# xmengli/H-DenseUNet

Hardware: AMD Instinct MI355X
Metric: CT slices/sec fwd+bwd (2D 512^2) (higher is better)
Workload: dtype bf16

## Files before the change

h-denseunet_amd/csrc/conv_halo_wide.hip:

```cpp
#include "conv_common.h"
#include "hdu_host.h"

typedef float f32x16 __attribute__((ext_vector_type(16)));

__device__ __forceinline__ f32x16 hdu_mfma_32x32x16_bf16(u32x4 a, u32x4 b, f32x16 c) {
#ifdef HDU_EMU
  return hipemu_mfma_32x32x16_bf16(__builtin_bit_cast(hipemu_u16x8, a), __builtin_bit_cast(hipemu_u16x8, b), c);
#else
  return __builtin_amdgcn_mfma_f32_32x32x16_bf16(__builtin_bit_cast(hdu_bf16x8, a), __builtin_bit_cast(hdu_bf16x8, b), c, 0, 0, 0);
#endif
}

template <int N> __device__ __forceinline__ void hw_wait_vmcnt() {
  static_assert(N >= 0 && N < 64, "vmcnt immediate");
#ifndef HDU_EMU
  asm volatile("s_waitcnt vmcnt(%0)" ::"i"(N) : "memory");
#endif
}

template <int TH_, int NT_, int WAVES_M_, int WAVES_N_, int NS_> struct HaloWide {
  static constexpr int TH = TH_, NT = NT_, WAVES_M = WAVES_M_, WAVES_N = WAVES_N_, NS = NS_;
  static constexpr int NW = WAVES_M * WAVES_N, NTHR = NW * 64;
  static constexpr int TW = 32, HC = TW + 2, HR = TH + 2, HP = HR * HC;
  static constexpr int BN = NT * 32, BM = TH * TW;
  static constexpr int XI = (HP * 2 + 63) / 64;
  static constexpr int WI = (BN * 18 + 63) / 64;
  static constexpr int LPW = (XI + WI + NW - 1) / NW;
  static constexpr int STAGE = LPW * NW * 1024;
  static constexpr int XBYTES = XI * 1024;
  static constexpr int ROWB = BN * 2 + 16;
  static constexpr int SMEM = NS * STAGE > BM * ROWB ? NS * STAGE : BM * ROWB;
  static constexpr int MT = TH / WAVES_M, NTW = NT / WAVES_N;
  static_assert(TH % WAVES_M == 0 && NT % WAVES_N == 0, "wave layout");
  static_assert(SMEM <= 160 * 1024, "LDS");
  static_assert((NS - 2) * LPW < 64, "vmcnt");
};

template <typename C, typename RowValid>
__device__ __forceinline__ void hw_epilogue_stats(const ConvK& p, const char* smem, int n0, int tid, unsigned slot, RowValid valid) {
  constexpr int NCC = C::BN / 8, CPI = C::NTHR / 16;
  float* dst = p.stats_partial + (long long)(slot % (unsigned)p.stats_slots) * 2 * p.Cout;
  const int rl = tid & 15;
#pragma unroll 1
  for (int it = 0; it < (NCC + CPI - 1) / CPI; ++it) {
    const int cc = (tid >> 4) + it * CPI;
    const int nbase = n0 + cc * 8;
    const bool col = cc < NCC && nbase < p.Cout;
    const int ccq = col ? cc : 0, nc = col ? nbase : 0;
    float s1[8], s2[8], sh[8];
#pragma unroll
    for (int j = 0; j < 8; j += 4) {
      const f32x4 v4 = *(const f32x4*)(p.stats_shift + nc + j);
      sh[j] = v4[0]; sh[j + 1] = v4[1]; sh[j + 2] = v4[2]; sh[j + 3] = v4[3];
    }
#pragma unroll
    for (int j = 0; j < 8; ++j) { s1[j] = 0.f; s2[j] = 0.f; }
#pragma unroll 1
    for (int q0 = 0; q0 < C::BM / 16; q0 += 8) {
      u32x4 rv[8];
#pragma unroll
      for (int q = 0; q < 8; ++q) rv[q] = *(const u32x4*)(smem + (rl + (q0 + q) * 16) * C::ROWB + ccq * 16);
#pragma unroll
      for (int q = 0; q < 8; ++q) {
        const float keep = (col && valid(rl + (q0 + q) * 16)) ? 1.f : 0.f;
        float f[8];
        Chunk<bf16_t>::unpack(rv[q], f);
#pragma unroll
        for (int j = 0; j < 8; ++j) { const float d = (f[j] - sh[j]) * keep; s1[j] += d; s2[j] += d * d; }
      }
    }
#pragma unroll
    for (int j = 0; j < 8; ++j) { s1[j] = hdu_row16_sum(s1[j]); s2[j] = hdu_row16_sum(s2[j]); }
    float mine = 0.f;
#pragma unroll
    for (int j = 0; j < 8; ++j) {
      mine = rl == j ? s1[j] : mine;
      mine = rl == 8 + j ? s2[j] : mine;
    }
    if (col) atomicAdd(dst + (rl < 8 ? 0 : p.Cout) + nbase + (rl & 7), mine);
  }
}

template <typename C>
__device__ __forceinline__ void hw_epilogue(const ConvK& p, f32x16 (&acc)[C::MT][C::NTW], char* smem, long long mplane, int y0, int x0,
                                            int n0, int wm, int wn, int lane, int tid, unsigned slot) {
  typedef bf16_t T;
  constexpr int BN = C::BN, BM = C::BM, NTHR = C::NTHR, ROWB = C::ROWB, MT = C::MT, NTW = C::NTW;
  const int l31 = lane & 31, lh = lane >> 5;
  hw_wait_vmcnt<0>();
  __syncthreads();
  const unsigned dseed = p.drop_seed + (p.drop_seed_dev ? *p.drop_seed_dev : 0u);
  const bool has_bias = p.bias != nullptr, drop = p.drop_scale != 0.f, has_epi = p.epi_a != nullptr;
#pragma unroll
  for (int j = 0; j < NTW; ++j) {
    f32x4 bias_v[4], epa_v[4], epb_v[4];
#pragma unroll
    for (int g = 0; g < 4; ++g) {
      const int nn = n0 + (wn * NTW + j) * 32 + 8 * g + 4 * lh;
      const int nc = nn < p.Cout ? nn : 0;
      bias_v[g] = has_bias ? *(const f32x4*)(p.bias + nc) : f32x4{0.f, 0.f, 0.f, 0.f};
      epa_v[g] = has_epi ? *(const f32x4*)(p.epi_a + nc) : f32x4{1.f, 1.f, 1.f, 1.f};
      epb_v[g] = has_epi ? *(const f32x4*)(p.epi_b + nc) : f32x4{0.f, 0.f, 0.f, 0.f};
    }
#pragma unroll
    for (int i = 0; i < MT; ++i) {
      const int trow = wm * MT + i;
      const int row = trow * 32 + l31;
      const long long m = (mplane + y0 + trow) * p.Wo + x0 + l31;
#pragma unroll
      for (int g = 0; g < 4; ++g) {
        const int col = (wn * NTW + j) * 32 + 8 * g + 4 * lh;
        const int nn = n0 + col;
        float v[4] = {acc[i][j][4 * g], acc[i][j][4 * g + 1], acc[i][j][4 * g + 2], acc[i][j][4 * g + 3]};
        if (has_bias) {
#pragma unroll
          for (int r = 0; r < 4; ++r) v[r] += bias_v[g][r];
        }
        if (drop) {
#pragma unroll
          for (int r = 0; r < 4; ++r) {
            const unsigned h = hdu_hash32((unsigned long long)m * (unsigned)p.Cout + (unsigned)(nn + r), dseed);
            v[r] = h < p.drop_thresh ? v[r] * p.drop_scale : 0.f;
          }
        }
        if (has_epi) {
#pragma unroll
          for (int r = 0; r < 4; ++r) {
            v[r] = epa_v[g][r] * v[r] + epb_v[g][r];
            if (p.epi_relu) v[r] = v[r] > 0.f ? v[r] : 0.f;
          }
        }
        Chunk<T>::store4((T*)(smem + row * ROWB) + col, v);
      }
    }
  }
  __syncthreads();
  T* __restrict__ yp = (T*)p.y;
  constexpr int NCC = BN / 8;
  constexpr int NIT = (BM * NCC + NTHR - 1) / NTHR;
  auto out_ptr = [&](int q, bool& ok) -> T* {
    const int row = q / NCC, cc = q - row * NCC;
    const int oy = y0 + (row >> 5), ox = x0 + (row & 31);
    const int nn = n0 + cc * 8;
    ok = q < BM * NCC && oy < p.Ho && ox < p.Wo && nn < p.Cout;
    return ok ? yp + ((mplane + oy) * p.Wo + ox) * p.ldy + nn : yp;
  };
  if (p.accumulate) {
#pragma unroll 1
    for (int it0 = 0; it0 < NIT; it0 += 4) {
      u32x4 old[4];
      T* dst[4];
      bool ok[4];
#pragma unroll
      for (int u = 0; u < 4; ++u) {
        dst[u] = out_ptr(tid + (it0 + u) * NTHR, ok[u]);
        ok[u] = ok[u] && it0 + u < NIT;
        old[u] = *(const u32x4*)dst[u];
      }
#pragma unroll
      for (int u = 0; u < 4; ++u) {
        if (!ok[u]) continue;
        const int q = tid + (it0 + u) * NTHR;
        const int row = q / NCC, cc = q - row * NCC;
        float f[8], g[8];
        Chunk<T>::unpack(*(const u32x4*)(smem + row * ROWB + cc * 16), f);
        Chunk<T>::unpack(old[u], g);
#pragma unroll
        for (int jj = 0; jj < 8; ++jj) f[jj] += g[jj];
        *(u32x4*)dst[u] = Chunk<T>::pack(f);
      }
    }
  } else {
#pragma unroll
    for (int it = 0; it < NIT; ++it) {
      const int q = tid + it * NTHR;
      bool ok;
      T* dst = out_ptr(q, ok);
      if (!ok) continue;
      const int row = q / NCC, cc = q - row * NCC;
      *(u32x4*)dst = *(const u32x4*)(smem + row * ROWB + cc * 16);
    }
  }
  if (p.stats_partial)
    hw_epilogue_stats<C>(p, smem, n0, tid, slot, [&](int row) { return y0 + (row >> 5) < p.Ho && x0 + (row & 31) < p.Wo; });
}

template <typename C>
__global__ __launch_bounds__(C::NTHR) void conv_halo_wide_kernel(ConvK p, int tiles_x, int tiles_y, int ngroups) {
  typedef bf16_t T;
  constexpr int TH = C::TH, HC = C::HC, HP = C::HP, BN = C::BN, BM = C::BM, NW = C::NW, NTHR = C::NTHR, NS = C::NS;
  constexpr int XI = C::XI, WI = C::WI, LPW = C::LPW, STAGE = C::STAGE, XBYTES = C::XBYTES, ROWB = C::ROWB;
  constexpr int MT = C::MT, NTW = C::NTW;
  __shared__ __attribute__((aligned(16))) char smem[C::SMEM];

  const int tid = threadIdx.x;
  const int lane = tid & 63;
#ifdef HDU_EMU
  const int wave = tid >> 6;
#else
  const int wave = __builtin_amdgcn_readfirstlane(tid >> 6);
#endif
  const int wm = wave / C::WAVES_N, wn = wave % C::WAVES_N;
  const T* __restrict__ xp = (const T*)p.x;
  const int He = p.He, We = p.We;

  unsigned t = (p.xcd_swizzle & 1) ? xcd_tile_index(blockIdx.x, gridDim.x) : blockIdx.x;
  const int ng = (int)(t % (unsigned)ngroups); t /= (unsigned)ngroups;
  const int od = (int)(t % (unsigned)p.Do); t /= (unsigned)p.Do;
  const int txi = (int)(t % (unsigned)tiles_x); t /= (unsigned)tiles_x;
  const int tyi = (int)(t % (unsigned)tiles_y);
  const int n = (int)(t / (unsigned)tiles_y);
  const int y0 = tyi * TH, x0 = txi * C::TW;
  const int n0 = ng * BN;

  unsigned roff[LPW];
  int rlc[LPW];
#pragma unroll
  for (int j = 0; j < LPW; ++j) {
    const int jj = j * NW + wave;
    if (jj < XI) {
      const int q = jj * 64 + lane;
      const int hp = q >> 1;
      const int lc = (q & 1) ^ ((hp >> 3) & 1);
      const int hr = hp / HC, hc = hp - hr * HC;
      const int iy = y0 - 1 + hr, ix = x0 - 1 + hc;
      const bool ok = hp < HP && (unsigned)iy < (unsigned)He && (unsigned)ix < (unsigned)We;
      roff[j] = ok ? (unsigned)(((iy >> p.uh) * p.Wi + (ix >> p.uw)) * (int)p.ldx + lc * 8) * 2u : HDU_OOB;
      rlc[j] = lc * 8;
    } else if (jj < XI + WI) {
      const int q = (jj - XI) * 64 + lane;
      const int row = q / 18, rem = q - row * 18;
      const int tap = rem >> 1;
      const int lc = (rem & 1) ^ ((row >> 3) & 1);
      const int co = n0 + row;
      const bool ok = row < BN && co < p.Cout;
      roff[j] = ok ? (unsigned)((co * p.KD * 9 + tap) * p.Cin + lc * 8) * 2u : HDU_OOB;
      rlc[j] = lc * 8;
    } else {
      roff[j] = HDU_OOB;
      rlc[j] = 0;
    }
  }
  const hdu_bufsrd wsrd = hdu_make_srd(p.w, p.w_bytes);
  const long long plane_elems = (long long)p.Hi * p.Wi * p.ldx;
  const unsigned plane_bytes = (unsigned)((((long long)p.Hi * p.Wi - 1) * p.ldx + p.Cin) * 2);

  auto stage_plane = [&](int kd, int c0) -> const T* {
    const int pz = od + kd - p.pd;
    return xp + (long long)(n * p.Di + (pz >> p.ud)) * plane_elems + c0;
  };
  auto issue_piece = [&](const hdu_bufsrd& xsrd, unsigned woff, int c0, char* base, int j, bool live) {
    const int jj = j * NW + wave;
    const bool ok = live && roff[j] != HDU_OOB && c0 + rlc[j] < p.Cin;
    if (jj < XI) hdu_bufload_lds16(xsrd, ok ? roff[j] : HDU_OOB, base + jj * 1024);
    else hdu_bufload_lds16(wsrd, ok ? roff[j] + woff : HDU_OOB, base + jj * 1024);
  };

  f32x16 acc[MT][NTW];
#pragma unroll
  for (int i = 0; i < MT; ++i)
#pragma unroll
    for (int j = 0; j < NTW; ++j)
#pragma unroll
      for (int r = 0; r < 16; ++r) acc[i][j][r] = 0.f;

  const int kd_lo = p.pd - od > 0 ? p.pd - od : 0;
  const int kd_hi = p.De + p.pd - od < p.KD ? p.De + p.pd - od : p.KD;
  const int nch = (p.Cin + 15) >> 4;
  const int nst = kd_hi > kd_lo ? (kd_hi - kd_lo) * nch : 0;
  int ikd = kd_lo, ic = 0;
#pragma unroll
  for (int pre = 0; pre < NS - 1; ++pre) {
    const bool live = pre < nst;
    const int c0 = live ? ic * 16 : 0;
    const hdu_bufsrd xsrd = hdu_make_srd(stage_plane(live ? ikd : kd_lo, c0), plane_bytes - (unsigned)c0 * 2u);
    const unsigned woff = (unsigned)(ikd * 9 * p.Cin + c0) * 2u;
#pragma unroll
    for (int j = 0; j < LPW; ++j) issue_piece(xsrd, woff, c0, smem + pre * STAGE, j, live);
    if (live && ++ic == nch) { ic = 0; ++ikd; }
  }

  const int l31 = lane & 31, lh = lane >> 5;
  int wrow_off[NTW];
#pragma unroll
  for (int j = 0; j < NTW; ++j) {
    const int row = (wn * NTW + j) * 32 + l31;
    wrow_off[j] = XBYTES + row * 288 + ((lh ^ ((row >> 3) & 1)) << 4);
  }
  const int hp_base = wm * MT * HC + l31;

  int slot = 0;
  for (int s = 0; s < nst; ++s) {
    hw_wait_vmcnt<(NS - 2) * LPW>();
    HDU_RAW_BARRIER();
    const bool more = s + NS - 1 < nst;
    const int nc0 = more ? ic * 16 : 0;
    const hdu_bufsrd nxsrd = hdu_make_srd(stage_plane(more ? ikd : kd_lo, nc0), plane_bytes - (unsigned)nc0 * 2u);
    const unsigned nwoff = (unsigned)(ikd * 9 * p.Cin + nc0) * 2u;
    char* nbase = smem + (slot == 0 ? NS - 1 : slot - 1) * STAGE;
    if (more && ++ic == nch) { ic = 0; ++ikd; }
    const char* Xs = smem + slot * STAGE;
    constexpr int PER_TAP = (LPW + 8) / 9;
#pragma unroll
    for (int tap = 0; tap < 9; ++tap) {
      const int kh = tap / 3, kw = tap - kh * 3;
      u32x4 af[MT], bf[NTW];
#pragma unroll
      for (int i = 0; i < MT; ++i) {
        const int hp = hp_base + (i + kh) * HC + kw;
        af[i] = *(const u32x4*)(Xs + hp * 32 + ((lh ^ ((hp >> 3) & 1)) << 4));
      }
#pragma unroll
      for (int j = 0; j < NTW; ++j) bf[j] = *(const u32x4*)(Xs + wrow_off[j] + tap * 32);
#pragma unroll
      for (int i = 0; i < MT; ++i)
#pragma unroll
        for (int j = 0; j < NTW; ++j) acc[i][j] = hdu_mfma_32x32x16_bf16(bf[j], af[i], acc[i][j]);
#pragma unroll
      for (int u = 0; u < PER_TAP; ++u)
        if (tap * PER_TAP + u < LPW) issue_piece(nxsrd, nwoff, nc0, nbase, tap * PER_TAP + u, more);
    }
    slot = slot == NS - 1 ? 0 : slot + 1;
  }

  const long long mplane = ((long long)n * p.Do + od) * p.Ho;
  hw_epilogue<C>(p, acc, smem, mplane, y0, x0, n0, wm, wn, lane, tid, blockIdx.x);
}

struct StemCfg {
  static constexpr int TH = 16, NT = 3, WAVES_M = 8, WAVES_N = 1, NS = 4;
  static constexpr int NW = 8, NTHR = 512, TW = 32;
  static constexpr int BN = 96, BM = TH * TW;
  static constexpr int SEG = 70;
  static constexpr int XSLOTS = TH * SEG;
  static constexpr int XI = (XSLOTS + 63) / 64;
  static constexpr int WSLOTS = BN * 9;
  static constexpr int WI = (WSLOTS + 63) / 64;
  static constexpr int LPW = (XI + WI + NW - 1) / NW;
  static constexpr int STAGE = LPW * NW * 1024;
  static constexpr int XBYTES = XI * 1024;
  static constexpr int ROWB = BN * 2 + 16;
  static constexpr int SMEM = NS * STAGE > BM * ROWB ? NS * STAGE : BM * ROWB;
  static constexpr int MT = 2, NTW = 3;
  static_assert(SMEM <= 160 * 1024, "LDS");
};

__global__ __launch_bounds__(StemCfg::NTHR) void conv_stem_s2_kernel(ConvK p, int tiles_x, int tiles_y, int ngroups) {
  typedef StemCfg C;
  typedef bf16_t T;
  constexpr int NW = C::NW, NS = C::NS, XI = C::XI, WI = C::WI, LPW = C::LPW, STAGE = C::STAGE, XBYTES = C::XBYTES, SEG = C::SEG;
  constexpr int MT = C::MT, NTW = C::NTW, BN = C::BN;
  __shared__ __attribute__((aligned(16))) char smem[C::SMEM];
  const int tid = threadIdx.x;
  const int lane = tid & 63;
#ifdef HDU_EMU
  const int wave = tid >> 6;
#else
  const int wave = __builtin_amdgcn_readfirstlane(tid >> 6);
#endif
  const T* __restrict__ xp = (const T*)p.x;
  unsigned t = (p.xcd_swizzle & 1) ? xcd_tile_index(blockIdx.x, gridDim.x) : blockIdx.x;
  const int ng = (int)(t % (unsigned)ngroups); t /= (unsigned)ngroups;
  const int od = (int)(t % (unsigned)p.Do); t /= (unsigned)p.Do;
  const int txi = (int)(t % (unsigned)tiles_x); t /= (unsigned)tiles_x;
  const int tyi = (int)(t % (unsigned)tiles_y);
  const int n = (int)(t / (unsigned)tiles_y);
  const int y0 = tyi * C::TH, x0 = txi * C::TW;
  const int n0 = ng * BN;

  unsigned roff[LPW];
  int riy[LPW];
#pragma unroll
  for (int j = 0; j < LPW; ++j) {
    const int jj = j * NW + wave;
    riy[j] = -(1 << 28);
    if (jj < XI) {
      const int ps = jj * 64 + lane;
      const int q = ps ^ ((ps >> 4) & 1);
      const int r = q / SEG, c = q - r * SEG;
      const int iy = 2 * (y0 + r) - p.ph, ix = 2 * x0 - p.pw + c;
      const bool ok = q < C::XSLOTS && (unsigned)ix < (unsigned)p.Wi;
      roff[j] = ok ? (unsigned)((iy * p.Wi + ix) * (int)p.ldx) * 2u : HDU_OOB;
      riy[j] = ok ? iy : -(1 << 28);
    } else if (jj < XI + WI) {
      const int ps = (jj - XI) * 64 + lane;
      const int row = ps / 9, kw = ps - row * 9;
      const int co = n0 + row;
      const bool ok = row < BN && co < p.Cout && kw < 7;
      roff[j] = ok ? (unsigned)((co * p.KD * 49 + kw) * 8) * 2u : HDU_OOB;
    } else {
      roff[j] = HDU_OOB;
    }
  }
  const hdu_bufsrd wsrd = hdu_make_srd(p.w, p.w_bytes);
  const long long plane_elems = (long long)p.Hi * p.Wi * p.ldx;
  const unsigned plane_bytes = (unsigned)((((long long)p.Hi * p.Wi - 1) * p.ldx + 8) * 2);
  const int row_bytes = p.Wi * (int)p.ldx * 2;

  auto stage_plane = [&](int kd) -> const T* {
    const int pz = od * p.sd + kd - p.pd;
    return xp + (long long)(n * p.Di + pz) * plane_elems;
  };
  auto issue_piece = [&](const hdu_bufsrd& xsrd, int kd, int kh, char* base, int j, bool live) {
    const int jj = j * NW + wave;
    if (jj < XI) {
      const bool ok = live && (unsigned)(riy[j] + kh) < (unsigned)p.Hi;
      hdu_bufload_lds16(xsrd, ok ? roff[j] + (unsigned)(kh * row_bytes) : HDU_OOB, base + jj * 1024);
    } else {
      const bool ok = live && roff[j] != HDU_OOB;
      hdu_bufload_lds16(wsrd, ok ? roff[j] + (unsigned)((kd * 7 + kh) * 7 * 8 * 2) : HDU_OOB, base + jj * 1024);
    }
  };

  f32x16 acc[MT][NTW];
#pragma unroll
  for (int i = 0; i < MT; ++i)
#pragma unroll
    for (int j = 0; j < NTW; ++j)
#pragma unroll
      for (int r = 0; r < 16; ++r) acc[i][j][r] = 0.f;

  const int pz0 = od * p.sd - p.pd;
  const int kd_lo = pz0 < 0 ? -pz0 : 0;
  const int kd_hi = p.Di - pz0 < p.KD ? p.Di - pz0 : p.KD;
  const int nst = kd_hi > kd_lo ? (kd_hi - kd_lo) * 7 : 0;
  int ikd = kd_lo, ikh = 0;
#pragma unroll
  for (int pre = 0; pre < NS - 1; ++pre) {
    const bool live = pre < nst;
    const hdu_bufsrd xsrd = hdu_make_srd(stage_plane(live ? ikd : kd_lo), plane_bytes);
#pragma unroll
    for (int j = 0; j < LPW; ++j) issue_piece(xsrd, ikd, ikh, smem + pre * STAGE, j, live);
    if (live && ++ikh == 7) { ikh = 0; ++ikd; }
  }

  const int l31 = lane & 31, lh = lane >> 5;
  int wrow_off[NTW];
#pragma unroll
  for (int j = 0; j < NTW; ++j) wrow_off[j] = XBYTES + ((j * 32 + l31) * 9 + lh) * 16;
  int xq[MT];
#pragma unroll
  for (int i = 0; i < MT; ++i) xq[i] = (wave * MT + i) * SEG + 2 * l31 + lh;

  int slot = 0;
  for (int s = 0; s < nst; ++s) {
    hw_wait_vmcnt<(NS - 2) * LPW>();
    HDU_RAW_BARRIER();
    const bool more = s + NS - 1 < nst;
    const hdu_bufsrd nxsrd = hdu_make_srd(stage_plane(more ? ikd : kd_lo), plane_bytes);
    const int nkd = ikd, nkh = ikh;
    char* nbase = smem + (slot == 0 ? NS - 1 : slot - 1) * STAGE;
    if (more && ++ikh == 7) { ikh = 0; ++ikd; }
    const char* Xs = smem + slot * STAGE;
#pragma unroll
    for (int ks = 0; ks < 4; ++ks) {
      u32x4 af[MT], bf[NTW];
#pragma unroll
      for (int i = 0; i < MT; ++i) {
        const int q = xq[i] + 2 * ks;
        af[i] = *(const u32x4*)(Xs + ((q ^ ((q >> 4) & 1)) << 4));
      }
#pragma unroll
      for (int j = 0; j < NTW; ++j) bf[j] = *(const u32x4*)(Xs + wrow_off[j] + ks * 32);
#pragma unroll
      for (int i = 0; i < MT; ++i)
#pragma unroll
        for (int j = 0; j < NTW; ++j) acc[i][j] = hdu_mfma_32x32x16_bf16(bf[j], af[i], acc[i][j]);
      if (ks < LPW) issue_piece(nxsrd, nkd, nkh, nbase, ks, more);
    }
    slot = slot == NS - 1 ? 0 : slot + 1;
  }
  const long long mplane = ((long long)n * p.Do + od) * p.Ho;
  hw_epilogue<C>(p, acc, smem, mplane, y0, x0, n0, wave, 0, lane, tid, blockIdx.x);
}

template <int NS_> struct StemWT {
  static constexpr int TH = 4, TW = 32, PX = TH * TW, SEG = 70, NR = 2 * TH + 5, NW = 8, NTHR = 512, NS = NS_;
  static constexpr int DSLOTS = PX * 12, DI = DSLOTS / 64;
  static constexpr int XSLOTS = NR * SEG, XI = (XSLOTS + 63) / 64;
  static constexpr int LPW = (DI + XI + NW - 1) / NW;
  static constexpr int STAGE = LPW * NW * 1024, DBYTES = DI * 1024;
  static_assert(NS * STAGE <= 160 * 1024, "LDS");
};

typedef StemWT<2> StemW;
template <int NS_>
__global__ __launch_bounds__(StemW::NTHR) void conv_stem_wgrad_kernel(ConvK p, float* __restrict__ dw, int tiles_x, int tiles_y,
                                                                      int nsplit, int ngroups) {
// ... 292 lines not shown
```

h-denseunet_amd/csrc/conv_igemm.hip:

```cpp
#include "conv_common.h"
#include "../../include/hdu.h"

template <typename T, int BM, int BN> struct BnbGeom {
  static constexpr int CH = Chunk<T>::CH;
  static constexpr int NCC = BN / CH;
  static constexpr int NCCP = NCC <= 4 ? 4 : (NCC <= 8 ? 8 : (NCC <= 16 ? 16 : 32));
  static constexpr int RSTEP = 256 / NCCP;
  static constexpr int IT = (BM + RSTEP - 1) / RSTEP;
  static constexpr bool EARLY = IT <= 8;
  static_assert(NCC <= 32, "tile shape");
};

template <bool SPLIT, typename T, int BM, int BN, int WAVES_M, int WAVES_N>
__device__ __forceinline__ void conv_igemm_body(const ConvK& p, char* smem) {
  constexpr int CH = Chunk<T>::CH;
  constexpr int BK = 8 * CH;
  constexpr int A_IT = BM / 32;
  constexpr int B_IT = (BN + 31) / 32;
  constexpr int WM = BM / WAVES_M;
  constexpr int WN = BN / WAVES_N;
  constexpr int TM = WM / 16;
  constexpr int TN = WN / 16;
  constexpr int STAGE = (BM + BN) * 128;
  static_assert(WAVES_M * WAVES_N == 4, "4 waves");
// ... 2429 lines not shown
#pragma unroll
        for (int i = 0; i < 2; ++i)
#pragma unroll
          for (int j = 0; j < TN; ++j) acc[i][j] = Mma<T>::kgroup(bf[j], af[i], acc[i][j]);
      }
    }
    __syncthreads();
  }

  constexpr int ROWB = BN * 2 + 16;
  const unsigned dseed = p.drop_seed + (p.drop_seed_dev ? *p.drop_seed_dev : 0u);
  const bool has_bias = p.bias != nullptr, drop = p.drop_scale != 0.f, has_epi = p.epi_a != nullptr;
  f32x4 bias_v[TN], epa_v[TN], epb_v[TN];
#pragma unroll
  for (int j = 0; j < TN; ++j) {
    const int nn = n0 + j * 16 + lg * 4;
    const int nc = nn < p.Cout ? nn : 0;
    bias_v[j] = has_bias ? *(const f32x4*)(p.bias + nc) : f32x4{0.f, 0.f, 0.f, 0.f};
    epa_v[j] = has_epi ? *(const f32x4*)(p.epi_a + nc) : f32x4{1.f, 1.f, 1.f, 1.f};
    epb_v[j] = has_epi ? *(const f32x4*)(p.epi_b + nc) : f32x4{0.f, 0.f, 0.f, 0.f};
  }
#pragma unroll
  for (int i = 0; i < 2; ++i) {
    const int tx = i * 16 + li;
    const int row = wave * 32 + tx;
    const long long m = ((long long)(n * H + y0 + wave)) * W + x0 + tx;
#pragma unroll
    for (int j = 0; j < TN; ++j) {
      const int col = j * 16 + lg * 4;
      const int nn = n0 + col;
      float v[4] = {acc[i][j][0], acc[i][j][1], acc[i][j][2], acc[i][j][3]};
      if (has_bias) {
#pragma unroll
        for (int r = 0; r < 4; ++r) v[r] += bias_v[j][r];
      }
      if (drop) {
#pragma unroll
        for (int r = 0; r < 4; ++r) {
          const unsigned h = hdu_hash32((unsigned long long)m * (unsigned)p.Cout + (unsigned)(nn + r), dseed);
          v[r] = h < p.drop_thresh ? v[r] * p.drop_scale : 0.f;
        }
      }
      if (has_epi) {
#pragma unroll
        for (int r = 0; r < 4; ++r) {
          v[r] = epa_v[j][r] * v[r] + epb_v[j][r];
          if (p.epi_relu) v[r] = v[r] > 0.f ? v[r] : 0.f;
        }
      }
      Chunk<T>::store4((T*)(smem + row * ROWB) + col, v);
    }
  }
  __syncthreads();
  T* __restrict__ yp = (T*)p.y;
  constexpr int NCC = BN / 8;
  for (int q = tid; q < BM * NCC; q += 256) {
    const int row = q / NCC, cc = q - row * NCC;
    const int oy = y0 + (row >> 5), ox = x0 + (row & 31);
    const int nn = n0 + cc * 8;
    if (oy >= H || ox >= W || nn >= p.Cout) continue;
    u32x4 v = *(const u32x4*)(smem + row * ROWB + cc * 16);
    T* dst = yp + (((long long)(n * H + oy)) * W + ox) * p.ldy + nn;
    if (p.accumulate) {
      float f[8], g[8];
      Chunk<T>::unpack(v, f);
      Chunk<T>::unpack(*(const u32x4*)dst, g);
#pragma unroll
      for (int jj = 0; jj < 8; ++jj) f[jj] += g[jj];
      v = Chunk<T>::pack(f);
    }
    *(u32x4*)dst = v;
  }
  if (p.stats_partial)
    epilogue_stats<T, BM, BN, ROWB>(p, smem, n0, tid, blockIdx.x,
                                    [&](int row) { return y0 + (row >> 5) < H && x0 + (row & 31) < W; });
}

template <typename T>
__global__ __launch_bounds__(256) void conv_dgrad_strided_kernel(ConvK p) {
  constexpr int CH = Chunk<T>::CH;
  const int ncc = p.Cin / CH;
  const long long total = (long long)p.N * p.Di * p.Hi * p.Wi * ncc;
  const T* __restrict__ dyp = (const T*)p.y;
  const T* __restrict__ wp = (const T*)p.w;
  T* __restrict__ dxp = (T*)p.x;
  for (long long q = (long long)blockIdx.x * blockDim.x + threadIdx.x; q < total;
       q += (long long)gridDim.x * blockDim.x) {
    const int cc = (int)(q % ncc);
    long long pix = q / ncc;
    const int iw = (int)(pix % p.Wi);
    long long t = pix / p.Wi;
    const int ih = (int)(t % p.Hi);
    t /= p.Hi;
    const int id = (int)(t % p.Di);
    const int n = (int)(t / p.Di);
    float acc[CH];
#pragma unroll
    for (int j = 0; j < CH; ++j) acc[j] = 0.f;
    for (int kd = 0; kd < p.KD; ++kd) {
      const int td = id + p.pd - kd;
      if (td < 0 || td % p.sd) continue;
      const int od = td / p.sd;
      if (od >= p.Do) continue;
      for (int kh = 0; kh < p.KH; ++kh) {
        const int th = ih + p.ph - kh;
        if (th < 0 || th % p.sh) continue;
        const int oh = th / p.sh;
        if (oh >= p.Ho) continue;
        for (int kw = 0; kw < p.KW; ++kw) {
          const int tw = iw + p.pw - kw;
          if (tw < 0 || tw % p.sw) continue;
          const int ow = tw / p.sw;
          if (ow >= p.Wo) continue;
          const long long m = (((long long)n * p.Do + od) * p.Ho + oh) * p.Wo + ow;
          const int tap = (kd * p.KH + kh) * p.KW + kw;
          const T* dyr = dyp + m * p.ldy;
          const T* wr = wp + (long long)tap * p.Cin + cc * CH;
          for (int co = 0; co < p.Cout; ++co) {
            const float g = Chunk<T>::load1(dyr + co);
            float wv[CH];
            Chunk<T>::unpack(*(const u32x4*)(wr + (long long)co * p.Ktot), wv);
#pragma unroll
            for (int j = 0; j < CH; ++j) acc[j] += g * wv[j];
          }
        }
      }
    }
    T* o = dxp + pix * p.ldx + cc * CH;
    if (p.accumulate) {
      float old[CH];
      Chunk<T>::unpack(*(const u32x4*)o, old);
#pragma unroll
      for (int j = 0; j < CH; ++j) acc[j] += old[j];
    }
    *(u32x4*)o = Chunk<T>::pack(acc);
  }
}

struct ParityGeom {
  int nt[3];
  int kmax[3];
  int step[3];
  long long dst_off;
};
struct ParityTable { ParityGeom c[8]; int n; };

template <typename T>
__global__ __launch_bounds__(256) void stride2_filter_kernel(const float* __restrict__ wm, int Cout, int KD, int KH, int KW,
                                                            int Cin, ParityTable tab, T* __restrict__ out) {
  const ParityGeom g = tab.c[blockIdx.y];
  const long long total = (long long)Cin * g.nt[0] * g.nt[1] * g.nt[2] * Cout;
  for (long long q = (long long)blockIdx.x * blockDim.x + threadIdx.x; q < total; q += (long long)gridDim.x * blockDim.x) {
    const int co = (int)(q % Cout);
    long long t = q / Cout;
    const int tw = (int)(t % g.nt[2]); t /= g.nt[2];
    const int th = (int)(t % g.nt[1]); t /= g.nt[1];
    const int td = (int)(t % g.nt[0]);
    const int ci = (int)(t / g.nt[0]);
    const int kd = g.kmax[0] - g.step[0] * td, kh = g.kmax[1] - g.step[1] * th, kw = g.kmax[2] - g.step[2] * tw;
    const float v = wm[((((long long)co * KD + kd) * KH + kh) * KW + kw) * Cin + ci];
    Chunk<T>::store1(out + g.dst_off + q, v);
  }
}

template <typename T>
__global__ __launch_bounds__(256) void parity_interleave_kernel(const T* __restrict__ cls, int N, int Di, int Hi, int Wi, int C,
                                                               int sd, int sh, int sw, T* __restrict__ dx, long long lddx,
                                                               int accumulate) {
  constexpr int CH = Chunk<T>::CH;
  const int ncc = C / CH;
  const long long total = (long long)N * Di * Hi * Wi * ncc;
  const int Dq = (Di + sd - 1) / sd, Hq = (Hi + sh - 1) / sh, Wq = (Wi + sw - 1) / sw;
  const long long cls_elems = (long long)N * Dq * Hq * Wq * C;
  for (long long q = (long long)blockIdx.x * blockDim.x + threadIdx.x; q < total; q += (long long)gridDim.x * blockDim.x) {
    const int cc = (int)(q % ncc);
    long long pix = q / ncc;
    const int iw = (int)(pix % Wi);
    long long t = pix / Wi;
    const int ih = (int)(t % Hi);
    t /= Hi;
    const int id = (int)(t % Di);
    const int n = (int)(t / Di);
    const int rd = id % sd, rh = ih % sh, rw = iw % sw;
    const int ci = (rd * sh + rh) * sw + rw;
    const long long src = ci * cls_elems + ((((long long)n * Dq + id / sd) * Hq + ih / sh) * Wq + iw / sw) * C + cc * CH;
    u32x4 v = *(const u32x4*)(cls + src);
    T* o = dx + pix * lddx + cc * CH;
    if (accumulate) {
      float a[CH], b[CH];
      Chunk<T>::unpack(v, a);
      Chunk<T>::unpack(*(const u32x4*)o, b);
#pragma unroll
      for (int j = 0; j < CH; ++j) a[j] += b[j];
      v = Chunk<T>::pack(a);
    }
    *(u32x4*)o = v;
  }
}

template <typename T>
__global__ __launch_bounds__(256) void weight_prep_kernel(const float* __restrict__ wm, int Cout, int Tn, int Cin,
                                                         T* __restrict__ wf, T* __restrict__ wd) {
  const long long total = (long long)Cout * Tn * Cin;
  for (long long q = (long long)blockIdx.x * blockDim.x + threadIdx.x; q < total;
       q += (long long)gridDim.x * blockDim.x) {
    const int ci = (int)(q % Cin);
    const long long t2 = q / Cin;
    const int t = (int)(t2 % Tn);
    const int co = (int)(t2 / Tn);
    const float v = wm[q];
    if (wf) Chunk<T>::store1(wf + q, v);
    if (wd) Chunk<T>::store1(wd + ((long long)ci * Tn + (Tn - 1 - t)) * Cout + co, v);
  }
}

#define HDU_PREP_TPW 2
template <typename T>
__global__ __launch_bounds__(256) void weight_prep_batched_kernel(const hdu_prep_entry* __restrict__ table, int n,
                                                                 const float* __restrict__ master, T* __restrict__ wc,
                                                                 long long total_tiles) {
  __shared__ float tile[2][64][65];
  const long long t0 = (long long)blockIdx.x * HDU_PREP_TPW;
  int lo = 0, hi = n - 1;
  while (lo < hi) {
    const int mid = (lo + hi + 1) >> 1;
    if (table[mid].tile_begin <= t0) lo = mid; else hi = mid - 1;
  }
  hdu_prep_entry e = table[lo];
  long long next_begin = lo + 1 < n ? table[lo + 1].tile_begin : total_tiles;
  const int tx = threadIdx.x & 15, ty = threadIdx.x >> 4;
  for (int it = 0; it < HDU_PREP_TPW; ++it) {
    const long long t = t0 + it;
    if (t >= total_tiles) break;
    while (t >= next_begin) {
      ++lo;
      e = table[lo];
      next_begin = lo + 1 < n ? table[lo + 1].tile_begin : total_tiles;
    }
    const int t_local = (int)(t - e.tile_begin);
    const int nci = (e.Cin + 63) / 64, nco = (e.Cout + 63) / 64;
    const int cib = t_local % nci;
    const int cob = (t_local / nci) % nco;
    const int tap = t_local / (nci * nco);
    const float* wm = master + e.master_off;
    T* wf = e.w_f_off >= 0 ? wc + e.w_f_off : nullptr;
    T* wd = e.w_d_off >= 0 ? wc + e.w_d_off : nullptr;
    float (*tl)[65] = tile[it & 1];
    const bool vec = ((e.master_off | (e.w_f_off >= 0 ? e.w_f_off : 0) | (e.w_d_off >= 0 ? e.w_d_off : 0) | (long long)e.Cin | (long long)e.Cout) & 3) == 0 &&
                     (((uintptr_t)master | (uintptr_t)wc) & 15) == 0;
    if (vec) {
#pragma unroll
      for (int k = 0; k < 4; ++k) {
        const int r = ty + 16 * k;
        const int co = cob * 64 + r, ci = cib * 64 + tx * 4;
        float v[4] = {0.f, 0.f, 0.f, 0.f};
        if (co < e.Cout && ci < e.Cin) {
          const long long q = ((long long)co * e.T + tap) * e.Cin + ci;
          const f32x4 m = *(const f32x4*)(wm + q);
          v[0] = m.x; v[1] = m.y; v[2] = m.z; v[3] = m.w;
          if (wf) Chunk<T>::store4(wf + q, v);
        }
#pragma unroll
        for (int j = 0; j < 4; ++j) tl[r][tx * 4 + j] = v[j];
      }
      __syncthreads();
      if (wd) {
#pragma unroll
        for (int k = 0; k < 4; ++k) {
          const int r = ty + 16 * k;
          const int ci = cib * 64 + r, co = cob * 64 + tx * 4;
          if (co < e.Cout && ci < e.Cin) {
            const float v[4] = {tl[tx * 4 + 0][r], tl[tx * 4 + 1][r], tl[tx * 4 + 2][r], tl[tx * 4 + 3][r]};
            Chunk<T>::store4(wd + ((long long)ci * e.T + (e.T - 1 - tap)) * e.Cout + co, v);
          }
        }
      }
    } else {
      for (int idx = threadIdx.x; idx < 64 * 64; idx += 256) {
        const int r = idx >> 6, c = idx & 63;
        const int co = cob * 64 + r, ci = cib * 64 + c;
        float v = 0.f;
        if (co < e.Cout && ci < e.Cin) {
          const long long q = ((long long)co * e.T + tap) * e.Cin + ci;
          v = wm[q];
          if (wf) Chunk<T>::store1(wf + q, v);
        }
        tl[r][c] = v;
      }
      __syncthreads();
      if (wd) {
        for (int idx = threadIdx.x; idx < 64 * 64; idx += 256) {
          const int r = idx >> 6, c = idx & 63;
          const int ci = cib * 64 + r, co = cob * 64 + c;
          if (co < e.Cout && ci < e.Cin)
            Chunk<T>::store1(wd + ((long long)ci * e.T + (e.T - 1 - tap)) * e.Cout + co, tl[c][r]);
        }
      }
    }
  }
}

#include "hdu_host.h"

int g_tuning[32] = {2, 0, 0, 1, 0, 0, 0, 0, 0, 0, 0, 0, 0, 0, 0, 0, 0, 0, 0, 0, 0, 0, 0, 0, 0, 0, 0, 0, 0, 0, 0, 0};

extern "C" int hdu_set_tuning(int key, int value) {
  if (key < 0 || key >= 32) return hdu_set_error(HDU_ERR_ARG, "set_tuning: bad key");
  g_tuning[key] = value;
  return 0;
}

static void fastdiv_magic(int d, unsigned* mul, unsigned* shr) {
  if (d <= 1) { *mul = 0u; *shr = 0u; return; }
  int cl = 0;
  while ((1ll << cl) < (long long)d) ++cl;
  const int p = 31 + cl;
  *mul = (unsigned)((((unsigned long long)1 << p) + (unsigned long long)d - 1) / (unsigned long long)d);
  *shr = (unsigned)(p - 32);
}

static int fill_convk(const hdu_conv_desc* d, ConvK* k, bool wgrad, bool exact_grid = false) {
  if (!d) return hdu_set_error(HDU_ERR_ARG, "conv: null descriptor");
  if (d->dtype != HDU_BF16 && d->dtype != HDU_F32) return hdu_set_error(HDU_ERR_ARG, "conv: bad dtype");
  const int ch = d->dtype == HDU_BF16 ? 8 : 4;
  if (d->Cin <= 0 || d->Cin % ch) return hdu_set_error(HDU_ERR_ARG, "conv: Cin must be a positive multiple of the 16-byte chunk");
  if (d->ldx % ch || (d->skip && d->ldskip % ch)) return hdu_set_error(HDU_ERR_ARG, "conv: input pixel stride must be a multiple of the 16-byte chunk");
  if (wgrad && (d->ldy % ch || d->Cout % ch)) return hdu_set_error(HDU_ERR_ARG, "conv_wgrad: dy stride / Cout must be multiples of the 16-byte chunk");
  if ((uintptr_t)d->x % 16 || (uintptr_t)d->w % 16 || (d->skip && (uintptr_t)d->skip % 16))
    return hdu_set_error(HDU_ERR_ARG, "conv: x / w / skip must be 16-byte aligned");
  if ((d->ud | d->uh | d->uw) & ~1) return hdu_set_error(HDU_ERR_ARG, "conv: upsample shifts must be 0 or 1");
  if (d->KD <= 0 || d->KH <= 0 || d->KW <= 0 || d->sd <= 0 || d->sh <= 0 || d->sw <= 0)
    return hdu_set_error(HDU_ERR_ARG, "conv: bad kernel/stride");
  if ((d->pro_a == nullptr) != (d->pro_b == nullptr)) return hdu_set_error(HDU_ERR_ARG, "conv: pro_a/pro_b must both be set");
  k->x = d->x; k->skip = d->skip; k->w = d->w; k->y = d->y;
  k->pro_a = d->pro_a; k->pro_b = d->pro_b; k->bias = d->bias;
  k->epi_a = wgrad ? nullptr : d->epi_a; k->epi_b = d->epi_b; k->epi_relu = d->epi_relu;
  if (k->epi_a && (!k->epi_b || d->accumulate || d->stats_partial || d->bnb_u))
    return hdu_set_error(HDU_ERR_ARG, "conv: the output affine needs epi_b and excludes accumulate / epilogue statistics / the fused BN backward");
  k->ldx = d->ldx; k->ldskip = d->ldskip; k->ldy = d->ldy;
  k->N = d->N; k->Di = d->Di; k->Hi = d->Hi; k->Wi = d->Wi; k->Cin = d->Cin;
  k->ud = d->ud; k->uh = d->uh; k->uw = d->uw;
  k->De = d->Di << d->ud; k->He = d->Hi << d->uh; k->We = d->Wi << d->uw;
  k->KD = d->KD; k->KH = d->KH; k->KW = d->KW;
  k->sd = d->sd; k->sh = d->sh; k->sw = d->sw;
  k->pd = d->pd; k->ph = d->ph; k->pw = d->pw;
  k->Do = d->Do; k->Ho = d->Ho; k->Wo = d->Wo; k->Cout = d->Cout;
  const int eDo = (k->De + 2 * d->pd - d->KD) / d->sd + 1;
  const int eHo = (k->He + 2 * d->ph - d->KH) / d->sh + 1;
  const int eWo = (k->We + 2 * d->pw - d->KW) / d->sw + 1;
  const bool exact = wgrad || exact_grid;
  const int xd = exact ? 0 : d->KD - 1, xh = exact ? 0 : d->KH - 1, xw = exact ? 0 : d->KW - 1;
  if (d->Do < eDo || d->Do > eDo + xd || d->Ho < eHo || d->Ho > eHo + xh || d->Wo < eWo || d->Wo > eWo + xw)
    return hdu_set_error(HDU_ERR_ARG, "conv: output dims inconsistent with input dims / kernel / stride / pad");
  k->M = (long long)d->N * d->Do * d->Ho * d->Wo;
  if ((long long)d->N * k->De * k->He * k->We >= (1ll << 31) || k->M >= (1ll << 31))
    return hdu_set_error(HDU_ERR_ARG, "conv: more than 2^31 pixels per tensor (shard the volume)");
  k->Ktot = d->KD * d->KH * d->KW * d->Cin;
  fastdiv_magic(d->Wo, &k->div_wo_mul, &k->div_wo_shr);
  fastdiv_magic(d->Ho, &k->div_ho_mul, &k->div_ho_shr);
  fastdiv_magic(d->Do, &k->div_do_mul, &k->div_do_shr);
  k->spread_h = k->spread_d = 0u;
  if (d->KD * d->KH * d->KW <= 32) {
    for (int q = 0; q < d->KH; ++q) k->spread_h |= 1u << (q * d->KW);
    for (int q = 0; q < d->KD; ++q) k->spread_d |= 1u << (q * d->KH * d->KW);
  }
  fastdiv_magic(d->Cin, &k->div_cin_mul, &k->div_cin_shr);
  fastdiv_magic(d->KW, &k->div_kw_mul, &k->div_kw_shr);
  fastdiv_magic(d->KH, &k->div_kh_mul, &k->div_kh_shr);
  k->sk_div_mul = 0u; k->sk_div_shr = 0u;
  {
    const long long esz = d->dtype == HDU_BF16 ? 2 : 4;
    const long long xb = (((long long)d->N * d->Di * d->Hi * d->Wi - 1) * d->ldx + d->Cin) * esz;
    const long long wb = (long long)d->Cout * k->Ktot * esz;
    k->x_bytes = xb > 0 && xb < (1ll << 32) ? (unsigned)xb : 0u;
    if (g_tuning[HDU_TUNE_DEBUG] & 16) k->x_bytes = 0u;
    if (!wgrad && wb >= (1ll << 32)) return hdu_set_error(HDU_ERR_ARG, "conv: filter larger than 4 GiB");
    k->w_bytes = (unsigned)wb;
  }
  k->pro_relu = d->pro_relu; k->accumulate = d->accumulate;
  if (d->drop_keep > 0.f && d->drop_keep < 1.f) {
    k->drop_scale = 1.f / d->drop_keep;
    k->drop_thresh = (unsigned)((double)d->drop_keep * 4294967296.0);
  } else {
    k->drop_scale = 0.f;
    k->drop_thresh = 0xffffffffu;
  }
  k->drop_seed = d->drop_seed;
  k->drop_seed_dev = d->drop_seed_dev;
  k->stats_partial = wgrad ? nullptr : d->stats_partial;
  k->stats_shift = d->stats_shift;
  k->stats_slots = d->stats_slots;
  if (k->stats_partial && (!k->stats_shift || k->stats_slots <= 0 || d->accumulate))
    return hdu_set_error(HDU_ERR_ARG, "conv: epilogue statistics need stats_shift, stats_slots > 0 and accumulate == 0");
  k->bnb_u = wgrad ? nullptr : d->bnb_u; k->bnb_ldu = d->bnb_ldu;
  k->bnb_a = d->bnb_a; k->bnb_b = d->bnb_b; k->bnb_mean = d->bnb_mean; k->bnb_rstd = d->bnb_rstd;
  k->bnb_relu = d->bnb_relu; k->bnb_partial = d->bnb_partial; k->bnb_slots = d->bnb_slots;
  if (k->bnb_u) {
    if (!k->bnb_a || !k->bnb_b || (uintptr_t)k->bnb_u % 16 || k->bnb_ldu % ch || d->pro_a || d->skip || d->bias ||
        d->stats_partial || (d->drop_keep > 0.f && d->drop_keep < 1.f))
      return hdu_set_error(HDU_ERR_ARG, "conv: the fused BN backward needs bnb_a/bnb_b, a 16-byte addressable bnb_u and a plain data-gradient launch (no prologue / skip / bias / dropout / statistics)");
    if (k->bnb_partial && (!k->bnb_mean || !k->bnb_rstd || k->bnb_slots <= 0))
      return hdu_set_error(HDU_ERR_ARG, "conv: bnb_partial needs bnb_mean, bnb_rstd and bnb_slots > 0");
  }
  if (((uintptr_t)k->bias | (uintptr_t)k->epi_a | (uintptr_t)k->epi_b | (uintptr_t)(k->stats_partial ? k->stats_shift : nullptr) |
       (uintptr_t)k->bnb_a | (uintptr_t)k->bnb_b | (uintptr_t)k->bnb_mean | (uintptr_t)k->bnb_rstd) & 15)
    return hdu_set_error(HDU_ERR_ARG, "conv: bias / epi_* / stats_shift / bnb_* vectors must be 16-byte aligned");
  k->M_layer = d->layer_rows > 0 ? d->layer_rows : k->M;
  k->sk_ws = wgrad ? nullptr : (float*)d->splitk_ws;
  k->sk_cnt = wgrad ? nullptr : d->splitk_counters;
  if (k->sk_ws && ((uintptr_t)k->sk_ws % 16 || !k->sk_cnt))
    return hdu_set_error(HDU_ERR_ARG, "conv: splitk_ws must be 16-byte aligned and come with splitk_counters");
  k->xcd_swizzle = g_tuning[HDU_TUNE_XCD_SWIZZLE];
  k->vec_out = 1;
  k->debug_flags = g_tuning[HDU_TUNE_DEBUG];
  k->f32_split = (d->dtype == HDU_F32 && g_tuning[HDU_TUNE_F32_SPLIT]) ? 1 : 0;
  if (!wgrad && d->y && (d->Cout % ch || d->ldy % ch || (uintptr_t)d->y % 16))
    return hdu_set_error(HDU_ERR_ARG, "conv: Cout / output pixel stride must be multiples of the 16-byte chunk and y 16-byte aligned");
  return 0;
}

static bool igemm_fast_ok(const ConvK& k) {
  if (g_tuning[HDU_TUNE_NO_FAST]) return false;
  if ((k.ud | k.uh | k.uw) != 0 || k.KD * k.KH * k.KW > 32) return false;
  const long long span = ((long long)k.N * k.De * k.He * k.We + (long long)k.He * k.We * 8) * k.ldx;
  return span < (1ll << 31) && k.x_bytes != 0;
}

static bool conv_pointwise(const ConvK& k) {
  return k.KD * k.KH * k.KW == 1 && k.sd == 1 && k.sh == 1 && k.sw == 1 && (k.pd | k.ph | k.pw) == 0 && (k.ud | k.uh | k.uw) == 0;
}

static bool igemm_pro_dma_ok(const ConvK& k) {
  return k.pro_a != nullptr && k.skip == nullptr && k.vec_out && k.bnb_u == nullptr && conv_pointwise(k) && k.Cin <= HDU_PRO_CMAX &&
         k.Do == k.De && k.Ho == k.He && k.Wo == k.We && igemm_fast_ok(k) && !g_tuning[HDU_TUNE_NO_PRO_DMA] &&
         ((uintptr_t)k.pro_a % 16 == 0) && ((uintptr_t)k.pro_b % 16 == 0);
}

static int ring_wgs_per_cu(int bm, bool bf16) { return (bm == 64 && bf16) ? 2 : 1; }

static int choose_splitk(long long nblk, int nk, int bm, int bn, int per_cu, size_t* bytes) {
  *bytes = 0;
  const int mode = g_tuning[HDU_TUNE_SPLITK];
  const int target = g_tuning[HDU_TUNE_SPLITK_TARGET] > 0 ? g_tuning[HDU_TUNE_SPLITK_TARGET] : 256 * per_cu;
  const int min_steps = g_tuning[HDU_TUNE_SPLITK_MIN_STEPS] > 0 ? g_tuning[HDU_TUNE_SPLITK_MIN_STEPS] : 4;
  if (mode == 1 || nblk > target / 2) return 1;
  int S = mode >= 2 ? mode : (int)((target + nblk - 1) / nblk);
  if (S > nk / min_steps) S = nk / min_steps;
  if (S > 16) S = 16;
  if (S < 2) return 1;
  *bytes = (size_t)nblk * (size_t)S * (size_t)bm * (size_t)bn * sizeof(float);
  return S;
}

static bool igemm_ring_ok(long long nblk, int Ktot, int stage_bytes, int nsd) {
  const int mode = g_tuning[HDU_TUNE_DMA_STAGES];
  return stage_bytes * nsd <= 160 * 1024 && (mode == 6 || (mode == 2 && nblk <= 256 && Ktot > g_tuning[HDU_TUNE_RING_MIN_K]));
}

template <typename T, int BM, int BN, int PROC> struct ProRing {
  static constexpr int STAGE = (BM + ((BN + 31) / 32) * 32) * 128;
  static constexpr int NSD = STAGE * 6 <= 160 * 1024 ? 6 : 4;
  static constexpr int NSR0 = (BM == 64 && sizeof(T) == 2 && NSD == 6) ? 3 : NSD;
  static constexpr int NSR = (NSR0 * STAGE + 8 * PROC <= 160 * 1024) ? NSR0 : (NSR0 == 6 ? 4 : 3);
  static_assert(NSR * STAGE + 8 * PROC <= 160 * 1024, "LDS");
};

template <typename T, int BM, int BN, int WMv, int WNv, int PROC>
static void launch_igemm_pro(const ConvK& k, dim3 grid, size_t sk_bytes_avail, hipStream_t s) {
  typedef ProRing<T, BM, BN, PROC> R;
  const long long nblk = (long long)grid.x * grid.y;
  const long long nblk_layer = (long long)((k.M_layer + BM - 1) / BM) * grid.y;
  if (igemm_ring_ok(nblk_layer, k.Ktot, R::STAGE, R::NSD)) {
    constexpr int BK = 8 * Chunk<T>::CH;
    size_t need;
    const int S = choose_splitk(nblk_layer, (k.Ktot + BK - 1) / BK, BM, BN, ring_wgs_per_cu(BM, sizeof(T) == 2), &need);
    need = need / (size_t)nblk_layer * (size_t)nblk;
    ConvK kk = k;
    if (S > 1 && k.sk_ws && k.sk_cnt && need <= sk_bytes_avail && nblk <= 512) {
      grid.z = (unsigned)S;
      fastdiv_magic(S, &kk.sk_div_mul, &kk.sk_div_shr);
    }
    HDU_LAUNCH((conv_igemm_ring_kernel<T, BM, BN, WMv, WNv, R::NSR, true, false, PROC>), grid, dim3(256), 0, s, kk);
  } else {
    HDU_LAUNCH((conv_igemm_dma_kernel<T, BM, BN, WMv, WNv, true, false, PROC>), grid, dim3(256), 0, s, k);
  }
}

template <typename T, int BM, int BN, int WMv, int WNv>
static void launch_igemm(const ConvK& k, size_t sk_bytes_avail, hipStream_t s) {
  dim3 grid((unsigned)((k.M + BM - 1) / BM), (unsigned)((k.Cout + BN - 1) / BN), 1);
  if (igemm_pro_dma_ok(k)) {
    if (k.Cin <= HDU_PRO_CSMALL) launch_igemm_pro<T, BM, BN, WMv, WNv, HDU_PRO_CSMALL>(k, grid, sk_bytes_avail, s);
    else launch_igemm_pro<T, BM, BN, WMv, WNv, HDU_PRO_CMAX>(k, grid, sk_bytes_avail, s);
    return;
  }
  if (k.pro_a == nullptr && k.skip == nullptr && k.vec_out) {
    constexpr int STAGE = (BM + ((BN + 31) / 32) * 32) * 128;
    constexpr int NSD = STAGE * 6 <= 160 * 1024 ? 6 : 4;
    const long long nblk = (long long)grid.x * grid.y;
    const long long nblk_layer = (long long)((k.M_layer + BM - 1) / BM) * grid.y;
    const int mode = g_tuning[HDU_TUNE_DMA_STAGES];
    const bool fast = igemm_fast_ok(k);
    if (igemm_ring_ok(nblk_layer, k.Ktot, STAGE, NSD)) {
      constexpr int BK = 8 * Chunk<T>::CH;
      size_t need;
      const int S = choose_splitk(nblk_layer, (k.Ktot + BK - 1) / BK, BM, BN, ring_wgs_per_cu(BM, sizeof(T) == 2), &need);
      need = need / (size_t)nblk_layer * (size_t)nblk;
      ConvK kk = k;
      if (S > 1 && k.sk_ws && k.sk_cnt && need <= sk_bytes_avail && nblk <= 512) {
        grid.z = (unsigned)S;
        fastdiv_magic(S, &kk.sk_div_mul, &kk.sk_div_shr);
      }
      constexpr int NSR = (BM == 64 && sizeof(T) == 2 && NSD == 6) ? 3 : NSD;
      if (k.bnb_u != nullptr) {
        if (fast) HDU_LAUNCH((conv_igemm_ring_kernel<T, BM, BN, WMv, WNv, NSR, true, true>), grid, dim3(256), 0, s, kk);
        else HDU_LAUNCH((conv_igemm_ring_kernel<T, BM, BN, WMv, WNv, NSR, false, true>), grid, dim3(256), 0, s, kk);
      } else if (fast) HDU_LAUNCH((conv_igemm_ring_kernel<T, BM, BN, WMv, WNv, NSR, true>), grid, dim3(256), 0, s, kk);
      else HDU_LAUNCH((conv_igemm_ring_kernel<T, BM, BN, WMv, WNv, NSR, false>), grid, dim3(256), 0, s, kk);
    } else {
      if (k.bnb_u != nullptr) {
        if (fast) HDU_LAUNCH((conv_igemm_dma_kernel<T, BM, BN, WMv, WNv, true, true>), grid, dim3(256), 0, s, k);
        else HDU_LAUNCH((conv_igemm_dma_kernel<T, BM, BN, WMv, WNv, false, true>), grid, dim3(256), 0, s, k);
      } else if (fast) HDU_LAUNCH((conv_igemm_dma_kernel<T, BM, BN, WMv, WNv, true>), grid, dim3(256), 0, s, k);
      else HDU_LAUNCH((conv_igemm_dma_kernel<T, BM, BN, WMv, WNv, false>), grid, dim3(256), 0, s, k);
    }
  } else
    HDU_LAUNCH((conv_igemm_kernel<T, BM, BN, WMv, WNv>), grid, dim3(256), 0, s, k);
}

static void choose_igemm(const ConvK& k, int* bm, int* bn) {
  const int cands[5] = {128, 96, 64, 48, 32};
  int best = 64;
  long long best_cost = -1;
  const int maxbn = g_tuning[HDU_TUNE_MAX_BN] > 0 ? g_tuning[HDU_TUNE_MAX_BN] : 128;
  for (int i = 0; i < 5; ++i) {
    const int c = cands[i];
    if (c > maxbn) continue;
    const long long ntiles = (k.Cout + c - 1) / c;
    const long long cost = ntiles * (c + 32);
    if (best_cost < 0 || cost < best_cost) { best_cost = cost; best = c; }
  }
  *bn = best;
  *bm = (k.M_layer <= (g_tuning[HDU_TUNE_BM64_MAX_M] > 0 ? (long long)g_tuning[HDU_TUNE_BM64_MAX_M] : 16384)) ? 64 : 128;
}

template <int BM, int BN> struct WaveLayout {
  static constexpr int WM = (BN >= 128) ? 2 : ((BM == 64 && (BN == 64 || BN == 32)) ? 2 : 4);
  static constexpr int WN = 4 / WM;
};

template <typename T, int BM>
static void dispatch_igemm_bn(const ConvK& k, int bn, size_t skb, hipStream_t s) {
  switch (bn) {
    case 128: launch_igemm<T, BM, 128, WaveLayout<BM, 128>::WM, WaveLayout<BM, 128>::WN>(k, skb, s); return;
    case 96: launch_igemm<T, BM, 96, WaveLayout<BM, 96>::WM, WaveLayout<BM, 96>::WN>(k, skb, s); return;
    case 64: launch_igemm<T, BM, 64, WaveLayout<BM, 64>::WM, WaveLayout<BM, 64>::WN>(k, skb, s); return;
    case 48: launch_igemm<T, BM, 48, WaveLayout<BM, 48>::WM, WaveLayout<BM, 48>::WN>(k, skb, s); return;
    default: launch_igemm<T, BM, 32, WaveLayout<BM, 32>::WM, WaveLayout<BM, 32>::WN>(k, skb, s); return;
  }
}

static int pers_table_cap(int bn, int cin) {
  const int stage3 = 3 * (256 + bn) * 128;
  if (cin <= HDU_PRO_CSMALL && stage3 + 8 * HDU_PRO_CSMALL <= 160 * 1024) return HDU_PRO_CSMALL;
  if (stage3 + 8 * HDU_PRO_CMAX <= 160 * 1024) return HDU_PRO_CMAX;
  return -1;
}

static bool igemm_pers_ok(const ConvK& k, int bn) {
  if (g_tuning[HDU_TUNE_PERS] == 0) return false;
  if (k.skip != nullptr || !k.vec_out || k.bnb_u != nullptr || !igemm_fast_ok(k)) return false;
  if (k.f32_split) return false;
  if (k.pro_a != nullptr && (!igemm_pro_dma_ok(k) || pers_table_cap(bn, k.Cin) < 0)) return false;
  const long long items = ((k.M_layer + 255) / 256) * ((k.Cout + bn - 1) / bn);
  const int min_items = g_tuning[HDU_TUNE_PERS_MIN_ITEMS] > 0 ? g_tuning[HDU_TUNE_PERS_MIN_ITEMS] : 512;
  return items >= min_items && k.M < (1ll << 31) - 256;
}

template <typename T, int BN>
static void launch_pers(const ConvK& k, hipStream_t s) {
  const int tiles_m = (int)((k.M + 255) / 256), tiles_n = (k.Cout + BN - 1) / BN;
  const int cus = g_tuning[HDU_TUNE_PERS] > 1 ? g_tuning[HDU_TUNE_PERS] : 256;
  long long items = (long long)tiles_m * tiles_n;
  const dim3 grid((unsigned)(items < cus ? items : cus));
  if (k.pro_a != nullptr) {
    const int cap = pers_table_cap(BN, k.Cin);
    if (cap == HDU_PRO_CSMALL) {
      if constexpr (3 * (256 + BN) * 128 + 8 * HDU_PRO_CSMALL <= 160 * 1024)
        HDU_LAUNCH((conv_igemm_pers_kernel<T, BN, HDU_PRO_CSMALL>), grid, dim3(512), 0, s, k, tiles_m, tiles_n);
    } else {
      if constexpr (3 * (256 + BN) * 128 + 8 * HDU_PRO_CMAX <= 160 * 1024)
        HDU_LAUNCH((conv_igemm_pers_kernel<T, BN, HDU_PRO_CMAX>), grid, dim3(512), 0, s, k, tiles_m, tiles_n);
    }
  } else {
    HDU_LAUNCH((conv_igemm_pers_kernel<T, BN, 0>), grid, dim3(512), 0, s, k, tiles_m, tiles_n);
  }
}

template <typename T>
static void dispatch_igemm(const ConvK& k, size_t skb, hipStream_t s) {
  int bm, bn;
  choose_igemm(k, &bm, &bn);
  if (bm == 128 && igemm_pers_ok(k, bn)) {
    switch (bn) {
      case 128: launch_pers<T, 128>(k, s); return;
      case 96: launch_pers<T, 96>(k, s); return;
      case 64: launch_pers<T, 64>(k, s); return;
      case 48: launch_pers<T, 48>(k, s); return;
      default: launch_pers<T, 32>(k, s); return;
    }
  }
  if (bm == 64) dispatch_igemm_bn<T, 64>(k, bn, skb, s);
  else dispatch_igemm_bn<T, 128>(k, bn, skb, s);
}

bool hdu_halo_wide_taken(const ConvK& k, int dtype);
const char* hdu_halo_wide_name(const ConvK& k, int dtype);
bool hdu_halo_wide_launch(const ConvK& k, int dtype, hipStream_t s);
bool hdu_stem_wgrad_taken(const ConvK& k, int dtype);
bool hdu_stem_wgrad_launch(const ConvK& k, int dtype, float* dw, hipStream_t s);

static bool fprop_halo_ok(const ConvK& k, int dtype) {
  return dtype == HDU_BF16 && k.bnb_u == nullptr && !g_tuning[HDU_TUNE_NO_HALO_FPROP] && k.pro_a == nullptr && k.skip == nullptr && k.KD == 1 &&
         k.KH == 3 && k.KW == 3 && k.sd == 1 && k.sh == 1 && k.sw == 1 && k.pd == 0 && k.ph == 1 && k.pw == 1 &&
         (k.ud | k.uh | k.uw) == 0 && k.Di == 1 && k.Cin % 8 == 0 && k.We >= 32 && k.He >= 4 &&
         k.Do == 1 && k.Ho == k.He && k.Wo == k.We &&
         k.Cin >= 128 && k.Cout <= 96 &&
         (long long)k.N * ((k.He + 3) / 4) * ((k.We + 31) / 32) * k.M_layer / k.M >= (g_tuning[HDU_TUNE_HALO_MIN_TILES] > 0 ? g_tuning[HDU_TUNE_HALO_MIN_TILES] : 128);
}

static int choose_halo_bn(const ConvK& k) {
  const int cands[4] = {96, 64, 48, 32};
  int best = 64;
  long long best_cost = -1;
  for (int i = 0; i < 4; ++i) {
    const int c = cands[i];
    const long long cost = (long long)((k.Cout + c - 1) / c) * (c + 24);
    if (best_cost < 0 || cost < best_cost) { best_cost = cost; best = c; }
  }
  return best;
}

template <int BN>
static void launch_halo_fprop(const ConvK& k, hipStream_t s) {
  const unsigned tiles = (unsigned)(k.N * ((k.He + 3) / 4) * ((k.We + 31) / 32));
  HDU_LAUNCH((conv_halo_fprop_kernel<BN>), dim3(tiles, (unsigned)((k.Cout + BN - 1) / BN)), dim3(256), 0, s, k);
}

static bool pw_bstat_ok(const ConvK& k, int dtype) {
  return dtype == HDU_BF16 && !g_tuning[HDU_TUNE_NO_PW_BSTAT] && k.KD * k.KH * k.KW == 1 && k.sd == 1 && k.sh == 1 && k.sw == 1 &&
         (k.pd | k.ph | k.pw) == 0 && (k.ud | k.uh | k.uw) == 0 && k.pro_a == nullptr && k.skip == nullptr && k.bias == nullptr &&
         k.epi_a == nullptr && k.stats_partial == nullptr && (k.bnb_u != nullptr ? (!g_tuning[HDU_TUNE_NO_PW_BSTAT_BNB] && !(k.bnb_relu & 6)) : !k.accumulate) &&
         k.drop_scale == 0.f &&
         (k.Ktot == 128 || k.Ktot == 192) && k.Cout >= 256 && k.M >= 64 && k.x_bytes != 0 &&
         (k.M - 1) * k.ldy + k.Cout < (1ll << 31) && (k.bnb_u == nullptr || (k.M - 1) * k.bnb_ldu + k.Cout < (1ll << 31)) &&
         (long long)k.Cout * k.Ktot * 2 < (1ll << 31) && k.Do == k.De && k.Ho == k.He && k.Wo == k.We;
}

template <int BN, int NSA>
static void launch_pw_bstat_form(const ConvK& k, int target, hipStream_t s) {
  const unsigned ny = (unsigned)((k.Cout + BN - 1) / BN);
  long long splits = target / (long long)ny;
  if (splits < 1) splits = 1;
  const long long tiles = (k.M + 63) / 64;
  if (splits > tiles) splits = tiles;
  const long long rows = ((tiles + splits - 1) / splits) * 64;
  const unsigned gx = (unsigned)((k.M + rows - 1) / rows);
  if (k.bnb_u != nullptr) {
    if (k.Ktot == 192) HDU_LAUNCH((conv_pw_bstat_kernel<3, BN, true, NSA>), dim3(gx, ny), dim3(256), 0, s, k, (int)rows);
    else HDU_LAUNCH((conv_pw_bstat_kernel<2, BN, true, NSA>), dim3(gx, ny), dim3(256), 0, s, k, (int)rows);
    return;
  }
  if (k.Ktot == 192) HDU_LAUNCH((conv_pw_bstat_kernel<3, BN, false, NSA>), dim3(gx, ny), dim3(256), 0, s, k, (int)rows);
  else HDU_LAUNCH((conv_pw_bstat_kernel<2, BN, false, NSA>), dim3(gx, ny), dim3(256), 0, s, k, (int)rows);
}

static int pw_bstat_form(const ConvK& k) {
  const int f = g_tuning[HDU_TUNE_PW_BSTAT_FORM];
  if (f == 1 || f == 2) return f;
  return k.bnb_u != nullptr ? 2 : 1;
}

static void launch_pw_bstat(const ConvK& k, hipStream_t s) {
  const int wgs = g_tuning[HDU_TUNE_PW_BSTAT_WGS];
  if (pw_bstat_form(k) == 2) launch_pw_bstat_form<64, 2>(k, wgs > 0 ? wgs : 512, s);
  else launch_pw_bstat_form<128, 3>(k, wgs > 0 ? wgs : 256, s);
}

extern "C" int hdu_conv_fprop(const hdu_conv_desc* d, void* stream) {
  ConvK k;
  if (int e = fill_convk(d, &k, false)) return e;
  if (!d->y) return hdu_set_error(HDU_ERR_ARG, "conv_fprop: null output");
  if (k.M == 0) return 0;
  if (pw_bstat_ok(k, d->dtype)) {
    launch_pw_bstat(k, (hipStream_t)stream);
    return hdu_check_launch("conv_fprop(pointwise, filter-stationary)");
  }
  if (hdu_halo_wide_launch(k, d->dtype, (hipStream_t)stream)) return hdu_check_launch("conv_fprop(halo, wide)");
  if (fprop_halo_ok(k, d->dtype)) {
    switch (choose_halo_bn(k)) {
      case 96: launch_halo_fprop<96>(k, (hipStream_t)stream); break;
      case 64: launch_halo_fprop<64>(k, (hipStream_t)stream); break;
      case 48: launch_halo_fprop<48>(k, (hipStream_t)stream); break;
      default: launch_halo_fprop<32>(k, (hipStream_t)stream); break;
    }
    return hdu_check_launch("conv_fprop(halo)");
  }
  if (d->dtype == HDU_BF16) dispatch_igemm<bf16_t>(k, d->splitk_ws_bytes, (hipStream_t)stream);
  else dispatch_igemm<float>(k, d->splitk_ws_bytes, (hipStream_t)stream);
  return hdu_check_launch("conv_fprop");
}

extern "C" size_t hdu_conv_splitk_ws_bytes(const hdu_conv_desc* d) {
  ConvK k;
  if (fill_convk(d, &k, false)) return 0;
  if (k.M == 0 || pw_bstat_ok(k, d->dtype) || hdu_halo_wide_taken(k, d->dtype) || fprop_halo_ok(k, d->dtype) || (k.pro_a != nullptr && !igemm_pro_dma_ok(k)) || k.skip != nullptr) return 0;
  int bm, bn;
  choose_igemm(k, &bm, &bn);
  if (bm == 128 && igemm_pers_ok(k, bn)) return 0;
  const long long nblk = ((k.M + bm - 1) / bm) * ((k.Cout + bn - 1) / bn);
  const long long nblk_layer = ((k.M_layer + bm - 1) / bm) * ((k.Cout + bn - 1) / bn);
  const int stage = (bm + ((bn + 31) / 32) * 32) * 128;
  const int nsd = stage * 6 <= 160 * 1024 ? 6 : 4;
  if (!igemm_ring_ok(nblk_layer, k.Ktot, stage, nsd)) return 0;
  const int bk = d->dtype == HDU_BF16 ? 64 : 32;
  size_t need;
  choose_splitk(nblk_layer, (k.Ktot + bk - 1) / bk, bm, bn, ring_wgs_per_cu(bm, d->dtype == HDU_BF16), &need);
  return need / (size_t)nblk_layer * (size_t)nblk;
}

template <typename T, int BCO>
static void launch_wgrad(const ConvK& k, float* dw, hipStream_t s) {
  constexpr int PX = 8 * Chunk<T>::CH;
  const unsigned gx = (unsigned)((k.Ktot + 127) / 128), gy = (unsigned)((k.Cout + BCO - 1) / BCO);
  const long long target = g_tuning[HDU_TUNE_WGRAD_TARGET_WGS] > 0 ? g_tuning[HDU_TUNE_WGRAD_TARGET_WGS] : 1024;
  long long want = target / ((long long)gx * gy);
  if (want < 1) want = 1;
  long long steps = (k.M + PX - 1) / PX;
  if (want > steps) want = steps;
  long long steps_per = (steps + want - 1) / want;
  const long long rows_per = steps_per * PX;
  const unsigned gz = (unsigned)((k.M + rows_per - 1) / rows_per);
  HDU_LAUNCH((conv_wgrad_kernel<T, BCO>), dim3(gx, gy, gz), dim3(256), 0, s, k, dw, rows_per);
}

static int choose_wgrad(const ConvK& k) {
  const int cands[3] = {64, 48, 32};
  int best = 64;
  long long best_cost = -1;
  for (int i = 0; i < 3; ++i) {
    const long long padded = (long long)((k.Cout + cands[i] - 1) / cands[i]) * cands[i];
    if (best_cost < 0 || padded < best_cost) { best_cost = padded; best = cands[i]; }
  }
  return best;
}

static unsigned wgrad_grid(const ConvK& k) { return (unsigned)k.wg_gz * (unsigned)(k.wg_gx * k.wg_gy); }


static bool wgrad_pointwise(const ConvK& k) {
  return k.KD * k.KH * k.KW == 1 && k.sd == 1 && k.sh == 1 && k.sw == 1 && (k.pd | k.ph | k.pw) == 0 &&
         (k.ud | k.uh | k.uw) == 0;
}

static int wgrad_nct(const ConvK& k, int BCO) {
  if (g_tuning[HDU_TUNE_WGRAD_NCT] == 1 || !wgrad_pointwise(k) || BCO != 64) return 1;
  const int tiles = (k.Cout + BCO - 1) / BCO;
  return tiles >= 3 ? 3 : (tiles == 2 ? 2 : 1);
}

static bool wgrad_dma_ok(const ConvK& k) {
  return k.skip == nullptr && (k.pro_a == nullptr || (wgrad_pointwise(k) && !g_tuning[HDU_TUNE_NO_PRO_DMA]));
}

static long long wgrad_dma_geometry(const ConvK& k, int BCO, int target, ConvK* kk, int default_min_steps = 4, int nct = 1) {
  constexpr int PX = 64;
  const unsigned gx = (unsigned)((k.Ktot + 127) / 128), gy = (unsigned)((k.Cout + BCO * nct - 1) / (BCO * nct));
  long long want = target / ((long long)gx * gy);
  if (want < 1) want = 1;
  long long steps = (k.M + PX - 1) / PX;
  const int min_steps = g_tuning[HDU_TUNE_WGRAD_MIN_STEPS] > 0 ? g_tuning[HDU_TUNE_WGRAD_MIN_STEPS] : default_min_steps;
  if (want > (steps + min_steps - 1) / min_steps) want = (steps + min_steps - 1) / min_steps;
  if (want < 1) want = 1;
  long long steps_per = (steps + want - 1) / want;
  const long long rows_per = steps_per * PX;
  const unsigned gz = (unsigned)((k.M + rows_per - 1) / rows_per);
  *kk = k;
  kk->wg_gx = (int)gx; kk->wg_gy = (int)gy; kk->wg_gz = (int)gz;
  return rows_per;
}

template <int BCO>
static void launch_wgrad_tr(const ConvK& k, float* dw, hipStream_t s) {
  const int target = g_tuning[HDU_TUNE_WGRAD_TARGET_WGS] > 0 ? g_tuning[HDU_TUNE_WGRAD_TARGET_WGS] : 768;
  ConvK kk;
  const bool dma = wgrad_dma_ok(k);
  const int nct = dma ? wgrad_nct(k, BCO) : 1;
  const long long rows_per = wgrad_dma_geometry(k, BCO, target, &kk, 4, nct);
  if (dma) {
    if constexpr (BCO == 64) {
      if (nct == 3) { HDU_LAUNCH((conv_wgrad_dma_kernel<64, true, 3>), dim3(wgrad_grid(kk)), dim3(256), 0, s, kk, dw, rows_per); return; }
      if (nct == 2) { HDU_LAUNCH((conv_wgrad_dma_kernel<64, true, 2>), dim3(wgrad_grid(kk)), dim3(256), 0, s, kk, dw, rows_per); return; }
    }
    if (wgrad_pointwise(k)) HDU_LAUNCH((conv_wgrad_dma_kernel<BCO, true>), dim3(wgrad_grid(kk)), dim3(256), 0, s, kk, dw, rows_per);
    else HDU_LAUNCH((conv_wgrad_dma_kernel<BCO, false>), dim3(wgrad_grid(kk)), dim3(256), 0, s, kk, dw, rows_per);
  } else
    HDU_LAUNCH((conv_wgrad_tr_kernel<BCO>), dim3((unsigned)kk.wg_gx, (unsigned)kk.wg_gy, (unsigned)kk.wg_gz), dim3(256), 0, s,
               k, dw, rows_per);
}

static bool wgrad_halo_ok(const ConvK& k) {
  const bool d2 = k.KD == 1 && k.pd == 0 && k.Di == 1;
  const bool d3 = k.KD == 3 && k.pd >= -1 && k.pd <= 1 && k.Do == k.De + 2 * k.pd - 2 && k.Ho == k.He && k.Wo == k.We &&
                  !(g_tuning[HDU_TUNE_NO_HALO] & 2);
  return !(g_tuning[HDU_TUNE_NO_HALO] & 1) && k.pro_a == nullptr && k.skip == nullptr && (d2 || d3) && k.KH == 3 && k.KW == 3 &&
         k.sd == 1 && k.sh == 1 && k.sw == 1 && k.ph == 1 && k.pw == 1 &&
         ((k.ud | k.uh | k.uw) == 0 || !(g_tuning[HDU_TUNE_NO_HALO] & 4)) &&
         k.Cin % 8 == 0 && k.We >= (g_tuning[HDU_TUNE_HALO_MIN_W] > 0 ? g_tuning[HDU_TUNE_HALO_MIN_W] : 24) &&
         ((long long)k.Hi * k.Wi + k.Wi + 2) * k.ldx * 2 < (1ll << 31) && ((long long)k.He * k.We + k.We + 2) * k.ldy * 2 < (1ll << 31);
}

static int wgrad_halo_geometry(const ConvK& k, int BCO, int target, ConvK* kk, int min_tiles = 2) {
  const int tiles = k.N * k.Do * ((k.He + 3) / 4) * ((k.We + 31) / 32);
  const unsigned gx = (unsigned)((k.Cin + 31) / 32), gy = (unsigned)((k.Cout + BCO - 1) / BCO);
  int want = target / (int)(gx * gy * (unsigned)k.KD);
  if (want < 1) want = 1;
  if (min_tiles < 1) min_tiles = 1;
  if (want > (tiles + min_tiles - 1) / min_tiles) want = (tiles + min_tiles - 1) / min_tiles;
  if (want < 1) want = 1;
  const int per = (tiles + want - 1) / want;
  const unsigned gz = (unsigned)((tiles + per - 1) / per) * (unsigned)k.KD;
  *kk = k;
  kk->wg_gx = (int)gx; kk->wg_gy = (int)gy; kk->wg_gz = (int)gz;
  return per;
}

template <int BCO>
static void launch_wgrad_halo(const ConvK& k, float* dw, hipStream_t s) {
  const int target = g_tuning[HDU_TUNE_HALO_TARGET_WGS] > 0 ? g_tuning[HDU_TUNE_HALO_TARGET_WGS] : 512;
  ConvK kk;
  const int per = wgrad_halo_geometry(k, BCO, target, &kk);
  HDU_LAUNCH((conv_wgrad_halo_kernel<BCO>), dim3(wgrad_grid(kk)), dim3(256), 0, s, kk, dw, per);
}

template <typename T>
static void dispatch_wgrad(const ConvK& k, float* dw, hipStream_t s) {
  const int best = choose_wgrad(k);
  if (sizeof(T) == 2 && wgrad_halo_ok(k)) {
    if (best == 64) launch_wgrad_halo<64>(k, dw, s);
    else if (best == 48) launch_wgrad_halo<48>(k, dw, s);
    else launch_wgrad_halo<32>(k, dw, s);
    return;
  }
  if (sizeof(T) == 2) {
    if (best == 64) launch_wgrad_tr<64>(k, dw, s);
    else if (best == 48) launch_wgrad_tr<48>(k, dw, s);
    else launch_wgrad_tr<32>(k, dw, s);
    return;
  }
  if (best == 64) launch_wgrad<T, 64>(k, dw, s);
  else if (best == 48) launch_wgrad<T, 48>(k, dw, s);
  else launch_wgrad<T, 32>(k, dw, s);
}

extern "C" int hdu_conv_wgrad(const hdu_conv_desc* d, float* dw, void* stream) {
  ConvK k;
  if (int e = fill_convk(d, &k, true)) return e;
  if (!dw || !d->y) return hdu_set_error(HDU_ERR_ARG, "conv_wgrad: null dw / dy");
  if ((uintptr_t)d->y % 16) return hdu_set_error(HDU_ERR_ARG, "conv_wgrad: dy must be 16-byte aligned");
  if (k.M == 0) return 0;
  if (hdu_stem_wgrad_launch(k, d->dtype, dw, (hipStream_t)stream)) return hdu_check_launch("conv_wgrad(stem)");
  if (d->dtype == HDU_BF16) dispatch_wgrad<bf16_t>(k, dw, (hipStream_t)stream);
  else dispatch_wgrad<float>(k, dw, (hipStream_t)stream);
  return hdu_check_launch("conv_wgrad");
}

extern "C" size_t hdu_wgrad_plan_entry_bytes(void) { return sizeof(WgradEntry); }

extern "C" int hdu_wgrad_plan_fill(const hdu_conv_desc* d, float* dw, int target_wgs, int min_steps, void* entry, int* variant,
                                   uint32_t* nblocks) {
  if (!d || !dw || !entry || !variant || !nblocks) return hdu_set_error(HDU_ERR_ARG, "wgrad_plan_fill: null pointer");
  ConvK k;
  if (int e = fill_convk(d, &k, true)) return e;
  if (d->dtype != HDU_BF16 || !wgrad_dma_ok(k) || k.M == 0 || !d->y || (uintptr_t)d->y % 16)
    return hdu_set_error(HDU_ERR_ARG, "wgrad_plan_fill: only bf16 layers with materialised inputs (or pointwise layers with a BN prologue) and a 16-byte aligned dy can be batched");
  WgradEntry* e = (WgradEntry*)entry;
  const int best = choose_wgrad(k);
  const int bi = best == 64 ? 0 : (best == 48 ? 1 : 2);
  if (wgrad_halo_ok(k)) {
    const int target = target_wgs > 0 ? target_wgs : (g_tuning[HDU_TUNE_HALO_TARGET_WGS] > 0 ? g_tuning[HDU_TUNE_HALO_TARGET_WGS] : 512);
    e->per = wgrad_halo_geometry(k, best, target, &e->k, min_steps > 0 ? min_steps : 2);
    *variant = 8 + bi;
  } else {
    const int target = target_wgs > 0 ? target_wgs : (g_tuning[HDU_TUNE_WGRAD_TARGET_WGS] > 0 ? g_tuning[HDU_TUNE_WGRAD_TARGET_WGS] : 768);
    const int nct = wgrad_nct(k, best);
    e->per = wgrad_dma_geometry(k, best, target, &e->k, min_steps > 0 ? min_steps : 8, nct);
    *variant = nct == 3 ? 6 : (nct == 2 ? 7 : bi * 2 + (wgrad_pointwise(k) ? 1 : 0));
  }
  e->dw = dw;
  *nblocks = wgrad_grid(e->k);
  return 0;
}

extern "C" int hdu_wgrad_plan_shape(const hdu_conv_desc* d, int* variant, uint32_t* tiles, uint32_t* steps) {
  if (!d || !variant || !tiles || !steps) return hdu_set_error(HDU_ERR_ARG, "wgrad_plan_shape: null pointer");
  ConvK k;
  if (int e = fill_convk(d, &k, true)) return e;
  if (d->dtype != HDU_BF16 || !wgrad_dma_ok(k) || k.M == 0)
    return hdu_set_error(HDU_ERR_ARG, "wgrad_plan_shape: not a layer hdu_wgrad_plan_fill accepts");
  const int best = choose_wgrad(k);
  const int bi = best == 64 ? 0 : (best == 48 ? 1 : 2);
  if (wgrad_halo_ok(k)) {
    *variant = 8 + bi;
    *tiles = (uint32_t)((k.Cin + 31) / 32) * (uint32_t)((k.Cout + best - 1) / best) * (uint32_t)k.KD;
    *steps = (uint32_t)(k.N * k.Do * ((k.He + 3) / 4) * ((k.We + 31) / 32));
  } else {
    const int nct = wgrad_nct(k, best);
    *variant = nct == 3 ? 6 : (nct == 2 ? 7 : bi * 2 + (wgrad_pointwise(k) ? 1 : 0));
    *tiles = (uint32_t)((k.Ktot + 127) / 128) * (uint32_t)((k.Cout + best * nct - 1) / (best * nct));
    *steps = (uint32_t)((k.M + 63) / 64);
  }
  return 0;
}

extern "C" int hdu_wgrad_plan_run(int variant, const void* dev_entries, const uint32_t* dev_begins, int n,
                                  uint32_t total_blocks, void* stream) {
  if (!dev_entries || !dev_begins || n <= 0 || total_blocks == 0) return hdu_set_error(HDU_ERR_ARG, "wgrad_plan_run: bad args");
  const WgradEntry* tab = (const WgradEntry*)dev_entries;
  hipStream_t s = (hipStream_t)stream;
  const dim3 g(total_blocks), b(256);
  switch (variant) {
    case 0: HDU_LAUNCH((conv_wgrad_dma_batched_kernel<64, false>), g, b, 0, s, tab, dev_begins, n); break;
    case 1: HDU_LAUNCH((conv_wgrad_dma_batched_kernel<64, true>), g, b, 0, s, tab, dev_begins, n); break;
    case 2: HDU_LAUNCH((conv_wgrad_dma_batched_kernel<48, false>), g, b, 0, s, tab, dev_begins, n); break;
    case 3: HDU_LAUNCH((conv_wgrad_dma_batched_kernel<48, true>), g, b, 0, s, tab, dev_begins, n); break;
    case 4: HDU_LAUNCH((conv_wgrad_dma_batched_kernel<32, false>), g, b, 0, s, tab, dev_begins, n); break;
    case 5: HDU_LAUNCH((conv_wgrad_dma_batched_kernel<32, true>), g, b, 0, s, tab, dev_begins, n); break;
    case 6: HDU_LAUNCH((conv_wgrad_dma_batched_kernel<64, true, 3>), g, b, 0, s, tab, dev_begins, n); break;
    case 7: HDU_LAUNCH((conv_wgrad_dma_batched_kernel<64, true, 2>), g, b, 0, s, tab, dev_begins, n); break;
    case 8: HDU_LAUNCH((conv_wgrad_halo_batched_kernel<64>), g, b, 0, s, tab, dev_begins, n); break;
    case 9: HDU_LAUNCH((conv_wgrad_halo_batched_kernel<48>), g, b, 0, s, tab, dev_begins, n); break;
    case 10: HDU_LAUNCH((conv_wgrad_halo_batched_kernel<32>), g, b, 0, s, tab, dev_begins, n); break;
    default: return hdu_set_error(HDU_ERR_ARG, "wgrad_plan_run: unknown variant");
  }
  return hdu_check_launch("wgrad_plan_run");
}

extern "C" int hdu_conv_dgrad_strided(const hdu_conv_desc* d, void* stream) {
  ConvK k;
  if (int e = fill_convk(d, &k, false, true)) return e;
  if (d->ud | d->uh | d->uw) return hdu_set_error(HDU_ERR_ARG, "conv_dgrad_strided: upsampled input not supported");
  if (!d->x || !d->y) return hdu_set_error(HDU_ERR_ARG, "conv_dgrad_strided: null dx / dy");
  if (d->epi_a) return hdu_set_error(HDU_ERR_ARG, "conv_dgrad_strided: no output affine");
  const long long total = (long long)d->N * d->Di * d->Hi * d->Wi * (d->Cin / (d->dtype == HDU_BF16 ? 8 : 4));
  if (total == 0) return 0;
  long long blocks = (total + 255) / 256;
  if (blocks > 8192) blocks = 8192;
  if (d->dtype == HDU_BF16)
    HDU_LAUNCH((conv_dgrad_strided_kernel<bf16_t>), dim3((unsigned)blocks), dim3(256), 0, (hipStream_t)stream, k);
  else
    HDU_LAUNCH((conv_dgrad_strided_kernel<float>), dim3((unsigned)blocks), dim3(256), 0, (hipStream_t)stream, k);
  return hdu_check_launch("conv_dgrad_strided");
}

static int parity_table(int KD, int KH, int KW, int sd, int sh, int sw, int pd, int ph, int pw, int Cin, int Cout,
                        ParityTable* tab) {
  const int K[3] = {KD, KH, KW}, S[3] = {sd, sh, sw}, P[3] = {pd, ph, pw};
  for (int a = 0; a < 3; ++a)
    if (S[a] != 1 && S[a] != 2) return -1;
  tab->n = sd * sh * sw;
  long long off = 0;
  for (int c = 0; c < tab->n; ++c) {
    const int r[3] = {c / (sh * sw), (c / sw) % sh, c % sw};
    ParityGeom& g = tab->c[c];
    for (int a = 0; a < 3; ++a) {
      g.step[a] = S[a];
      int kmax = K[a] - 1;
      if (S[a] == 2 && ((kmax - r[a] - P[a]) & 1)) --kmax;
      g.kmax[a] = kmax;
      g.nt[a] = kmax < 0 ? 0 : kmax / S[a] + 1;
      if (g.nt[a] <= 0) return -1;
    }
    g.dst_off = off;
    off += (long long)Cin * g.nt[0] * g.nt[1] * g.nt[2] * Cout;
  }
  return 0;
}

extern "C" int hdu_stride2_dgrad_filters(int dtype, const float* w_master, int Cout, int KD, int KH, int KW, int Cin, int sd,
                                         int sh, int sw, int pd, int ph, int pw, void* w_out, void* stream) {
  ParityTable tab;
  if (!w_master || !w_out || Cout <= 0 || Cin <= 0 || parity_table(KD, KH, KW, sd, sh, sw, pd, ph, pw, Cin, Cout, &tab))
    return hdu_set_error(HDU_ERR_ARG, "stride2_dgrad_filters: bad args (strides must be 1 or 2)");
  const dim3 grid(64, (unsigned)tab.n);
  if (dtype == HDU_BF16)
    HDU_LAUNCH((stride2_filter_kernel<bf16_t>), grid, dim3(256), 0, (hipStream_t)stream, w_master, Cout, KD, KH, KW, Cin, tab, (bf16_t*)w_out);
  else if (dtype == HDU_F32)
    HDU_LAUNCH((stride2_filter_kernel<float>), grid, dim3(256), 0, (hipStream_t)stream, w_master, Cout, KD, KH, KW, Cin, tab, (float*)w_out);
  else
    return hdu_set_error(HDU_ERR_ARG, "stride2_dgrad_filters: bad dtype");
  return hdu_check_launch("stride2_dgrad_filters");
}

extern "C" int hdu_parity_interleave(int dtype, const void* cls, int N, int Di, int Hi, int Wi, int C, int sd, int sh, int sw,
                                     void* dx, int64_t lddx, int accumulate, void* stream) {
  const int ch = dtype == HDU_BF16 ? 8 : 4;
  if (!cls || !dx || N <= 0 || C <= 0 || C % ch || lddx % ch || Di % sd || Hi % sh || Wi % sw || (sd != 1 && sd != 2) ||
      (sh != 1 && sh != 2) || (sw != 1 && sw != 2))
    return hdu_set_error(HDU_ERR_ARG, "parity_interleave: bad args (dims must be multiples of the strides)");
  const long long total = (long long)N * Di * Hi * Wi * (C / ch);
  long long blocks = (total + 255) / 256;
  if (blocks > 8192) blocks = 8192;
  if (dtype == HDU_BF16)
    HDU_LAUNCH((parity_interleave_kernel<bf16_t>), dim3((unsigned)blocks), dim3(256), 0, (hipStream_t)stream, (const bf16_t*)cls,
               N, Di, Hi, Wi, C, sd, sh, sw, (bf16_t*)dx, (long long)lddx, accumulate);
  else if (dtype == HDU_F32)
    HDU_LAUNCH((parity_interleave_kernel<float>), dim3((unsigned)blocks), dim3(256), 0, (hipStream_t)stream, (const float*)cls, N,
               Di, Hi, Wi, C, sd, sh, sw, (float*)dx, (long long)lddx, accumulate);
  else
    return hdu_set_error(HDU_ERR_ARG, "parity_interleave: bad dtype");
  return hdu_check_launch("parity_interleave");
}

extern "C" int hdu_weight_prep(int dtype, const float* w_master, int Cout, int T, int Cin, void* w_f, void* w_d,
                               void* stream) {
  if (!w_master || Cout <= 0 || T <= 0 || Cin <= 0) return hdu_set_error(HDU_ERR_ARG, "weight_prep: bad args");
  const long long total = (long long)Cout * T * Cin;
  long long blocks = (total + 255) / 256;
  if (blocks > 2048) blocks = 2048;
  if (dtype == HDU_BF16)
    HDU_LAUNCH((weight_prep_kernel<bf16_t>), dim3((unsigned)blocks), dim3(256), 0, (hipStream_t)stream, w_master,
               Cout, T, Cin, (bf16_t*)w_f, (bf16_t*)w_d);
  else if (dtype == HDU_F32)
    HDU_LAUNCH((weight_prep_kernel<float>), dim3((unsigned)blocks), dim3(256), 0, (hipStream_t)stream, w_master,
               Cout, T, Cin, (float*)w_f, (float*)w_d);
  else
    return hdu_set_error(HDU_ERR_ARG, "weight_prep: bad dtype");
  return hdu_check_launch("weight_prep");
}

#include <cstdio>
extern "C" int hdu_conv_kernel_name(const hdu_conv_desc* d, int op, char* buf, size_t buflen) {
  ConvK k;
  if (int e = fill_convk(d, &k, op == 1)) return e;
  if (!buf || buflen < 8) return hdu_set_error(HDU_ERR_ARG, "conv_kernel_name: bad buffer");
  const char* t = d->dtype == HDU_BF16 ? "unsigned short" : "float";
  if (op == 1) {
    const bool dma = wgrad_dma_ok(k);
    const bool pw = k.KD * k.KH * k.KW == 1 && k.sd == 1 && k.sh == 1 && k.sw == 1 && (k.pd | k.ph | k.pw) == 0 &&
                    (k.ud | k.uh | k.uw) == 0;
    if (hdu_stem_wgrad_taken(k, d->dtype)) snprintf(buf, buflen, "conv_stem_wgrad_kernel");
    else if (d->dtype == HDU_BF16 && wgrad_halo_ok(k)) snprintf(buf, buflen, "conv_wgrad_halo_kernel<%d>", choose_wgrad(k));
    else if (d->dtype == HDU_BF16 && dma) snprintf(buf, buflen, "conv_wgrad_dma_kernel<%d, %s>", choose_wgrad(k), pw ? "true" : "false");
    else if (d->dtype == HDU_BF16) snprintf(buf, buflen, "conv_wgrad_tr_kernel<%d>", choose_wgrad(k));
    else snprintf(buf, buflen, "conv_wgrad_kernel<float, %d>", choose_wgrad(k));
  } else if (pw_bstat_ok(k, d->dtype)) {
    if (pw_bstat_form(k) == 2) snprintf(buf, buflen, "conv_pw_bstat_kernel<%d, 64, %s, 2>", k.Ktot / 64, k.bnb_u ? "true" : "false");
    else snprintf(buf, buflen, "conv_pw_bstat_kernel<%d, 128, %s, 3>", k.Ktot / 64, k.bnb_u ? "true" : "false");
  } else if (hdu_halo_wide_taken(k, d->dtype)) {
    snprintf(buf, buflen, "%s", hdu_halo_wide_name(k, d->dtype));
  } else if (fprop_halo_ok(k, d->dtype)) {
    snprintf(buf, buflen, "conv_halo_fprop_kernel<%d>", choose_halo_bn(k));
  } else {
    int bm, bn;
    choose_igemm(k, &bm, &bn);
    if (bm == 128 && igemm_pers_ok(k, bn)) {
      snprintf(buf, buflen, "conv_igemm_pers_kernel<%s, %d, %d>", t, bn, k.pro_a ? pers_table_cap(bn, k.Cin) : 0);
      return 0;
    }
    const int wm = (bn >= 128) ? 2 : ((bm == 64 && (bn == 64 || bn == 32)) ? 2 : 4);
    const bool prodma = igemm_pro_dma_ok(k);
    const bool dma = prodma || (k.pro_a == nullptr && k.skip == nullptr && k.vec_out);
    const long long nblk = ((k.M_layer + bm - 1) / bm) * ((k.Cout + bn - 1) / bn);
    const int mode = g_tuning[HDU_TUNE_DMA_STAGES];
    const int stage = (bm + ((bn + 31) / 32) * 32) * 128;
    const int nsd = stage * 6 <= 160 * 1024 ? 6 : 4;
    const bool ring = dma && igemm_ring_ok(nblk, k.Ktot, stage, nsd);
    int nsr = (nsd == 6 && ring_wgs_per_cu(bm, d->dtype == HDU_BF16) == 2) ? 3 : nsd;
    const int proc = prodma ? (k.Cin <= HDU_PRO_CSMALL ? HDU_PRO_CSMALL : HDU_PRO_CMAX) : 0;
    if (prodma && nsr * stage + 8 * proc > 160 * 1024) nsr = nsr == 6 ? 4 : 3;
    const char* fast = igemm_fast_ok(k) ? "true" : "false";
    const char* bnb = k.bnb_u != nullptr ? "true" : "false";
    if (ring) snprintf(buf, buflen, "conv_igemm_ring_kernel<%s, %d, %d, %d, %d, %d, %s, %s, %d>", t, bm, bn, wm, 4 / wm, nsr, fast, bnb, proc);
    else if (dma) snprintf(buf, buflen, "conv_igemm_dma_kernel<%s, %d, %d, %d, %d, %s, %s, %d>", t, bm, bn, wm, 4 / wm, fast, bnb, proc);
    else snprintf(buf, buflen, "conv_igemm_kernel<%s, %d, %d, %d, %d>", t, bm, bn, wm, 4 / wm);
  }
  return 0;
}

extern "C" int hdu_weight_prep_batched(int dtype, const hdu_prep_entry* table, int n, int64_t total_tiles,
                                       const float* master_base, void* wc_base, void* stream) {
  if (!table || n <= 0 || total_tiles <= 0 || !master_base || !wc_base)
    return hdu_set_error(HDU_ERR_ARG, "weight_prep_batched: bad args");
  if (dtype == HDU_BF16)
    HDU_LAUNCH((weight_prep_batched_kernel<bf16_t>), dim3((unsigned)((total_tiles + HDU_PREP_TPW - 1) / HDU_PREP_TPW)), dim3(256), 0,
               (hipStream_t)stream, table, n, master_base, (bf16_t*)wc_base, (long long)total_tiles);
  else if (dtype == HDU_F32)
    HDU_LAUNCH((weight_prep_batched_kernel<float>), dim3((unsigned)((total_tiles + HDU_PREP_TPW - 1) / HDU_PREP_TPW)), dim3(256), 0,
               (hipStream_t)stream, table, n, master_base, (float*)wc_base, (long long)total_tiles);
  else
    return hdu_set_error(HDU_ERR_ARG, "weight_prep_batched: bad dtype");
  return hdu_check_launch("weight_prep_batched");
}
```

h-denseunet_amd/csrc/hdu_host.h:

```cpp
#pragma once
#include "../../include/hdu.h"
#include "hdu_platform.h"

int hdu_set_error(int code, const char* msg);
int hdu_check_launch(const char* what);

static inline unsigned hdu_grid_1d(long long work_items, int per_block, unsigned cap) {
  long long b = (work_items + per_block - 1) / per_block;
  if (b < 1) b = 1;
  if (b > (long long)cap) b = cap;
  return (unsigned)b;
}

extern int g_tuning[32];
```

h-denseunet_amd/engine.py:

```python
import ctypes
import math
import os
from collections import OrderedDict

import numpy as np
import torch

from . import ops
from . import shard as _sh
from .lib import HDU_BF16, HDU_F32


class Param:
    __slots__ = ("layer", "idx", "kind", "keras_shape", "shape", "trainable", "init", "offset", "numel", "ctx", "meta")

    def __init__(self, ctx, layer, idx, kind, keras_shape, shape, trainable, init, meta=None):
        self.ctx, self.layer, self.idx, self.kind = ctx, layer, idx, kind
        self.keras_shape, self.shape, self.trainable, self.init = tuple(keras_shape), tuple(shape), trainable, init
        self.numel = int(np.prod(shape))
        self.offset = None
        self.meta = meta or {}

    @property
    def data(self):
# ... 628 lines not shown
                _sh.allreduce_sum(ctx.shard, self.s12)
                ops.bn_bwd_coef(self.C, x.M * ctx.shard.world, True, self.s12[:self.C], self.s12[self.C:],
                                self.gamma.data, self.beta.data, self.sg.data if self.sg else None, self.rstd, self.k1,
                                self.k2, self.k3)
        elif (need_sums and self.bsum is not None and xvar.root.needs_grad and ctx._zeroed_bwd_pass == ctx.pass_id
              and self._bsum_pass != ctx.pass_id):
            self._bsum_pass = ctx.pass_id
            acc = xvar.grad_mode()
            drop = xvar.root.drop if (ctx.dropout_enabled and ctx.learning_phase == 1) else None
            ops.bn_bwd_fused(dz_act, x, self.a, self.b, self.relu, self.mean_used, self.rstd, self.batch_now,
                             self.gamma.data, self.beta.data, self.sg.data if self.sg else None, self.bsum, self.BSUM_SLOTS,
                             self.gamma.grad if tr_bn else None, self.beta.grad if tr_bn else None,
                             self.sg.grad if tr_sc else None, self.sb.grad if tr_sc else None, xvar.grad, acc,
                             drop[0] if drop else 1.0, drop[1] if drop else 0, ctx.seed_dev if drop else None,
                             sums_ready=sums_ready)
            return
        elif need_sums:
            assert not sums_ready
            ops.bn_bwd_reduce_coef(dz_act, x, self.a, self.b, self.relu, self.mean_used, self.rstd, self.batch_now,
                                   self.gamma.data, self.beta.data, self.sg.data if self.sg else None, self.s1,
                                   self.s2, self.k1, self.k2, self.k3, self.gamma.grad if tr_bn else None,
                                   self.beta.grad if tr_bn else None, self.sg.grad if tr_sc else None,
                                   self.sb.grad if tr_sc else None, ctx.ws)
        else:
            ops.bn_bwd_coef(self.C, x.M, False, None, None, self.gamma.data, self.beta.data,
                            self.sg.data if self.sg else None, self.rstd, self.k1, self.k2, self.k3)
        if xvar.root.needs_grad:
            acc = xvar.grad_mode()
            drop = xvar.root.drop if (ctx.dropout_enabled and ctx.learning_phase == 1) else None
            ops.bn_bwd_apply(dz_act, x, self.a, self.b, self.relu, self.mean_used, self.k1, self.k2, self.k3,
                             xvar.grad, acc, drop[0] if drop else 1.0, drop[1] if drop else 0,
                             ctx.seed_dev if drop else None)


class ConvLayer:

    def __init__(self, ctx, name, x, filters, K, stride=(1, 1, 1), pad=(0, 0, 0), bn=None, up=(0, 0, 0), skip=None,
                 use_bias=True, out=None, init="glorot", trainable=True, dropout=0.0, keras_nd=2, cin_logical=None,
                 halo=0, producer=None):
        self.ctx, self.name, self.x, self.bn, self.up, self.skip = ctx, name, x, bn, up, skip
        self.K, self.stride = K, stride
        self.halo = halo
        if halo:
            assert not ctx.fuse_prologue, "halo mode materialises the conv input"
            assert skip is None or up == (0, 0, 0), "a skip add in halo mode must be at the stored resolution"
            pad = (pad[0] - (halo << up[0]), pad[1], pad[2])
        self.pad = pad
        self.trainable = trainable
        dt = ctx.dtype
        xa = x.act
        cin_p = xa.C
        cin = cin_logical or cin_p
        cout_p = ops.cpad(filters, dt)
        De, He, We = (xa.D + 2 * halo) << up[0], xa.H << up[1], xa.W << up[2]
        Do = (De + 2 * pad[0] - K[0]) // stride[0] + 1
        Ho = (He + 2 * pad[1] - K[1]) // stride[1] + 1
        Wo = (We + 2 * pad[2] - K[2]) // stride[2] + 1
        if out is None:
            out = ctx.new_var(xa.N, Do, Ho, Wo, cout_p)
        else:
            assert (out.act.N, out.act.D, out.act.H, out.act.W, out.act.C) == (xa.N, Do, Ho, Wo, cout_p)
        self.out = out
        kshape = ((K[1], K[2]) if keras_nd == 2 else (K[1], K[2], K[0])) + (cin, filters)
        self.kernel = ctx.add_param(name, "conv_kernel", 0, kshape, (cout_p, K[0], K[1], K[2], cin_p), trainable, init)
        self.bias = ctx.add_param(name, "conv_bias", 1, (filters,), (cout_p,), trainable, "zeros") if use_bias else None
        ctx.layer_kind[name] = "conv"
        self.T = K[0] * K[1] * K[2]
        self.cin_p, self.cout_p = cin_p, cout_p
        self.dropout = dropout
        if dropout > 0:
            ctx.drop_layers += 1
            self.drop_seed = 7919 * ctx.drop_layers
            out.root.drop = (1.0 - dropout, self.drop_seed)
        need_input_grad = x.root.needs_grad
        if ctx.grad_enabled:
            out.require_grad()
        self.xin = None
        self.conv_up = up
        self.pw_fused = bool(ctx.fuse_pw and bn is not None and skip is None and not halo and K == (1, 1, 1)
                             and stride == (1, 1, 1) and pad == (0, 0, 0) and up == (0, 0, 0) and cin_p <= ops.PRO_CMAX)
        if self.pw_fused:
            pass
        elif halo:
            self.xin = ctx.new_var(xa.N, xa.D + 2 * halo, xa.H, xa.W, cin_p)
            plane = xa.H * xa.W * cin_p
            self.xin_interior = ops.Act(self.xin.act.buf, halo * plane, xa.N, xa.D, xa.H, xa.W, cin_p, cin_p, dt)
            self._halo_tmp = ctx.scratch("halo_tmp", 1, 2 * halo, xa.H, xa.W, cin_p)
        elif (bn is not None or skip is not None) and not ctx.fuse_prologue:
            if skip is not None:
                self.xin = ctx.new_var(xa.N, De, He, We, cin_p)
                self.conv_up = (0, 0, 0)
            else:
                self.xin = ctx.new_var(xa.N, xa.D, xa.H, xa.W, cin_p)
        st = getattr(bn, "stats_src", None) if bn is not None else None
        if (st is not None and self.xin is not None and not halo and st.producer is not None and st.absorber is None
                and x.root is st.var.root and bn.C == x.C and x.c0 == (0 if bn is st.fold_next else st.var.c0)):
            st.absorber = self
        self.need_input_grad = need_input_grad
        self.epi_consumer = None
        self.epi_producer = None
        if (producer is not None and ctx.fuse_bn_epilogue and bn is not None and self.xin is not None and not halo
                and skip is None and up == (0, 0, 0) and x is producer.out and x.root is x and producer.epi_consumer is None):
            self.epi_producer = producer
            producer.epi_consumer = self
        self.strided = stride != (1, 1, 1)
        pw_stream = bool(ctx.fuse_bn_bwd_pw and dt == HDU_BF16 and K == (1, 1, 1) and pad == (0, 0, 0) and cout_p in (128, 192)
                         and cin_p >= 256 and xa.M >= 64)
        self.bnb_fused = bool(ctx.fuse_bn_bwd and need_input_grad and bn is not None and up == (0, 0, 0) and skip is None
                              and not halo and stride == (1, 1, 1) and not ctx.fuse_prologue and x.root.drop is None
                              and (ctx.fuse_bn_bwd_mode >= 2 or bn.mode != "batch" or pw_stream))
        self.bnb_off = None
        self._sums_kernel_ok = None
        self._s2 = None
        self._s2_ok = (os.environ.get("HDU_STRIDE2_DGRAD", "1") == "1" and all(v in (1, 2) for v in stride)
                       and xa.D % stride[0] == 0 and xa.H % stride[1] == 0 and xa.W % stride[2] == 0 and up == (0, 0, 0)
                       and bn is None and skip is None and not halo)
        self.need_dgrad_filter = need_input_grad and not self.strided
        self.wf_off = self.wd_off = None
        ctx.convs.append(self)
        if bn is not None:
            ctx.need_ws(xa.M, xa.C)
        ctx.need_ws(out.act.M, cout_p)
        if need_input_grad:
            if bn is not None or up != (0, 0, 0) or halo:
                self._dxe = ctx.scratch("dxe", xa.N, De, He, We, cin_p)
            if (bn is not None or halo) and up != (0, 0, 0):
                self._dz = ctx.scratch("dz", xa.N, xa.D + 2 * halo, xa.H, xa.W, cin_p)
        ctx.fwd.append(self.forward)
        ctx.bwd.append(self.backward)

    def bind(self):
        ctx = self.ctx
        esz = ctx.Wc.element_size()
        if ctx.dtype == HDU_F32:
            self.wf_ptr = ctypes.c_void_p(self.kernel.data.data_ptr())
        else:
            self.wf_ptr = ctypes.c_void_p(ctx.Wc.data_ptr() + self.wf_off * esz)
        self.wd_ptr = ctypes.c_void_p(ctx.Wc.data_ptr() + self.wd_off * esz) if self.need_dgrad_filter else None
        x, out = self.x.act, self.out.act
        pro = (self.bn.a, self.bn.b) if self.bn is not None else None
        relu = self.bn.relu if self.bn is not None else False
        skip = self.skip.act if self.skip is not None else None
        up = self.up
        if self.xin is not None:
            x, pro, relu, skip, up = self.xin.act, None, False, None, self.conv_up
        bias = self.bias.data if self.bias is not None else None
        if self.strided and self.need_input_grad and self._s2_ok and self.out.root.needs_grad:
            xa = self.x.act
            self._s2 = ops.Stride2Dgrad(ctx.dtype, self.kernel.data, self.out.grad, (xa.N, xa.D, xa.H, xa.W), xa.C, self.K,
                                        self.stride, self.pad, shard_world=ctx.shard_world())
        self.d_f = ctx.conv_desc(x, self.wf_ptr, out, self.K, self.stride, self.pad, up, skip, pro, relu, bias)
        self.d_f_drop = None
        if self.dropout > 0:
            self.d_f_drop = ctx.conv_desc(x, self.wf_ptr, out, self.K, self.stride, self.pad, up, skip, pro, relu,
                                          bias, False, 1.0 - self.dropout, self.drop_seed, ctx.seed_dev)
        self.d_f_epi = self.d_f_drop_epi = None
        cons = self.epi_consumer
        if cons is not None:
            epi = (cons.bn.a, cons.bn.b, cons.bn.relu)
            self.d_f_epi = ctx.conv_desc(x, self.wf_ptr, cons.xin.act, self.K, self.stride, self.pad, up, skip, pro, relu, bias,
                                         epi=epi)
            if self.dropout > 0:
                self.d_f_drop_epi = ctx.conv_desc(x, self.wf_ptr, cons.xin.act, self.K, self.stride, self.pad, up, skip, pro,
                                                  relu, bias, False, 1.0 - self.dropout, self.drop_seed, ctx.seed_dev, epi=epi)
        self.d_f_st = self.d_f_drop_st = None
        sink = getattr(self, "stats_sink", None)
        if sink is not None:
            shift = sink.var.stats_shift()
            part = ctypes.c_void_p(ctx.stats_acc.data_ptr() + 4 * sink.acc_off)

            def with_stats(d):
                if d is None:
                    return None
                c = type(d)()
                ctypes.memmove(ctypes.byref(c), ctypes.byref(d), ctypes.sizeof(d))
                c.stats_partial, c.stats_shift, c.stats_slots = part, ctypes.c_void_p(shift.data_ptr()), sink.SLOTS
                return c
            self.d_f_st, self.d_f_drop_st = with_stats(self.d_f), with_stats(self.d_f_drop)

    def prep(self):
        ctx = self.ctx
        if ctx.dtype == HDU_F32 and not self.need_dgrad_filter:
            return
        wf = None if ctx.dtype == HDU_F32 else ctx.Wc[self.wf_off:self.wf_off + self.kernel.numel]
        wd = ctx.Wc[self.wd_off:self.wd_off + self.kernel.numel] if self.need_dgrad_filter else None
        ops.weight_prep(ctx.dtype, self.kernel.data, self.cout_p, self.T, self.cin_p, wf, wd)

    def epi_active(self):
        ctx, bn = self.ctx, self.bn
        if self.epi_producer is None or (bn.mode == "batch" and ctx.learning_phase == 1):
            return False
        if ctx.learning_phase == 0 or not (self.need_input_grad or bn.any_trainable()):
            return True
        return ctx.fuse_bn_epilogue_train and self.bnb_fused and self.need_input_grad and ctx.bnb_fusable()

    def forward(self):
        ctx = self.ctx
        if self.epi_producer is not None and self.epi_active():
            return self._forward_conv()
        if self.bn is not None:
            self.bn.fold(self.x)
        if self.xin is not None:
            bn = self.bn
            up = self.up if self.skip is not None else (0, 0, 0)
            skip = self.skip.act if self.skip is not None else None
            dst = self.xin_interior if self.halo else self.xin.act
            pend = bn.pending_stats if bn is not None else None
            if pend is not None and pend[0] == ctx.pass_id and pend[1].absorber is self:
                ops.materialize_stats(self.x.act, pend[1].stats_block(bn), bn.relu, up, skip, dst)
            else:
                ops.materialize(self.x.act, bn.a if bn else None, bn.b if bn else None, bn.relu if bn else False, up, skip, dst)
            if self.halo:
                _sh.halo_exchange(ctx.shard, self.xin.act, self.halo)
        self._forward_conv()

    def _forward_conv(self):
        ctx = self.ctx
        cons = self.epi_consumer
        if cons is not None and cons.epi_active():
            cons.bn.fold(self.out)
            drop = self.d_f_drop_epi is not None and ctx.learning_phase == 1 and ctx.dropout_enabled
            ops.conv_fprop(self.d_f_drop_epi if drop else self.d_f_epi)
            return
        st = ctx.learning_phase == 1 and self.d_f_st is not None and self.stats_sink.primed
        if self.d_f_drop is not None and ctx.learning_phase == 1 and ctx.dropout_enabled:
            ops.conv_fprop(self.d_f_drop_st if st else self.d_f_drop)
        else:
            ops.conv_fprop(self.d_f_st if st else self.d_f)

    def backward(self):
        ctx = self.ctx
        out = self.out
        if not out.root.needs_grad:
            return
        dy = out.dy()
        x = self.x.act
        if self.trainable and (getattr(self, "in_plan", False) or (ctx._split_now and getattr(self, "in_split_plan", False))):
            if self.bias is not None:
                ops.colsum(dy, self.bias.grad, ctx.ws)
        elif self.trainable:
            if self.xin is not None:
                d = ctx.conv_desc(self.xin.act, self.wf_ptr, dy, self.K, self.stride, self.pad, self.conv_up)
            else:
                d = ctx.conv_desc(x, self.wf_ptr, dy, self.K, self.stride, self.pad, self.up,
                                  self.skip.act if self.skip is not None else None,
                                  (self.bn.a, self.bn.b) if self.bn is not None else None,
                                  self.bn.relu if self.bn is not None else False)
            ops.conv_wgrad(d, self.kernel.grad)
            if self.bias is not None:
                ops.colsum(dy, self.bias.grad, ctx.ws)
        if not self.need_input_grad:
            return
        K, pad = self.K, self.pad
        if self.halo:
            return self._backward_halo(dy)
        if self.bnb_fused and ctx.fuse_bn_bwd_now:
            return self._backward_fused_bn(dy)
        De, He, We = x.D << self.up[0], x.H << self.up[1], x.W << self.up[2]
        direct = self.bn is None and self.up == (0, 0, 0)
        sums_ready = False
        skip_first = self.skip is not None and self.skip.root.needs_grad and not self.skip.root.written \
            and self.skip.c0 == 0
        if direct:
            tgt, acc = self.x.grad, self.x.grad_mode()
        elif skip_first:
            tgt, acc = self.skip.grad, self.skip.grad_mode()
        else:
            tgt, acc = self._dxe(), False
        if self.strided:
            tgt_act = ops.Act(tgt.buf, tgt.off, x.N, x.D, x.H, x.W, x.C, tgt.ld, tgt.dtype)
            if self._s2 is not None:
                self._s2.run(tgt_act, accumulate=acc)
            else:
                d = ctx.conv_desc(tgt_act, self.wf_ptr, dy, K, self.stride, pad, accumulate=acc)
                ops.conv_dgrad_strided(d)
        else:
            d = ctx.conv_desc(dy, self.wd_ptr, ops.Act(tgt.buf, tgt.off, x.N, De, He, We, x.C, tgt.ld, tgt.dtype), K,
                              (1, 1, 1), (K[0] - 1 - pad[0], K[1] - 1 - pad[1], K[2] - 1 - pad[2]), accumulate=acc)
            sums_ready = self._epilogue_sums(d)
            ops.conv_fprop(d)
        if self.skip is not None and self.skip.root.needs_grad and not skip_first:
            ops.upsample_bwd(tgt, self.skip.grad, (0, 0, 0), accumulate=self.skip.grad_mode())
        if direct:
            return
        dz = tgt
        if self.up != (0, 0, 0):
            if self.bn is None:
                ops.upsample_bwd(tgt, self.x.grad, self.up, accumulate=self.x.grad_mode())
                return
            dz = self._dz()
            ops.upsample_bwd(tgt, dz, self.up)
        if self.bn is not None:
            self.bn.backward(self.x, dz, sums_ready=sums_ready)
        else:
            ops.upsample_bwd(dz, self.x.grad, (0, 0, 0), accumulate=self.x.grad_mode())

    def _epilogue_sums(self, d):
        ctx, bn = self.ctx, self.bn
        if not (ctx.bnb_sums_epilogue and bn is not None and self.up == (0, 0, 0) and self.skip is None and not self.halo
                and self.x.root.drop is None and ctx.bnb_fusable() and bn.BSUM_SLOTS <= 32):
            return False
        if self._sums_kernel_ok is None:
            name = ops.conv_kernel_name(d, 0)
            self._sums_kernel_ok = name.startswith("conv_igemm_ring_kernel") or name.startswith("conv_igemm_dma_kernel")
        if not self._sums_kernel_ok or not bn.takes_epilogue_sums(self.x):
            return False
        x = self.x.act
        d.bnb_u, d.bnb_ldu = x.ptr, x.ld
        d.bnb_a, d.bnb_b = bn.a.data_ptr(), bn.b.data_ptr()
        d.bnb_relu = (1 if bn.relu else 0) | 4
        d.bnb_mean, d.bnb_rstd = bn.mean_used.data_ptr(), bn.rstd.data_ptr()
        d.bnb_partial, d.bnb_slots = bn.bsum.data_ptr(), bn.BSUM_SLOTS
        return True


def _conv_backward_fused_bn(self, dy):
    ctx, bn, xv = self.ctx, self.bn, self.x
    x = xv.act
    K, pad = self.K, self.pad
    acc = xv.grad_mode()
    tgt = xv.grad
    d = ctx.conv_desc(dy, self.wd_ptr, ops.Act(tgt.buf, tgt.off, x.N, x.D, x.H, x.W, x.C, tgt.ld, tgt.dtype), K, (1, 1, 1),
                      (K[0] - 1 - pad[0], K[1] - 1 - pad[1], K[2] - 1 - pad[2]), accumulate=acc)
    d.bnb_u, d.bnb_ldu = x.ptr, x.ld
    d.bnb_a, d.bnb_b, d.bnb_relu = bn.a.data_ptr(), bn.b.data_ptr(), 1 if bn.relu else 0
    if self.epi_producer is not None and self.epi_active():
        d.bnb_u, d.bnb_ldu = self.xin.act.ptr, self.xin.act.ld
        d.bnb_relu |= 2
    need_sums = bn.batch_now or bn.any_trainable()
    part = None
    if need_sums:
        n = self.BNB_SLOTS * 2 * bn.C
        part = ctx.bnb_acc[self.bnb_off:self.bnb_off + n]
        d.bnb_mean, d.bnb_rstd = bn.mean_used.data_ptr(), bn.rstd.data_ptr()
        d.bnb_partial, d.bnb_slots = part.data_ptr(), self.BNB_SLOTS
    ops.conv_fprop(d)
    if need_sums:
        tr_bn = bn.trainable
        tr_sc = bn.sg is not None and bn.scale_trainable
        c3 = c4 = None
        if bn.batch_now:
            r = xv.root
            ld = r.act.ld
            base = r.corr_off + xv.c0
            c3, c4 = ctx.corr_acc[base:base + bn.C], ctx.corr_acc[base + ld:base + ld + bn.C]
        if not bn.batch_now and ctx.batch_wgrad and ctx.defer_bnb_finalize:
            ctx._bnb_deferred.append((id(self), (part, self.BNB_SLOTS, bn.C, bn.gamma.data, bn.beta.data,
                                                 bn.sg.data if bn.sg else None, bn.gamma.grad if tr_bn else None,
                                                 bn.beta.grad if tr_bn else None, bn.sg.grad if tr_sc else None,
                                                 bn.sb.grad if tr_sc else None)))
            return
        fin_args = (part, self.BNB_SLOTS, x.M, bn.C, bn.gamma.data, bn.beta.data, bn.sg.data if bn.sg else None, bn.mean_used, bn.rstd,
                    bn.gamma.grad if tr_bn else None, bn.beta.grad if tr_bn else None,
                    bn.sg.grad if tr_sc else None, bn.sb.grad if tr_sc else None, c3, c4)
        if bn.batch_now and ctx.merge_fin_correct and self.BNB_SLOTS <= 32 and bn.C % 4 == 0:
            ctx.flush_pending_finalize()
            ctx._pending_fin = dict(root=xv.root, c0=xv.c0, C=bn.C, M=x.M, args=fin_args)
            return
        ops.bn_bwd_finalize(part, self.BNB_SLOTS, x.M, bn.C, bn.batch_now, bn.gamma.data, bn.beta.data,
                            bn.sg.data if bn.sg else None, bn.mean_used, bn.rstd,
                            bn.gamma.grad if tr_bn else None, bn.beta.grad if tr_bn else None,
                            bn.sg.grad if tr_sc else None, bn.sb.grad if tr_sc else None, c3, c4)


ConvLayer._backward_fused_bn = _conv_backward_fused_bn
ConvLayer.BNB_SLOTS = int(os.environ.get("HDU_BNB_SLOTS", "16"))


def _conv_backward_halo(self, dy):
    ctx = self.ctx
    x = self.x.act
    K, pad, h = self.K, self.pad, self.halo
    De, He, We = (x.D + 2 * h) << self.up[0], x.H << self.up[1], x.W << self.up[2]
    tgt = self._dxe()
    if self.strided:
        d = ctx.conv_desc(ops.Act(tgt.buf, tgt.off, x.N, De, He, We, x.C, tgt.ld, tgt.dtype), self.wf_ptr, dy, K,
                          self.stride, pad)
        ops.conv_dgrad_strided(d)
    else:
        d = ctx.conv_desc(dy, self.wd_ptr, ops.Act(tgt.buf, tgt.off, x.N, De, He, We, x.C, tgt.ld, tgt.dtype), K, (1, 1, 1),
                          (K[0] - 1 - pad[0], K[1] - 1 - pad[1], K[2] - 1 - pad[2]), halo_out=(2 * h) << self.up[0])
        ops.conv_fprop(d)
    dz = tgt
    if self.up != (0, 0, 0):
        dz = self._dz()
        ops.upsample_bwd(tgt, dz, self.up)
    _sh.halo_reduce(ctx.shard, dz, h, self._halo_tmp().buf)
    plane = x.H * x.W * dz.ld
    interior = ops.Act(dz.buf, dz.off + h * plane, x.N, x.D, x.H, x.W, x.C, dz.ld, dz.dtype)
    if self.skip is not None and self.skip.root.needs_grad:
        ops.upsample_bwd(interior, self.skip.grad, (0, 0, 0), accumulate=self.skip.grad_mode())
    if self.bn is not None:
        self.bn.backward(self.x, interior)
    else:
        ops.upsample_bwd(interior, self.x.grad, (0, 0, 0), accumulate=self.x.grad_mode())


ConvLayer._backward_halo = _conv_backward_halo


class StatsOp:

    SLOTS = int(os.environ.get("HDU_STATS_SLOTS", "32"))

    def __init__(self, ctx, var):
        self.ctx, self.var = ctx, var
        self.fused = None
        self.fold_next = None
        self.absorber = None
        world = ctx.shard.world if ctx.shard is not None else 1
        self.sync_buf = ctx.fvec(world * (1 + 2 * var.C)) if world > 1 else None
        ctx.need_ws(var.act.M, var.C)
        var.stats()
        self.producer = None
        prod = ctx.convs[-1] if ctx.convs else None
        sharded = ctx.shard is not None and ctx.shard.world > 1
        if (ctx.epilogue_stats and not sharded and prod is not None and ctx.fwd and ctx.fwd[-1] == prod.forward
                and prod.out.root is var.root and prod.out.c0 == var.c0 and prod.out.C == var.C
                and getattr(prod, "stats_sink", None) is None):
            self.producer = prod
            prod.stats_sink = self
            self.acc_off = None
            self.primed = False
            ctx.stats_sinks.append(self)
        ctx.fwd.append(self.forward)

    def fuse(self, bn):
        assert bn.C == self.var.C and bn.mode == "batch"
        self.fused = bn
        bn.stats_src = self
        return self

    def then_fold(self, bn):
        if self.fused is None and bn.mode == "batch" and self.ctx.fold_next and bn.C == self.var.c0 + self.var.C:
            self.fold_next = bn
            bn.stats_src = self
        return self

    def stats_block(self, bn):
        ctx = self.ctx
        n = self.SLOTS * 2 * self.var.C
        fold = (bn.gamma.data, bn.beta.data, bn.eps, bn.sg.data if bn.sg else None, bn.sb.data if bn.sb else None,
                bn.a, bn.b, bn.rstd, bn.mm.data, bn.mv.data, bn.momentum)
        part = ctx.stats_acc[self.acc_off:self.acc_off + n]
        if bn is self.fused:
            mean, var = self.var.stats()
            return (part, self.SLOTS, self.var.act.M, self.var.C, 0, self.var.stats_shift(), mean, var, fold)
        r = self.var.root
        return (part, self.SLOTS, self.var.act.M, self.var.C, self.var.c0, r.shift[:bn.C], r.mean[:bn.C], r.var[:bn.C], fold)

    def forward(self):
        ctx = self.ctx
        if ctx.learning_phase != 1:
            return
        mean, var = self.var.stats()
        bn = self.fused
        if ctx.shard is not None and ctx.shard.world > 1:
            ops.bn_stats(self.var.act, mean, var, ctx.ws)
            _sh.sync_stats(ctx.shard, mean, var, self.var.act.M, self.sync_buf)
            return
        fold = None
        if bn is not None:
            fold = (bn.gamma.data, bn.beta.data, bn.eps, bn.sg.data if bn.sg else None, bn.sb.data if bn.sb else None,
                    bn.a, bn.b, bn.rstd, bn.mm.data, bn.mv.data, bn.momentum)
        if self.producer is not None and not self.primed:
            self.primed = True
            if bn is None:
                ops.bn_stats(self.var.act, mean, var, ctx.ws)
                return
            ops.bn_stats_fold(self.var.act, mean, var, *fold, ctx.ws)
        elif self.producer is not None:
            n = self.SLOTS * 2 * self.var.C
            nb = self.fold_next
            tgt = nb if nb is not None else bn
            if tgt is not None and self.absorber is not None and ctx.absorb_stats:
                tgt.batch_now = True
                tgt.mean_used = self.var.root.mean[:tgt.C] if nb is not None else mean
                tgt.folded_pass = ctx.pass_id
                tgt.pending_stats = (ctx.pass_id, self)
                return
            if nb is not None:
                r = self.var.root
                f2 = (nb.gamma.data, nb.beta.data, nb.eps, nb.sg.data if nb.sg else None, nb.sb.data if nb.sb else None,
                      nb.a, nb.b, nb.rstd, nb.mm.data, nb.mv.data, nb.momentum)
                ops.bn_stats_finalize_fold_next(ctx.stats_acc[self.acc_off:self.acc_off + n], self.SLOTS, self.var.act.M,
                                                self.var.C, self.var.c0, nb.C, r.shift[:nb.C], r.mean[:nb.C], r.var[:nb.C], f2)
                nb.batch_now = True
                nb.mean_used = r.mean[:nb.C]
                nb.folded_pass = ctx.pass_id
                return
            ops.bn_stats_finalize(ctx.stats_acc[self.acc_off:self.acc_off + n], self.SLOTS, self.var.act.M, self.var.C,
                                  self.var.stats_shift(), mean, var, fold)
        elif bn is None:
            ops.bn_stats(self.var.act, mean, var, ctx.ws)
            return
        else:
            ops.bn_stats_fold(self.var.act, mean, var, *fold, ctx.ws)
        if bn is not None:
            bn.mean_used = mean
            bn.folded_pass = ctx.pass_id


class MaterializeLayer:

    def __init__(self, ctx, x, bn, halo=0):
        self.ctx, self.x, self.bn, self.halo = ctx, x, bn, halo
        a = x.act
        self.out = ctx.new_var(a.N, a.D + 2 * halo, a.H, a.W, a.C)
        if ctx.grad_enabled:
            self.out.require_grad()
        if halo:
            self._halo_tmp = ctx.scratch("halo_tmp", 1, 2 * halo, a.H, a.W, a.C)
        ctx.need_ws(a.M, a.C)
        ctx.fwd.append(self.forward)
        ctx.bwd.append(self.backward)

    def _interior(self, act):
        a, h = self.x.act, self.halo
        return ops.Act(act.buf, act.off + h * a.H * a.W * act.ld, a.N, a.D, a.H, a.W, a.C, act.ld, act.dtype)

    def forward(self):
        self.bn.fold(self.x)
        if self.halo:
            ops.affine_act(self.x.act, self.bn.a, self.bn.b, self.bn.relu, self._interior(self.out.act))
            _sh.halo_exchange(self.ctx.shard, self.out.act, self.halo)
        else:
            ops.affine_act(self.x.act, self.bn.a, self.bn.b, self.bn.relu, self.out.act)

    def backward(self):
        if not self.out.root.needs_grad:
            return
        if self.halo:
            _sh.halo_reduce(self.ctx.shard, self.out.grad, self.halo, self._halo_tmp().buf)
            self.bn.backward(self.x, self._interior(self.out.grad))
        else:
            self.bn.backward(self.x, self.out.dy())


class MaxPoolLayer:

    def __init__(self, ctx, x, out=None, pad_d=1):
        self.ctx, self.x, self.pad_d = ctx, x, pad_d
        a = x.act
        Do = 1 if a.D == 1 else (a.D + 2 * pad_d - 3) // 2 + 1
        dims = (a.N, Do, (a.H - 1) // 2 + 1, (a.W - 1) // 2 + 1)
        self.out = out if out is not None else ctx.new_var(*dims, a.C)
        assert (self.out.act.N, self.out.act.D, self.out.act.H, self.out.act.W) == dims
        if ctx.grad_enabled:
            self.out.require_grad()
        oa = self.out.act
        self.argmax = torch.zeros(oa.M * a.C, dtype=torch.uint8, device=ctx.dev) if self.x.root.needs_grad else None
        ctx.fwd.append(lambda: ops.maxpool_fwd(self.x.act, self.out.act, self.argmax, self.pad_d))
        ctx.bwd.append(self.backward)

    def backward(self):
        if self.out.root.needs_grad and self.x.root.needs_grad:
            ops.maxpool_bwd(self.argmax, self.out.dy(), self.x.grad, self.x.grad_mode(), self.pad_d)


class AvgPoolLayer:

    def __init__(self, ctx, x, out):
        self.ctx, self.x, self.out = ctx, x, out
        if ctx.grad_enabled:
            out.require_grad()
        ctx.fwd.append(lambda: ops.avgpool_fwd(self.x.act, self.out.act))
        ctx.bwd.append(self.backward)

    def backward(self):
        if self.out.root.needs_grad and self.x.root.needs_grad:
            ops.avgpool_bwd(self.out.dy(), self.x.grad, self.x.grad_mode())


class LossLayer:

    def __init__(self, ctx, logits, ranges, weights=(0.78, 0.65, 8.57)):
        self.ctx, self.logits, self.ranges, self.weights = ctx, logits, ranges, weights
        self.count = sum(m for _, m in ranges)
        self.labels = torch.zeros(logits.act.M, dtype=torch.uint8, device=ctx.dev)
        self.loss_sum = torch.zeros(1, dtype=torch.float32, device=ctx.dev)
        self.class_count = torch.zeros(3, dtype=torch.float32, device=ctx.dev)
        self.global_scale = 1.0
        ctx.loss_layers.append(self)
        ctx.need_ws(1 << 14, 8)

    def set_labels(self, lab_u8_internal):
        lab = np.asarray(lab_u8_internal).reshape(-1)
        if lab.size != self.labels.numel():
            raise ValueError("labels: expected %d entries, got %d" % (self.labels.numel(), lab.size))
        if int(lab.max()) > 2 or int(lab.min()) < 0:
            raise ValueError("labels must be in {0,1,2} (loss.py:14-21)")
        self.labels.copy_(torch.from_numpy(lab.astype(np.uint8)).to(self.ctx.dev))

    def run(self, with_grad=True):
        if self.ctx._zeroed_fwd_pass != self.ctx.pass_id:
            i = self.ctx.loss_layers.index(self)
            ops.zero_tensor(self.ctx.arena[4 * i:4 * i + 4])
        dl = None
        if with_grad:
            self.logits.root.written = True
            dl = self.logits.grad
        gs = self.global_scale / float(self.count)
        for row0, m in self.ranges:
            ops.wce_loss(self.logits.act, self.labels, row0, m, self.weights, gs, dl, self.loss_sum, self.class_count,
                         self.ctx.ws)

    def value(self):
# ... 2 lines not shown
```

h-denseunet_amd/lib.py:

```python
import ctypes
import os

_HERE = os.path.dirname(os.path.abspath(__file__))
_ROOT = os.path.dirname(_HERE)

HDU_BF16 = 0
HDU_F32 = 1

c_int, c_i64, c_f, c_p, c_u32, c_sz = (ctypes.c_int, ctypes.c_int64, ctypes.c_float, ctypes.c_void_p,
                                       ctypes.c_uint32, ctypes.c_size_t)


class ConvDesc(ctypes.Structure):
    _fields_ = [
        ("dtype", c_int),
        ("x", c_p), ("ldx", c_i64),
        ("N", c_int), ("Di", c_int), ("Hi", c_int), ("Wi", c_int), ("Cin", c_int),
        ("ud", c_int), ("uh", c_int), ("uw", c_int),
        ("skip", c_p), ("ldskip", c_i64),
        ("pro_a", c_p), ("pro_b", c_p), ("pro_relu", c_int),
        ("w", c_p),
        ("KD", c_int), ("KH", c_int), ("KW", c_int),
        ("sd", c_int), ("sh", c_int), ("sw", c_int),
        ("pd", c_int), ("ph", c_int), ("pw", c_int),
        ("y", c_p), ("ldy", c_i64),
        ("Do", c_int), ("Ho", c_int), ("Wo", c_int), ("Cout", c_int),
        ("bias", c_p),
        ("epi_a", c_p), ("epi_b", c_p), ("epi_relu", c_int),
        ("accumulate", c_int),
        ("drop_keep", c_f),
        ("drop_seed", c_u32),
        ("drop_seed_dev", c_p),
        ("stats_partial", c_p),
        ("stats_shift", c_p),
        ("stats_slots", c_int),
        ("bnb_u", c_p), ("bnb_ldu", c_i64),
        ("bnb_a", c_p), ("bnb_b", c_p), ("bnb_mean", c_p), ("bnb_rstd", c_p),
        ("bnb_relu", c_int),
        ("bnb_partial", c_p), ("bnb_slots", c_int),
        ("splitk_ws", c_p),
        ("splitk_ws_bytes", c_sz),
        ("splitk_counters", c_p),
        ("layer_rows", ctypes.c_int64),
    ]


class PrepEntry(ctypes.Structure):
    _fields_ = [("master_off", c_i64), ("w_f_off", c_i64), ("w_d_off", c_i64), ("tile_begin", c_i64),
                ("Cout", ctypes.c_int32), ("T", ctypes.c_int32), ("Cin", ctypes.c_int32), ("pad_", ctypes.c_int32)]


class AugSample(ctypes.Structure):
    _fields_ = [("img_off", c_i64), ("vrows", ctypes.c_int32), ("vcols", ctypes.c_int32), ("vslices", ctypes.c_int32),
                ("a0", ctypes.c_int32), ("b0", ctypes.c_int32), ("c0", ctypes.c_int32), ("crop", ctypes.c_int32),
                ("flip", ctypes.c_int32)]


class ZeroEntry(ctypes.Structure):
    _fields_ = [("ptr", c_p), ("bytes", ctypes.c_uint64), ("block_begin", ctypes.c_uint32), ("pad_", ctypes.c_uint32),
                ("src", c_p)]


class BnBwdEntry(ctypes.Structure):
    _fields_ = [("partial", c_p), ("slots", ctypes.c_int32), ("C", ctypes.c_int32), ("gamma", c_p), ("beta", c_p),
                ("sgamma", c_p), ("dgamma", c_p), ("dbeta", c_p), ("dsgamma", c_p), ("dsbeta", c_p)]


class BnStatsFold(ctypes.Structure):
    _fields_ = [("partial", c_p), ("slots", ctypes.c_int32), ("Cseg", ctypes.c_int32), ("seg_c0", ctypes.c_int32),
                ("pad_", ctypes.c_int32), ("M", c_i64), ("shift", c_p), ("mean", c_p), ("var", c_p), ("gamma", c_p),
                ("beta", c_p), ("sgamma", c_p), ("sbeta", c_p), ("eps", c_f), ("momentum", c_f), ("a", c_p), ("b", c_p),
                ("rstd", c_p), ("mov_mean", c_p), ("mov_var", c_p)]


ZERO_BLOCK_BYTES = 65536


class Split3Entry(ctypes.Structure):
    _fields_ = [("src", c_p), ("dst", c_p), ("a", c_p), ("b", c_p), ("ld_src", ctypes.c_uint64), ("rows", ctypes.c_uint64),
                ("C", ctypes.c_uint32), ("relu", ctypes.c_uint32), ("pattern", ctypes.c_uint32), ("cols", ctypes.c_uint32),
                ("col_groups", ctypes.c_uint32), ("block_begin", ctypes.c_uint32), ("iters", ctypes.c_uint32),
                ("chl", ctypes.c_uint32)]


SPLIT3_OPERAND, SPLIT3_GRADIENT = 0, 1


class FoldEntry(ctypes.Structure):
    _fields_ = [("mean", c_p), ("var", c_p), ("gamma", c_p), ("beta", c_p), ("sgamma", c_p), ("sbeta", c_p),
                ("a", c_p), ("b", c_p), ("rstd", c_p), ("C", ctypes.c_int32), ("eps", c_f)]


_SIGS = {
    "hdu_last_error": (ctypes.c_char_p, []),
    "hdu_backend": (ctypes.c_char_p, []),
    "hdu_abi_version": (c_int, []),
    "hdu_sizeof_conv_desc": (c_sz, []),
    "hdu_set_tuning": (c_int, [c_int, c_int]),
    "hdu_conv_fprop": (c_int, [ctypes.POINTER(ConvDesc), c_p]),
    "hdu_bn_bwd_finalize": (c_int, [c_p, c_int, c_i64, c_int, c_int, c_p, c_p, c_p, c_p, c_p, c_p, c_p, c_p, c_p, c_p, c_p, c_p]),
    "hdu_bn_bwd_correct": (c_int, [c_int, c_p, c_i64, c_i64, c_int, c_p, c_p, c_p, c_i64, c_p]),
    "hdu_bn_bwd_finalize_correct": (c_int, [c_int, c_p, c_int, c_i64, c_int, c_p, c_p, c_p, c_p, c_p, c_p, c_p, c_p, c_p, c_p, c_p,
                                            c_int, c_int, c_p, c_i64, c_p, c_i64, c_p]),
    "hdu_conv_splitk_ws_bytes": (c_sz, [ctypes.POINTER(ConvDesc)]),
    "hdu_conv_wgrad": (c_int, [ctypes.POINTER(ConvDesc), c_p, c_p]),
    "hdu_conv_dgrad_strided": (c_int, [ctypes.POINTER(ConvDesc), c_p]),
    "hdu_stride2_dgrad_filters": (c_int, [c_int, c_p, c_int, c_int, c_int, c_int, c_int, c_int, c_int, c_int, c_int, c_int,
                                          c_int, c_p, c_p]),
    "hdu_parity_interleave": (c_int, [c_int, c_p, c_int, c_int, c_int, c_int, c_int, c_int, c_int, c_int, c_p, c_i64, c_int,
                                      c_p]),
    "hdu_conv_kernel_name": (c_int, [ctypes.POINTER(ConvDesc), c_int, ctypes.c_char_p, c_sz]),
    "hdu_weight_prep": (c_int, [c_int, c_p, c_int, c_int, c_int, c_p, c_p, c_p]),
    "hdu_weight_prep_batched": (c_int, [c_int, c_p, c_int, c_i64, c_p, c_p, c_p]),
    "hdu_reduce_ws_bytes": (c_sz, [c_i64, c_int]),
    "hdu_bn_stats": (c_int, [c_int, c_p, c_i64, c_i64, c_int, c_p, c_p, c_p, c_sz, c_p]),
    "hdu_bn_fold": (c_int, [c_int, c_p, c_p, c_p, c_p, c_f, c_p, c_p, c_p, c_p, c_p, c_p, c_p, c_f, c_p]),
    "hdu_augment_batch": (c_int, [c_p, c_p, c_p, c_int, c_int, c_int, c_int, c_f, c_p, c_p, c_i64, c_i64, c_i64, c_p, c_i64,
                                  c_i64, c_p]),
    "hdu_bn_fold_batched": (c_int, [c_p, c_p, c_int, ctypes.c_uint32, c_p]),
    "hdu_bn_stats_fold": (c_int, [c_int, c_p, c_i64, c_i64, c_int, c_p, c_p, c_p, c_p, c_f, c_p, c_p, c_p, c_p, c_p, c_p,
                                  c_p, c_f, c_p, c_sz, c_p]),
    "hdu_bn_bwd_reduce_coef": (c_int, [c_int, c_p, c_i64, c_p, c_i64, c_i64, c_int, c_p, c_p, c_int, c_p, c_p, c_int,
                                       c_p, c_p, c_p, c_p, c_p, c_p, c_p, c_p, c_p, c_p, c_p, c_p, c_p, c_sz, c_p]),
    "hdu_bn_bwd_reduce": (c_int, [c_int, c_p, c_i64, c_p, c_i64, c_i64, c_int, c_p, c_p, c_int, c_p, c_p, c_p, c_p,
                                  c_p, c_sz, c_p]),
    "hdu_bn_bwd_coef": (c_int, [c_int, c_i64, c_int, c_p, c_p, c_p, c_p, c_p, c_p, c_p, c_p, c_p, c_p, c_p, c_p,
                                c_p, c_p]),
    "hdu_bn_bwd_apply": (c_int, [c_int, c_p, c_i64, c_p, c_i64, c_i64, c_int, c_p, c_p, c_int, c_p, c_p, c_p, c_p,
                                 c_p, c_i64, c_int, c_f, c_u32, c_p, c_p]),
    "hdu_bn_bwd_fused": (c_int, [c_int, c_p, c_i64, c_p, c_i64, c_i64, c_int, c_p, c_p, c_int, c_p, c_p, c_int, c_p, c_p,
                                 c_p, c_p, c_int, c_p, c_p, c_p, c_p, c_p, c_i64, c_int, c_f, c_u32, c_p, c_p]),
    "hdu_bn_bwd_apply_sums": (c_int, [c_int, c_p, c_i64, c_p, c_i64, c_i64, c_int, c_p, c_p, c_int, c_p, c_p, c_int, c_p, c_p,
                                      c_p, c_p, c_int, c_p, c_p, c_p, c_p, c_p, c_i64, c_int, c_f, c_u32, c_p, c_p]),
    "hdu_affine_act": (c_int, [c_int, c_p, c_i64, c_i64, c_int, c_p, c_p, c_int, c_p, c_i64, c_p]),
    "hdu_materialize": (c_int, [c_int, c_p, c_i64, c_int, c_int, c_int, c_int, c_int, c_p, c_p, c_int, c_int, c_int, c_int,
                                c_p, c_i64, c_p, c_i64, c_p]),
    "hdu_bn_bwd_finalize_batched": (c_int, [c_p, c_p, c_int, c_u32, c_p]),
    "hdu_materialize_stats": (c_int, [c_int, c_p, c_i64, c_int, c_int, c_int, c_int, c_int, c_p, c_int, c_int, c_int, c_int,
                                      c_p, c_i64, c_p, c_i64, c_p]),
    "hdu_wgrad_plan_entry_bytes": (c_sz, []),
    "hdu_wgrad_plan_fill": (c_int, [ctypes.POINTER(ConvDesc), c_p, c_int, c_int, c_p, ctypes.POINTER(c_int), ctypes.POINTER(ctypes.c_uint32)]),
    "hdu_wgrad_plan_shape": (c_int, [ctypes.POINTER(ConvDesc), ctypes.POINTER(c_int), ctypes.POINTER(ctypes.c_uint32),
                                     ctypes.POINTER(ctypes.c_uint32)]),
    "hdu_wgrad_plan_run": (c_int, [c_int, c_p, c_p, c_int, ctypes.c_uint32, c_p]),
    "hdu_bn_stats_finalize_fold_next": (c_int, [c_p, c_int, c_i64, c_int, c_int, c_int, c_p, c_p, c_p, c_p, c_p, c_f, c_p, c_p,
                                                c_p, c_p, c_p, c_p, c_p, c_f, c_p]),
    "hdu_bn_stats_finalize": (c_int, [c_p, c_int, c_i64, c_int, c_p, c_p, c_p, c_p, c_p, c_f, c_p, c_p, c_p, c_p, c_p, c_p, c_p,
                                      c_f, c_p]),
    "hdu_stats_sync_floats": (c_sz, [c_int, c_int]),
    "hdu_stats_pack": (c_int, [c_int, c_p, c_p, c_i64, c_int, c_int, c_p, c_p]),
    "hdu_stats_unpack": (c_int, [c_int, c_p, c_int, c_p, c_p, c_p]),
    "hdu_colsum": (c_int, [c_int, c_p, c_i64, c_i64, c_int, c_p, c_p, c_sz, c_p]),
    "hdu_maxpool3s2_fwd": (c_int, [c_int, c_p, c_i64, c_int, c_int, c_int, c_int, c_int, c_p, c_i64, c_p, c_int, c_p]),
    "hdu_maxpool3s2_bwd": (c_int, [c_int, c_p, c_p, c_i64, c_int, c_int, c_int, c_int, c_int, c_p, c_i64, c_int, c_int, c_p]),
    "hdu_avgpool2_fwd": (c_int, [c_int, c_p, c_i64, c_int, c_int, c_int, c_int, c_int, c_p, c_i64, c_p]),
    "hdu_avgpool2_bwd": (c_int, [c_int, c_p, c_i64, c_int, c_int, c_int, c_int, c_int, c_p, c_i64, c_int, c_p]),
    "hdu_upsample_bwd": (c_int, [c_int, c_p, c_i64, c_int, c_int, c_int, c_int, c_int, c_int, c_int, c_int, c_p,
                                 c_i64, c_int, c_p]),
    "hdu_wce_loss": (c_int, [c_int, c_p, c_i64, c_p, c_i64, c_f, c_f, c_f, c_f, c_p, c_i64, c_int, c_p, c_p, c_p,
                             c_sz, c_p]),
    "hdu_sgd_nesterov": (c_int, [c_p, c_p, c_p, c_i64, c_f, c_f, c_f, c_p]),
    "hdu_slab25d": (c_int, [c_int, c_p, c_int, c_int, c_int, c_p, c_int, c_p]),
    "hdu_make_input3d": (c_int, [c_int, c_p, c_p, c_i64, c_f, c_int, c_int, c_int, c_p, c_int, c_p]),
    "hdu_make_input3d_bwd": (c_int, [c_int, c_p, c_int, c_f, c_i64, c_p, c_i64, c_int, c_int, c_p]),
    "hdu_cast_pad": (c_int, [c_int, c_p, c_i64, c_int, c_p, c_i64, c_int, c_p]),
    "hdu_cast_out": (c_int, [c_int, c_p, c_i64, c_i64, c_int, c_p, c_p]),
    "hdu_softmax_accumulate": (c_int, [c_int, c_p, c_i64, c_i64, c_int, c_p, c_p]),
    "hdu_pp_threshold": (c_int, [c_p, c_p, c_int, c_int, c_int, c_int, c_int, c_int, ctypes.c_double, ctypes.c_double, c_p, c_p, c_p]),
    "hdu_pp_dilate": (c_int, [c_p, c_int, c_int, c_int, c_p, c_p]),
    "hdu_pp_label": (c_int, [c_p, c_int, c_int, c_int, c_int, c_int, c_p, c_p]),
    "hdu_pp_largest": (c_int, [c_p, c_int, c_int, c_int, c_p, c_p, c_p, c_p, c_p]),
    "hdu_pp_fill_holes": (c_int, [c_p, c_int, c_int, c_int, c_p, c_p, c_p, c_p]),
    "hdu_pp_bbox": (c_int, [c_p, c_int, c_int, c_int, c_p, c_p]),
    "hdu_pp_merge": (c_int, [c_int, c_p, c_p, c_i64, c_p, c_p]),
    "hdu_zero_regions": (c_int, [c_p, c_int, c_u32, c_p, c_u32, c_p]),
    "hdu_zero": (c_int, [c_p, ctypes.c_uint64, c_p]),
    "hdu_split3_entry_fill": (c_int, [c_p, c_p, c_i64, c_i64, c_int, c_p, c_p, c_int, c_int, c_p, c_u32, ctypes.POINTER(c_u32)]),
    "hdu_split3_batched": (c_int, [c_p, c_int, c_u32, c_int, c_p]),
    "hdu_profile_begin": (c_int, [c_int]),
    "hdu_profile_count": (c_int, []),
    "hdu_profile_end": (c_int, []),
    "hdu_profile_get": (c_int, [c_int, ctypes.c_char_p, c_sz, ctypes.POINTER(c_f)]),
    "hdu_comm_unique_id": (c_int, [c_p]),
    "hdu_comm_init": (c_int, [ctypes.POINTER(c_p), c_int, c_int, c_p]),
    "hdu_comm_destroy": (c_int, [c_p]),
    "hdu_comm_allreduce_f32": (c_int, [c_p, c_p, c_i64, c_p]),
    "hdu_comm_sendrecv": (c_int, [c_p, c_int, c_p, c_p, c_int, c_p, c_p, c_sz, c_p]),
}

EXPORTS = tuple(_SIGS.keys())

_lib = None
_backend = None


class HduError(RuntimeError):
    pass


ABI_VERSION = 8


def product_library_path():
    return os.path.join(_HERE, "libhdu.so")


def _bind(path):
    import torch
    lib = ctypes.CDLL(path)
    for name, (res, args) in _SIGS.items():
        fn = getattr(lib, name)
        fn.restype = res
        fn.argtypes = args
    if lib.hdu_abi_version() != ABI_VERSION or lib.hdu_sizeof_conv_desc() != ctypes.sizeof(ConvDesc):
        raise HduError("%s has ABI version %d / hdu_conv_desc of %d bytes, this binding expects %d / %d -- rebuild it "
                       "(python -c 'import __graft_entry__ as g; g.build()')" %
                       (path, lib.hdu_abi_version(), lib.hdu_sizeof_conv_desc(), ABI_VERSION, ctypes.sizeof(ConvDesc)))
    return lib


def _apply_env_tuning(lib):
    if "HDU_DMA_STAGES" in os.environ:
        lib.hdu_set_tuning(0, int(os.environ["HDU_DMA_STAGES"]))
    if "HDU_SPLITK" in os.environ:
        lib.hdu_set_tuning(13, int(os.environ["HDU_SPLITK"]))
    if "HDU_BM64_MAX_M" in os.environ:
        lib.hdu_set_tuning(18, int(os.environ["HDU_BM64_MAX_M"]))
    if "HDU_SPLITK_TARGET" in os.environ:
        lib.hdu_set_tuning(16, int(os.environ["HDU_SPLITK_TARGET"]))
    if "HDU_SPLITK_MIN_STEPS" in os.environ:
        lib.hdu_set_tuning(17, int(os.environ["HDU_SPLITK_MIN_STEPS"]))
    if "HDU_HALO_MIN_TILES" in os.environ:
        lib.hdu_set_tuning(15, int(os.environ["HDU_HALO_MIN_TILES"]))
    if "HDU_RING_MIN_K" in os.environ:
        lib.hdu_set_tuning(14, int(os.environ["HDU_RING_MIN_K"]))
    if "HDU_RED_WGS" in os.environ:
        lib.hdu_set_tuning(11, int(os.environ["HDU_RED_WGS"]))
    if "HDU_ROW_WGS" in os.environ:
        lib.hdu_set_tuning(12, int(os.environ["HDU_ROW_WGS"]))
    if "HDU_NO_HALO_FPROP" in os.environ:
        lib.hdu_set_tuning(9, int(os.environ["HDU_NO_HALO_FPROP"]))
    if "HDU_NO_HALO" in os.environ:
        lib.hdu_set_tuning(8, int(os.environ["HDU_NO_HALO"]))
    if "HDU_HALO_WIDE" in os.environ:
        lib.hdu_set_tuning(29, int(os.environ["HDU_HALO_WIDE"]))
    if "HDU_HALO_MIN_W" in os.environ:
        lib.hdu_set_tuning(28, int(os.environ["HDU_HALO_MIN_W"]))
    if "HDU_HALO_TARGET" in os.environ:
        lib.hdu_set_tuning(7, int(os.environ["HDU_HALO_TARGET"]))
    if "HDU_MAX_BN" in os.environ:
        lib.hdu_set_tuning(6, int(os.environ["HDU_MAX_BN"]))
    if "HDU_NO_FAST" in os.environ:
        lib.hdu_set_tuning(5, int(os.environ["HDU_NO_FAST"]))
    if "HDU_DEBUG_FLAGS" in os.environ:
        lib.hdu_set_tuning(4, int(os.environ["HDU_DEBUG_FLAGS"]))
    if "HDU_XCD_SWIZZLE" in os.environ:
        lib.hdu_set_tuning(3, int(os.environ["HDU_XCD_SWIZZLE"]))
    if "HDU_WGRAD_TARGET" in os.environ:
        lib.hdu_set_tuning(2, int(os.environ["HDU_WGRAD_TARGET"]))
    if "HDU_NO_PW_BSTAT" in os.environ:
        lib.hdu_set_tuning(19, int(os.environ["HDU_NO_PW_BSTAT"]))
    if "HDU_PW_BSTAT_WGS" in os.environ:
        lib.hdu_set_tuning(20, int(os.environ["HDU_PW_BSTAT_WGS"]))
    if "HDU_PW_BSTAT_FORM" in os.environ:
        lib.hdu_set_tuning(30, int(os.environ["HDU_PW_BSTAT_FORM"]))
    if "HDU_SPLIT3_FORM" in os.environ:
        lib.hdu_set_tuning(31, int(os.environ["HDU_SPLIT3_FORM"]))
    if "HDU_WGRAD_NCT" in os.environ:
        lib.hdu_set_tuning(21, int(os.environ["HDU_WGRAD_NCT"]))
    if "HDU_NO_PRO_DMA" in os.environ:
        lib.hdu_set_tuning(22, int(os.environ["HDU_NO_PRO_DMA"]))
    if "HDU_PERS" in os.environ:
        lib.hdu_set_tuning(23, int(os.environ["HDU_PERS"]))
    if "HDU_NO_PW_BSTAT_BNB" in os.environ:
        lib.hdu_set_tuning(26, int(os.environ["HDU_NO_PW_BSTAT_BNB"]))
    lib.hdu_set_tuning(TUNE_F32_SPLIT, _F32_MODES[_f32_contraction])
    if "HDU_PERS_MIN_ITEMS" in os.environ:
        lib.hdu_set_tuning(24, int(os.environ["HDU_PERS_MIN_ITEMS"]))
    if "HDU_WGRAD_MIN_STEPS" in os.environ:
        lib.hdu_set_tuning(1, int(os.environ["HDU_WGRAD_MIN_STEPS"]))


def load(path=None):
    global _lib, _backend
    path = path or product_library_path()
    if not os.path.exists(path):
        raise HduError(
            "libhdu.so not found at %s -- run `python -c 'import __graft_entry__ as g; g.build()'` "
            "(hipcc --offload-arch=gfx950).  There is no CPU fallback." % path)
    bound = _bind(path)
    backend = bound.hdu_backend().decode()
    if backend != "hip-gfx950":
        raise HduError("%s is not the gfx950 product library (hdu_backend() = %r).  There is no CPU fallback." % (path, backend))
    _lib, _backend = bound, backend
    _apply_env_tuning(_lib)
    return _lib


class _CallLog:

    def __init__(self, lib):
        self._lib, self.calls = lib, []

    def __getattr__(self, name):
        fn = getattr(self._lib, name)
        if not name.startswith("hdu_") or name.startswith("hdu_profile") or name in ("hdu_last_error", "hdu_conv_kernel_name"):
            return fn
        lib, calls = self._lib, self.calls

        def wrapped(*args):
            n0 = lib.hdu_profile_count()
            r = fn(*args)
            n1 = lib.hdu_profile_count()
            if n1 > n0:
                calls.append((name, args, n0, n1))
            return r
        return wrapped


_call_log = None

TUNE_F32_SPLIT = 27


def set_f32_contraction(mode):
    global _f32_contraction
    prev = _f32_contraction
    check(get().hdu_set_tuning(TUNE_F32_SPLIT, _F32_MODES[_check_f32_mode(mode)]), "hdu_set_tuning")
    _f32_contraction = mode
    return prev


_F32_MODES = {"exact": 0, "bf16x3": 1, "bf16x3_bwd": 0}


def f32_split_in_backward_only():
    return _f32_contraction == "bf16x3_bwd"


def f32_contraction():
    return _f32_contraction


def set_f32_split_now(on):
    check(get().hdu_set_tuning(TUNE_F32_SPLIT, 1 if on else 0), "hdu_set_tuning")


def _check_f32_mode(mode, what="f32 contraction mode"):
    if mode not in _F32_MODES:
        raise ValueError("%s: 'exact', 'bf16x3' or 'bf16x3_bwd', not %r" % (what, mode))
    return mode


_f32_contraction = _check_f32_mode(os.environ.get("HDU_F32_CONTRACTION", "exact"), "HDU_F32_CONTRACTION")


def profile_begin(max_records=1 << 16):
    global _call_log
    lib = get() if _call_log is None else _call_log._lib
    check(lib.hdu_profile_begin(max_records), "hdu_profile_begin")
    _call_log = _CallLog(lib)


def profile_end():
    global _call_log
    log, _call_log = _call_log, None
    lib = log._lib
    n = lib.hdu_profile_end()
    if n < 0:
        raise HduError("hdu_profile_end failed: %s" % lib.hdu_last_error().decode())
    buf = ctypes.create_string_buffer(256)
    ms = c_f(0.0)
    recs = []
    for i in range(n):
        check(lib.hdu_profile_get(i, buf, 256, ctypes.byref(ms)), "hdu_profile_get")
        recs.append((buf.value.decode(), float(ms.value)))
    return recs, log.calls


def get():
    if _call_log is not None:
        return _call_log
    if _lib is None:
        load()
    return _lib


def backend():
    get()
    return _backend


def is_emulator():
    return backend() == "emu-x86"


def check(code, what=""):
    if code != 0:
        raise HduError("%s failed (%d): %s" % (what or "hdu call", code, get().hdu_last_error().decode()))
```

include/hdu.h:

```cpp
#ifndef HDU_H_
#define HDU_H_

#include <stddef.h>
#include <stdint.h>

#ifdef __cplusplus
extern "C" {
#endif

#define HDU_BF16 0
#define HDU_F32 1

#define HDU_OK 0
#define HDU_ERR_ARG (-1)
#define HDU_ERR_LAUNCH (-2)
#define HDU_ERR_WORKSPACE (-3)

const char* hdu_last_error(void);
const char* hdu_backend(void);
#define HDU_ABI_VERSION 8
int hdu_abi_version(void);
size_t hdu_sizeof_conv_desc(void);
int hdu_profile_begin(int max_records);
int hdu_profile_count(void);
int hdu_profile_end(void);
int hdu_profile_get(int i, char* name_buf, size_t buflen, float* ms);
#define HDU_TUNE_DMA_STAGES 0
#define HDU_TUNE_HALO_TARGET_WGS 7
#define HDU_TUNE_MAX_BN 6
#define HDU_TUNE_NO_FAST 5
#define HDU_TUNE_DEBUG 4
#define HDU_TUNE_XCD_SWIZZLE 3
#define HDU_TUNE_RED_WGS 11
#define HDU_TUNE_ROW_WGS 12
#define HDU_TUNE_NO_HALO_FPROP 9
#define HDU_TUNE_NO_HALO 8
#define HDU_TUNE_WGRAD_TARGET_WGS 2
#define HDU_TUNE_SPLITK 13
#define HDU_TUNE_BM64_MAX_M 18
#define HDU_TUNE_SPLITK_TARGET 16
#define HDU_TUNE_SPLITK_MIN_STEPS 17
#define HDU_TUNE_HALO_MIN_TILES 15
#define HDU_TUNE_RING_MIN_K 14
#define HDU_TUNE_WGRAD_MIN_STEPS 1
#define HDU_TUNE_NO_PW_BSTAT 19
#define HDU_TUNE_PW_BSTAT_WGS 20
#define HDU_TUNE_PW_BSTAT_FORM 30
#define HDU_TUNE_NO_PRO_DMA 22
#define HDU_TUNE_PERS 23
#define HDU_TUNE_NO_PW_BSTAT_BNB 26
#define HDU_TUNE_PERS_MIN_ITEMS 24
#define HDU_TUNE_HALO_MIN_W 28
#define HDU_TUNE_F32_SPLIT 27
#define HDU_TUNE_HALO_WIDE 29
#define HDU_TUNE_SPLIT3_FORM 31
#define HDU_TUNE_WGRAD_NCT 21
int hdu_set_tuning(int key, int value);

typedef struct hdu_conv_desc {
  int dtype;
  const void* x;      int64_t ldx;
  int N, Di, Hi, Wi, Cin;
  int ud, uh, uw;
  const void* skip;   int64_t ldskip;
  const float* pro_a; const float* pro_b; int pro_relu;
  const void* w;
  int KD, KH, KW;
  int sd, sh, sw;
  int pd, ph, pw;
  void* y;            int64_t ldy;
  int Do, Ho, Wo, Cout;
  const float* bias;
  const float* epi_a; const float* epi_b; int epi_relu;
  int accumulate;
  float drop_keep;
  uint32_t drop_seed;
  const uint32_t* drop_seed_dev;
  float* stats_partial;
  const float* stats_shift;
  int stats_slots;
  const void* bnb_u;  int64_t bnb_ldu;
  const float* bnb_a; const float* bnb_b; const float* bnb_mean; const float* bnb_rstd;
  int bnb_relu;
  float* bnb_partial; int bnb_slots;
  void* splitk_ws;
  size_t splitk_ws_bytes;
  uint32_t* splitk_counters;
  int64_t layer_rows;
} hdu_conv_desc;

int hdu_bn_bwd_finalize(const float* partial, int slots, int64_t M, int C, int batch_stats, const float* gamma,
                        const float* beta, const float* sgamma, const float* mean, const float* rstd, float* dgamma,
                        float* dbeta, float* dsgamma, float* dsbeta, float* corr3, float* corr4, void* stream);

typedef struct hdu_bnbwd_entry {
  const float* partial;
  int32_t slots, C;
  const float* gamma; const float* beta; const float* sgamma;
  float* dgamma; float* dbeta; float* dsgamma; float* dsbeta;
} hdu_bnbwd_entry;
int hdu_bn_bwd_finalize_batched(const hdu_bnbwd_entry* table, const uint32_t* begins, int n, uint32_t total_blocks, void* stream);

int hdu_bn_bwd_correct(int dtype, const void* u, int64_t ldu, int64_t M, int C, const float* corr3, const float* corr4,
                       void* du, int64_t lddu, void* stream);
int hdu_bn_bwd_finalize_correct(int dtype, const float* partial, int slots, int64_t M, int C, const float* gamma, const float* beta,
                                const float* sgamma, const float* mean, const float* rstd, float* dgamma, float* dbeta,
                                float* dsgamma, float* dsbeta, float* corr3, float* corr4, int cs0, int Cc, const void* u,
                                int64_t ldu, void* du, int64_t lddu, void* stream);

size_t hdu_conv_splitk_ws_bytes(const hdu_conv_desc* d);

int hdu_conv_fprop(const hdu_conv_desc* d, void* stream);

int hdu_conv_wgrad(const hdu_conv_desc* d, float* dw, void* stream);

size_t hdu_wgrad_plan_entry_bytes(void);
int hdu_wgrad_plan_fill(const hdu_conv_desc* d, float* dw, int target_wgs, int min_steps, void* entry, int* variant,
                        uint32_t* nblocks);
int hdu_wgrad_plan_shape(const hdu_conv_desc* d, int* variant, uint32_t* tiles, uint32_t* steps);
int hdu_wgrad_plan_run(int variant, const void* dev_entries, const uint32_t* dev_begins, int n, uint32_t total_blocks,
                       void* stream);

int hdu_conv_dgrad_strided(const hdu_conv_desc* d, void* stream);

int hdu_stride2_dgrad_filters(int dtype, const float* w_master, int Cout, int KD, int KH, int KW, int Cin, int sd, int sh,
                              int sw, int pd, int ph, int pw, void* w_out, void* stream);
int hdu_parity_interleave(int dtype, const void* cls, int N, int Di, int Hi, int Wi, int C, int sd, int sh, int sw, void* dx,
                          int64_t lddx, int accumulate, void* stream);

int hdu_conv_kernel_name(const hdu_conv_desc* d, int op, char* buf, size_t buflen);

int hdu_weight_prep(int dtype, const float* w_master, int Cout, int T, int Cin, void* w_f, void* w_d, void* stream);

#define HDU_PREP_TILE 64
typedef struct hdu_prep_entry {
  int64_t master_off, w_f_off, w_d_off, tile_begin;
  int32_t Cout, T, Cin, pad_;
} hdu_prep_entry;
int hdu_weight_prep_batched(int dtype, const hdu_prep_entry* table, int n, int64_t total_tiles,
                            const float* master_base, void* wc_base, void* stream);

typedef struct hdu_aug_sample {
  int64_t img_off;
  int32_t vrows, vcols, vslices;
  int32_t a0, b0, c0;
  int32_t crop, flip;
} hdu_aug_sample;
int hdu_augment_batch(const float* img, const uint8_t* lab, const hdu_aug_sample* samples, int n, int size, int nslices,
                      int lab_slice, float mean, float* minmax_ws, float* x_out, int64_t x_sample, int64_t x_pix,
                      int64_t x_slice, uint8_t* y_out, int64_t y_sample, int64_t y_slice, void* stream);

size_t hdu_reduce_ws_bytes(int64_t M, int C);

typedef struct hdu_fold_entry {
  const float* mean; const float* var; const float* gamma; const float* beta; const float* sgamma; const float* sbeta;
  float* a; float* b; float* rstd;
  int32_t C; float eps;
} hdu_fold_entry;
int hdu_bn_fold_batched(const hdu_fold_entry* table, const uint32_t* begins, int n, uint32_t total_blocks, void* stream);

int hdu_bn_stats(int dtype, const void* x, int64_t ldx, int64_t M, int C, float* mean, float* var, void* ws,
                 size_t ws_bytes, void* stream);

int hdu_bn_fold(int C, const float* mean, const float* var, const float* gamma, const float* beta, float eps,
                const float* sgamma, const float* sbeta, float* a, float* b, float* rstd, float* mov_mean,
                float* mov_var, float momentum, void* stream);

int hdu_bn_stats_fold(int dtype, const void* x, int64_t ldx, int64_t M, int C, float* mean, float* var,
                      const float* gamma, const float* beta, float eps, const float* sgamma, const float* sbeta,
                      float* a, float* b, float* rstd, float* mov_mean, float* mov_var, float momentum, void* ws,
                      size_t ws_bytes, void* stream);

int hdu_bn_bwd_reduce_coef(int dtype, const void* dz, int64_t lddz, const void* x, int64_t ldx, int64_t M, int C,
                           const float* a, const float* b, int relu, const float* mean, const float* rstd,
                           int batch_stats, const float* gamma, const float* beta, const float* sgamma, float* s1,
                           float* s2, float* k1, float* k2, float* k3, float* dgamma, float* dbeta, float* dsgamma,
                           float* dsbeta, void* ws, size_t ws_bytes, void* stream);

int hdu_bn_bwd_reduce(int dtype, const void* dz, int64_t lddz, const void* x, int64_t ldx, int64_t M, int C,
                      const float* a, const float* b, int relu, const float* mean, const float* rstd, float* s1,
                      float* s2, void* ws, size_t ws_bytes, void* stream);

int hdu_bn_bwd_coef(int C, int64_t M, int batch_stats, const float* s1, const float* s2, const float* gamma,
                    const float* beta, const float* sgamma, const float* rstd, float* k1, float* k2, float* k3,
                    float* dgamma, float* dbeta, float* dsgamma, float* dsbeta, void* stream);

int hdu_bn_bwd_apply(int dtype, const void* dz, int64_t lddz, const void* x, int64_t ldx, int64_t M, int C,
                     const float* a, const float* b, int relu, const float* mean, const float* k1,
                     const float* k2, const float* k3, void* dx, int64_t lddx, int accumulate, float drop_keep,
                     uint32_t drop_seed, const uint32_t* drop_seed_dev, void* stream);

int hdu_bn_bwd_fused(int dtype, const void* dz, int64_t lddz, const void* x, int64_t ldx, int64_t M, int C, const float* a,
                     const float* b, int relu, const float* mean, const float* rstd, int batch_stats, const float* gamma,
                     const float* beta, const float* sgamma, float* sums, int slots, float* dgamma, float* dbeta,
                     float* dsgamma, float* dsbeta, void* dx, int64_t lddx, int accumulate, float drop_keep,
                     uint32_t drop_seed, const uint32_t* drop_seed_dev, void* stream);

int hdu_bn_bwd_apply_sums(int dtype, const void* dz, int64_t lddz, const void* x, int64_t ldx, int64_t M, int C, const float* a,
                          const float* b, int relu, const float* mean, const float* rstd, int batch_stats, const float* gamma,
                          const float* beta, const float* sgamma, float* sums, int slots, float* dgamma, float* dbeta,
                          float* dsgamma, float* dsbeta, void* dx, int64_t lddx, int accumulate, float drop_keep,
                          uint32_t drop_seed, const uint32_t* drop_seed_dev, void* stream);

int hdu_affine_act(int dtype, const void* x, int64_t ldx, int64_t M, int C, const float* a, const float* b,
                   int relu, void* z, int64_t ldz, void* stream);

int hdu_materialize(int dtype, const void* x, int64_t ldx, int N, int D, int H, int W, int C, const float* a,
                    const float* b, int relu, int ud, int uh, int uw, const void* skip, int64_t ldskip, void* out,
                    int64_t ldout, void* stream);

int hdu_bn_stats_finalize(const float* partial, int slots, int64_t M, int C, const float* shift, float* mean, float* var,
                          const float* gamma, const float* beta, float eps, const float* sgamma, const float* sbeta,
                          float* a, float* b, float* rstd, float* mov_mean, float* mov_var, float momentum, void* stream);

int hdu_bn_stats_finalize_fold_next(const float* partial, int slots, int64_t M, int Cseg, int seg_c0, int C_all,
                                    const float* shift_all, float* mean_all, float* var_all, const float* gamma,
                                    const float* beta, float eps, const float* sgamma, const float* sbeta, float* a, float* b,
                                    float* rstd, float* mov_mean, float* mov_var, float momentum, void* stream);

typedef struct hdu_stats_fold_desc {
  const float* partial;
  int32_t slots, Cseg, seg_c0, pad_;
  int64_t M;
  const float* shift;
  float* mean;
  float* var;
  const float* gamma; const float* beta; const float* sgamma; const float* sbeta;
  float eps, momentum;
  float* a; float* b; float* rstd; float* mov_mean; float* mov_var;
} hdu_stats_fold_desc;
int hdu_materialize_stats(int dtype, const void* x, int64_t ldx, int N, int D, int H, int W, int C, const hdu_stats_fold_desc* f,
                          int relu, int ud, int uh, int uw, const void* skip, int64_t ldskip, void* out, int64_t ldout,
                          void* stream);

size_t hdu_stats_sync_floats(int C, int world);
int hdu_stats_pack(int C, const float* mean, const float* var, int64_t n_local, int rank, int world, float* buf, void* stream);
int hdu_stats_unpack(int C, const float* buf, int world, float* mean, float* var, void* stream);

int hdu_colsum(int dtype, const void* x, int64_t ldx, int64_t M, int C, float* out, void* ws, size_t ws_bytes,
               void* stream);

int hdu_maxpool3s2_fwd(int dtype, const void* x, int64_t ldx, int N, int D, int H, int W, int C, void* y,
                       int64_t ldy, uint8_t* argmax ,
                       int pad_d ,
                       void* stream);
int hdu_maxpool3s2_bwd(int dtype, const uint8_t* argmax, const void* dy, int64_t lddy, int N, int D, int H, int W,
                       int C, void* dx, int64_t lddx, int accumulate, int pad_d, void* stream);
int hdu_avgpool2_fwd(int dtype, const void* x, int64_t ldx, int N, int D, int H, int W, int C, void* y,
                     int64_t ldy, void* stream);
int hdu_avgpool2_bwd(int dtype, const void* dy, int64_t lddy, int N, int D, int H, int W, int C, void* dx,
                     int64_t lddx, int accumulate, void* stream);
int hdu_upsample_bwd(int dtype, const void* dxe, int64_t lddxe, int N, int D, int H, int W, int C, int ud, int uh,
                     int uw, void* dz, int64_t lddz, int accumulate, void* stream);

int hdu_wce_loss(int dtype, const void* logits, int64_t ldl, const uint8_t* labels, int64_t M, float w0, float w1,
                 float w2, float grad_scale, void* dlogits, int64_t lddl, int C_pad, float* loss_sum,
                 float* class_count, void* ws, size_t ws_bytes, void* stream);

int hdu_sgd_nesterov(float* p, float* v, const float* g, int64_t n, float lr, float momentum, float grad_scale,
                     void* stream);

int hdu_slab25d(int dtype, const float* vol, int D, int H, int W, void* out, int Cpad, void* stream);
int hdu_make_input3d(int dtype, const float* vol, const void* logits2d, int64_t ldl, float scale, int D, int H,
                     int W, void* out, int Cpad, void* stream);
int hdu_make_input3d_bwd(int dtype, const void* dinput3d, int Cpad, float scale, int64_t M, void* dlogits2d,
                         int64_t lddl, int Cpad_l, int accumulate, void* stream);

int hdu_cast_pad(int dtype, const float* src, int64_t M, int C, void* dst, int64_t lddst, int Cpad, void* stream);
int hdu_cast_out(int dtype, const void* src, int64_t ldsrc, int64_t M, int C, float* dst, void* stream);

int hdu_softmax_accumulate(int dtype, const void* logits, int64_t ldl, int64_t M, int num, float* score, void* stream);

#define HDU_ZERO_BLOCK_BYTES 65536
typedef struct hdu_zero_entry {
  void* ptr;
  uint64_t bytes;
  uint32_t block_begin;
  uint32_t pad_;
  const void* src;
} hdu_zero_entry;
int hdu_zero_regions(const hdu_zero_entry* dev_table, int n, uint32_t total_blocks, uint32_t* counter, uint32_t counter_inc,
                     void* stream);
int hdu_zero(void* ptr, uint64_t bytes, void* stream);

#define HDU_SPLIT3_OPERAND 0
#define HDU_SPLIT3_GRADIENT 1
typedef struct hdu_split3_entry {
  const float* src;
  void* dst;
  const float* a;
  const float* b;
  uint64_t ld_src;
  uint64_t rows;
  uint32_t C;
  uint32_t relu;
  uint32_t pattern;
  uint32_t cols;
  uint32_t col_groups;
  uint32_t block_begin;
  uint32_t iters;
  uint32_t chl;
} hdu_split3_entry;
int hdu_split3_entry_fill(hdu_split3_entry* e, const float* src, int64_t ld_src, int64_t rows, int C, const float* a,
                          const float* b, int relu, int pattern, void* dst, uint32_t block_begin, uint32_t* nblocks);
int hdu_split3_batched(const hdu_split3_entry* dev_table, int n, uint32_t total_blocks, int chl, void* stream);

#define HDU_PP_AND 0
#define HDU_PP_LABEL 1
int hdu_pp_threshold(const float* score, const float* count, int X, int Y, int Z, int deps, int rows, int num,
                     double thres_liver, double thres_tumor, uint8_t* liver, uint8_t* tumor, void* stream);
int hdu_pp_dilate(const uint8_t* in, int X, int Y, int Z, uint8_t* out, void* stream);
int hdu_pp_label(const uint8_t* mask, int X, int Y, int Z, int connectivity, int background, uint32_t* root, void* stream);
int hdu_pp_largest(const uint32_t* root, int X, int Y, int Z, uint32_t* area, uint64_t* best, uint32_t* ncomp, uint8_t* out,
                   void* stream);
int hdu_pp_fill_holes(const uint8_t* mask, int X, int Y, int Z, uint32_t* root, uint8_t* flag, uint8_t* out, void* stream);
int hdu_pp_bbox(const uint8_t* mask, int X, int Y, int Z, uint32_t* box, void* stream);
int hdu_pp_merge(int op, const uint8_t* a, const uint8_t* b, int64_t n, uint8_t* out, void* stream);

typedef struct hdu_comm hdu_comm;
int hdu_comm_unique_id(void* id128);
int hdu_comm_init(hdu_comm** comm, int rank, int world, const void* id128);
int hdu_comm_destroy(hdu_comm* comm);
int hdu_comm_allreduce_f32(hdu_comm* comm, float* buf, int64_t n, void* stream);
int hdu_comm_sendrecv(hdu_comm* comm, int lo_rank, const void* send_lo, void* recv_lo, int hi_rank, const void* send_hi,
                      void* recv_hi, size_t bytes, void* stream);

#ifdef __cplusplus
}
#endif
#endif
```

Baseline: 531.4.

## Add split-K halo conv kernel for small spatial 3x3 convolutions

Adds a new halo-tiled 3x3 conv kernel with configurable tile width and split-K across channel chunks. Partial results are reduced through a workspace with a ticket counter, and the last block runs the epilogue, including a fused BN-backward variant. The kernel is dispatched ahead of the generic implicit GEMM for small feature maps, which should raise occupancy and halo reuse where the igemm path underfills the GPU. The cost is extra workspace traffic and atomics for the split reduction. The shared epilogue is moved to a common header and generalised from a fixed 32-pixel tile width to TW.

Result: no change. 529.9 (median of 3 runs) (-0.3%).

```diff
diff --git a/h-denseunet_amd/csrc/conv_halo_common.h b/h-denseunet_amd/csrc/conv_halo_common.h
--- /dev/null
+++ b/h-denseunet_amd/csrc/conv_halo_common.h
@@ -0,0 +1,168 @@
+#pragma once
+#include "conv_common.h"
+
+typedef float f32x16 __attribute__((ext_vector_type(16)));
+
+__device__ __forceinline__ f32x16 hdu_mfma_32x32x16_bf16(u32x4 a, u32x4 b, f32x16 c) {
+#ifdef HDU_EMU
+  return hipemu_mfma_32x32x16_bf16(__builtin_bit_cast(hipemu_u16x8, a), __builtin_bit_cast(hipemu_u16x8, b), c);
+#else
+  return __builtin_amdgcn_mfma_f32_32x32x16_bf16(__builtin_bit_cast(hdu_bf16x8, a), __builtin_bit_cast(hdu_bf16x8, b), c, 0, 0, 0);
+#endif
+}
+
+template <int N> __device__ __forceinline__ void hw_wait_vmcnt() {
+  static_assert(N >= 0 && N < 64, "vmcnt immediate");
+#ifndef HDU_EMU
+  asm volatile("s_waitcnt vmcnt(%0)" ::"i"(N) : "memory");
+#endif
+}
+
+
+template <typename C, typename RowValid>
+__device__ __forceinline__ void hw_epilogue_stats(const ConvK& p, const char* smem, int n0, int tid, unsigned slot, RowValid valid) {
+  constexpr int NCC = C::BN / 8, CPI = C::NTHR / 16;
+  float* dst = p.stats_partial + (long long)(slot % (unsigned)p.stats_slots) * 2 * p.Cout;
+  const int rl = tid & 15;
+#pragma unroll 1
+  for (int it = 0; it < (NCC + CPI - 1) / CPI; ++it) {
+    const int cc = (tid >> 4) + it * CPI;
+    const int nbase = n0 + cc * 8;
+    const bool col = cc < NCC && nbase < p.Cout;
+    const int ccq = col ? cc : 0, nc = col ? nbase : 0;
+    float s1[8], s2[8], sh[8];
+#pragma unroll
+    for (int j = 0; j < 8; j += 4) {
+      const f32x4 v4 = *(const f32x4*)(p.stats_shift + nc + j);
+      sh[j] = v4[0]; sh[j + 1] = v4[1]; sh[j + 2] = v4[2]; sh[j + 3] = v4[3];
+    }
+#pragma unroll
+    for (int j = 0; j < 8; ++j) { s1[j] = 0.f; s2[j] = 0.f; }
+#pragma unroll 1
+    for (int q0 = 0; q0 < C::BM / 16; q0 += 8) {
+      u32x4 rv[8];
+#pragma unroll
+      for (int q = 0; q < 8; ++q) rv[q] = *(const u32x4*)(smem + (rl + (q0 + q) * 16) * C::ROWB + ccq * 16);
+#pragma unroll
+      for (int q = 0; q < 8; ++q) {
+        const float keep = (col && valid(rl + (q0 + q) * 16)) ? 1.f : 0.f;
+        float f[8];
+        Chunk<bf16_t>::unpack(rv[q], f);
+#pragma unroll
+        for (int j = 0; j < 8; ++j) { const float d = (f[j] - sh[j]) * keep; s1[j] += d; s2[j] += d * d; }
+      }
+    }
+#pragma unroll
+    for (int j = 0; j < 8; ++j) { s1[j] = hdu_row16_sum(s1[j]); s2[j] = hdu_row16_sum(s2[j]); }
+    float mine = 0.f;
+#pragma unroll
+    for (int j = 0; j < 8; ++j) {
+      mine = rl == j ? s1[j] : mine;
+      mine = rl == 8 + j ? s2[j] : mine;
+    }
+    if (col) atomicAdd(dst + (rl < 8 ? 0 : p.Cout) + nbase + (rl & 7), mine);
+  }
+}
+
+template <typename C>
+__device__ __forceinline__ void hw_epilogue(const ConvK& p, f32x16 (&acc)[C::MT][C::NTW], char* smem, long long mplane, int y0, int x0,
+                                            int n0, int wm, int wn, int lane, int tid, unsigned slot) {
+  typedef bf16_t T;
+  constexpr int BN = C::BN, BM = C::BM, NTHR = C::NTHR, ROWB = C::ROWB, MT = C::MT, NTW = C::NTW;
+  const int l31 = lane & 31, lh = lane >> 5;
+  hw_wait_vmcnt<0>();
+  __syncthreads();
+  const unsigned dseed = p.drop_seed + (p.drop_seed_dev ? *p.drop_seed_dev : 0u);
+  const bool has_bias = p.bias != nullptr, drop = p.drop_scale != 0.f, has_epi = p.epi_a != nullptr;
+#pragma unroll
+  for (int j = 0; j < NTW; ++j) {
+    f32x4 bias_v[4], epa_v[4], epb_v[4];
+#pragma unroll
+    for (int g = 0; g < 4; ++g) {
+      const int nn = n0 + (wn * NTW + j) * 32 + 8 * g + 4 * lh;
+      const int nc = nn < p.Cout ? nn : 0;
+      bias_v[g] = has_bias ? *(const f32x4*)(p.bias + nc) : f32x4{0.f, 0.f, 0.f, 0.f};
+      epa_v[g] = has_epi ? *(const f32x4*)(p.epi_a + nc) : f32x4{1.f, 1.f, 1.f, 1.f};
+      epb_v[g] = has_epi ? *(const f32x4*)(p.epi_b + nc) : f32x4{0.f, 0.f, 0.f, 0.f};
+    }
+#pragma unroll
+    for (int i = 0; i < MT; ++i) {
+      const int row = (wm * MT + i) * 32 + l31;
+      const long long m = (mplane + y0 + row / C::TW) * p.Wo + x0 + row % C::TW;
+#pragma unroll
+      for (int g = 0; g < 4; ++g) {
+        const int col = (wn * NTW + j) * 32 + 8 * g + 4 * lh;
+        const int nn = n0 + col;
+        float v[4] = {acc[i][j][4 * g], acc[i][j][4 * g + 1], acc[i][j][4 * g + 2], acc[i][j][4 * g + 3]};
+        if (has_bias) {
+#pragma unroll
+          for (int r = 0; r < 4; ++r) v[r] += bias_v[g][r];
+        }
+        if (drop) {
+#pragma unroll
+          for (int r = 0; r < 4; ++r) {
+            const unsigned h = hdu_hash32((unsigned long long)m * (unsigned)p.Cout + (unsigned)(nn + r), dseed);
+            v[r] = h < p.drop_thresh ? v[r] * p.drop_scale : 0.f;
+          }
+        }
+        if (has_epi) {
+#pragma unroll
+          for (int r = 0; r < 4; ++r) {
+            v[r] = epa_v[g][r] * v[r] + epb_v[g][r];
+            if (p.epi_relu) v[r] = v[r] > 0.f ? v[r] : 0.f;
+          }
+        }
+        Chunk<T>::store4((T*)(smem + row * ROWB) + col, v);
+      }
+    }
+  }
+  __syncthreads();
+  T* __restrict__ yp = (T*)p.y;
+  constexpr int NCC = BN / 8;
+  constexpr int NIT = (BM * NCC + NTHR - 1) / NTHR;
+  auto out_ptr = [&](int q, bool& ok) -> T* {
+    const int row = q / NCC, cc = q - row * NCC;
+    const int oy = y0 + row / C::TW, ox = x0 + row % C::TW;
+    const int nn = n0 + cc * 8;
+    ok = q < BM * NCC && oy < p.Ho && ox < p.Wo && nn < p.Cout;
+    return ok ? yp + ((mplane + oy) * p.Wo + ox) * p.ldy + nn : yp;
+  };
+  if (p.accumulate) {
+#pragma unroll 1
+    for (int it0 = 0; it0 < NIT; it0 += 4) {
+      u32x4 old[4];
+      T* dst[4];
+      bool ok[4];
+#pragma unroll
+      for (int u = 0; u < 4; ++u) {
+        dst[u] = out_ptr(tid + (it0 + u) * NTHR, ok[u]);
+        ok[u] = ok[u] && it0 + u < NIT;
+        old[u] = *(const u32x4*)dst[u];
+      }
+#pragma unroll
+      for (int u = 0; u < 4; ++u) {
+        if (!ok[u]) continue;
+        const int q = tid + (it0 + u) * NTHR;
+        const int row = q / NCC, cc = q - row * NCC;
+        float f[8], g[8];
+        Chunk<T>::unpack(*(const u32x4*)(smem + row * ROWB + cc * 16), f);
+        Chunk<T>::unpack(old[u], g);
+#pragma unroll
+        for (int jj = 0; jj < 8; ++jj) f[jj] += g[jj];
+        *(u32x4*)dst[u] = Chunk<T>::pack(f);
+      }
+    }
+  } else {
+#pragma unroll
+    for (int it = 0; it < NIT; ++it) {
+      const int q = tid + it * NTHR;
+      bool ok;
+      T* dst = out_ptr(q, ok);
+      if (!ok) continue;
+      const int row = q / NCC, cc = q - row * NCC;
+      *(u32x4*)dst = *(const u32x4*)(smem + row * ROWB + cc * 16);
+    }
+  }
+  if (p.stats_partial)
+    hw_epilogue_stats<C>(p, smem, n0, tid, slot, [&](int row) { return y0 + row / C::TW < p.Ho && x0 + row % C::TW < p.Wo; });
+}
diff --git a/h-denseunet_amd/csrc/conv_halo_splitk.hip b/h-denseunet_amd/csrc/conv_halo_splitk.hip
--- /dev/null
+++ b/h-denseunet_amd/csrc/conv_halo_splitk.hip
@@ -0,0 +1,428 @@
+#include "conv_halo_common.h"
+#include "hdu_host.h"
+
+template <int TW_, int TH_, int NT_, int WAVES_M_, int NS_> struct HaloSplit {
+  static constexpr int TW = TW_, TH = TH_, NT = NT_, WAVES_M = WAVES_M_, WAVES_N = 4 / WAVES_M_, NS = NS_;
+  static constexpr int NW = 4, NTHR = 256;
+  static constexpr int HC = TW + 2, HR = TH + 2, HP = HR * HC;
+  static constexpr int BN = NT * 32, BM = TH * TW, PF = BM / 32;
+  static constexpr int XI = (HP * 2 + 63) / 64, WI = (BN * 18 + 63) / 64;
+  static constexpr int LPW = (XI + WI + NW - 1) / NW;
+  static constexpr int STAGE = LPW * NW * 1024, XBYTES = XI * 1024;
+  static constexpr int ROWB = BN * 2 + 16;
+  static constexpr int SMEM = NS * STAGE > BM * ROWB ? NS * STAGE : BM * ROWB;
+  static constexpr int MT = PF / WAVES_M, NTW = NT / WAVES_N;
+  static constexpr int SPLIT_FLOATS = NW * MT * NTW * 16 * 64;
+  static_assert(BM % 32 == 0 && PF % WAVES_M == 0 && NT % WAVES_N == 0 && WAVES_M * WAVES_N == 4, "wave layout");
+  static_assert(BN == 32 || BN == 64 || BN == 128, "BN-backward epilogue: a power-of-two number of 16-byte chunks per row");
+  static_assert(SMEM <= 160 * 1024, "LDS");
+  static_assert((NS - 2) * LPW < 64, "vmcnt");
+};
+
+template <typename C>
+__device__ __forceinline__ bool hs_combine(const ConvK& p, f32x16 (&acc)[C::MT][C::NTW], char* smem, unsigned tile, int z, int S,
+                                           int n0, int wn, int wave, int lane, int tid) {
+  constexpr int MT = C::MT, NTW = C::NTW;
+  float* base = p.sk_ws + (size_t)tile * (size_t)S * C::SPLIT_FLOATS;
+  const size_t woff = (size_t)wave * MT * NTW * 4 * 256 + lane * 4;
+  float* mine = base + (size_t)z * C::SPLIT_FLOATS + woff;
+#pragma unroll
+  for (int i = 0; i < MT; ++i)
+#pragma unroll
+    for (int j = 0; j < NTW; ++j)
+#pragma unroll
+      for (int g = 0; g < 4; ++g)
+        if (n0 + (wn * NTW + j) * 32 + 8 * g < p.Cout)
+          hdu_store_wt16(mine + ((i * NTW + j) * 4 + g) * 256, f32x4{acc[i][j][4 * g], acc[i][j][4 * g + 1], acc[i][j][4 * g + 2], acc[i][j][4 * g + 3]});
+  HDU_WAIT_STORES();
+  __syncthreads();
+  int* flag = (int*)smem;
+  if (tid == 0) *flag = hdu_ticket(p.sk_cnt + tile) == (unsigned)(S - 1) ? 1 : 0;
+  __syncthreads();
+  if (*flag == 0) return false;
+  if (tid == 0) hdu_acquire_agent();
+  __syncthreads();
+#pragma unroll
+  for (int i = 0; i < MT; ++i)
+#pragma unroll
+    for (int j = 0; j < NTW; ++j)
+#pragma unroll
+      for (int r = 0; r < 16; ++r) acc[i][j][r] = 0.f;
+  for (int s = 0; s < S; ++s) {
+    const float* o = base + (size_t)s * C::SPLIT_FLOATS + woff;
+#pragma unroll
+    for (int i = 0; i < MT; ++i)
+#pragma unroll
+      for (int j = 0; j < NTW; ++j)
+#pragma unroll
+        for (int g = 0; g < 4; ++g)
+          if (n0 + (wn * NTW + j) * 32 + 8 * g < p.Cout) {
+            const f32x4 v = *(const f32x4*)(o + ((i * NTW + j) * 4 + g) * 256);
+#pragma unroll
+            for (int r = 0; r < 4; ++r) acc[i][j][4 * g + r] += v[r];
+          }
+  }
+  if (tid == 0) hdu_store_agent_u32(p.sk_cnt + tile, 0u);
+  return true;
+}
+
+template <typename C>
+__device__ __forceinline__ void hs_epilogue_bnb(const ConvK& p, f32x16 (&acc)[C::MT][C::NTW], char* smem, long long mplane, int y0,
+                                                int x0, int n0, int wm, int wn, int lane, int tid) {
+  typedef bf16_t T;
+  constexpr int BN = C::BN, BM = C::BM, ROWB = C::ROWB, MT = C::MT, NTW = C::NTW, TW = C::TW;
+  constexpr int NCC = BN / 8, RSTEP = 256 / NCC, IT = BM / RSTEP;
+  static_assert(BM % RSTEP == 0, "tile rows");
+  const int cc = tid % NCC, r0 = tid / NCC;
+  const int n = n0 + cc * 8;
+  const bool col_ok = n < p.Cout;
+  const T* __restrict__ up = (const T*)p.bnb_u;
+  T* __restrict__ yp = (T*)p.y;
+  long long mrow[IT];
+  bool okr[IT];
+  u32x4 uv[IT], ov[IT];
+  hw_wait_vmcnt<0>();
+#pragma unroll
+  for (int q = 0; q < IT; ++q) {
+    const int row = r0 + q * RSTEP;
+    const int oy = y0 + row / TW, ox = x0 + row % TW;
+    okr[q] = col_ok && oy < p.Ho && ox < p.Wo;
+    mrow[q] = (mplane + oy) * p.Wo + ox;
+    uv[q] = *(const u32x4*)(up + (okr[q] ? mrow[q] * p.bnb_ldu + n : 0));
+    ov[q] = *(const u32x4*)(yp + ((okr[q] && p.accumulate) ? mrow[q] * p.ldy + n : 0));
+  }
+  __syncthreads();
+  const int l31 = lane & 31, lh = lane >> 5;
+#pragma unroll
+  for (int i = 0; i < MT; ++i) {
+    const int row = (wm * MT + i) * 32 + l31;
+#pragma unroll
+    for (int j = 0; j < NTW; ++j)
+#pragma unroll
+      for (int g = 0; g < 4; ++g) {
+        const int col = (wn * NTW + j) * 32 + 8 * g + 4 * lh;
+        float v[4] = {acc[i][j][4 * g], acc[i][j][4 * g + 1], acc[i][j][4 * g + 2], acc[i][j][4 * g + 3]};
+        Chunk<T>::store4((T*)(smem + row * ROWB) + col, v);
+      }
+  }
+  __syncthreads();
+  const bool sums = p.bnb_partial != nullptr;
+  const bool relu = (p.bnb_relu & 1) != 0, from_z = (p.bnb_relu & 2) != 0, raw = (p.bnb_relu & 4) != 0;
+  float a[8], b[8], mu[8], rs[8], s1[8], s2[8];
+  {
+    const int nc = col_ok ? n : 0;
+    const float* pmu = sums ? p.bnb_mean : p.bnb_a;
+    const float* prs = sums ? p.bnb_rstd : p.bnb_a;
+#pragma unroll
+    for (int j = 0; j < 8; j += 4) {
+      const f32x4 va = *(const f32x4*)(p.bnb_a + nc + j), vb = *(const f32x4*)(p.bnb_b + nc + j);
+      const f32x4 vm = *(const f32x4*)(pmu + nc + j), vr = *(const f32x4*)(prs + nc + j);
+#pragma unroll
+      for (int r = 0; r < 4; ++r) { a[j + r] = va[r]; b[j + r] = vb[r]; mu[j + r] = sums ? vm[r] : 0.f; rs[j + r] = sums ? vr[r] : 0.f; }
+    }
+    if (from_z) {
+#pragma unroll
+      for (int j = 0; j < 8; ++j) { mu[j] = b[j] + a[j] * mu[j]; rs[j] = a[j] != 0.f ? rs[j] / a[j] : 0.f; }
+    }
+#pragma unroll
+    for (int j = 0; j < 8; ++j) { s1[j] = 0.f; s2[j] = 0.f; }
+  }
+#pragma unroll
+  for (int q = 0; q < IT; ++q) {
+    if (!okr[q]) continue;
+    const int row = r0 + q * RSTEP;
+    float dz[8], u[8], o[8];
+    Chunk<T>::unpack(*(const u32x4*)(smem + row * ROWB + cc * 16), dz);
+    Chunk<T>::unpack(uv[q], u);
+#pragma unroll
+    for (int j = 0; j < 8; ++j) {
+      const float sj = from_z ? u[j] : a[j] * u[j] + b[j];
+      const float g = (!relu || sj > 0.f) ? dz[j] : 0.f;
+      s1[j] += g;
+      s2[j] += g * ((u[j] - mu[j]) * rs[j]);
+      o[j] = raw ? dz[j] : a[j] * g;
+    }
+    if (p.accumulate) {
+      float old[8];
+      Chunk<T>::unpack(ov[q], old);
+#pragma unroll
+      for (int j = 0; j < 8; ++j) o[j] += old[j];
+    }
+    *(u32x4*)(yp + mrow[q] * p.ldy + n) = Chunk<T>::pack(o);
+  }
+  if (!sums) return;
+#pragma unroll
+  for (int mask = NCC; mask < 64; mask <<= 1) {
+#pragma unroll
+    for (int j = 0; j < 8; ++j) { s1[j] += __shfl_xor(s1[j], mask); s2[j] += __shfl_xor(s2[j], mask); }
+  }
+  __syncthreads();
+  float* red = (float*)smem;
+  const int wave = tid >> 6;
+  if (lane < NCC) {
+#pragma unroll
+    for (int j = 0; j < 8; ++j) {
+      red[(wave * 2 + 0) * BN + cc * 8 + j] = s1[j];
+      red[(wave * 2 + 1) * BN + cc * 8 + j] = s2[j];
+    }
+  }
+  __syncthreads();
+  float* dst = p.bnb_partial + (long long)(blockIdx.x % (unsigned)p.bnb_slots) * 2 * p.Cout;
+  for (int q = tid; q < 2 * BN; q += 256) {
+    const int sidx = q / BN, col = q - sidx * BN;
+    if (n0 + col < p.Cout) {
+      const float t = red[(0 * 2 + sidx) * BN + col] + red[(1 * 2 + sidx) * BN + col] + red[(2 * 2 + sidx) * BN + col] +
+                      red[(3 * 2 + sidx) * BN + col];
+      atomicAdd(dst + (long long)sidx * p.Cout + n0 + col, t);
+    }
+  }
+}
+
+template <typename C, bool BNB>
+__global__ __launch_bounds__(256) void conv_halo_splitk_kernel(ConvK p, int tiles_x, int tiles_y, int ngroups, int nsplit) {
+  typedef bf16_t T;
+  constexpr int TW = C::TW, HC = C::HC, HP = C::HP, BN = C::BN, NW = C::NW, NS = C::NS;
+  constexpr int XI = C::XI, WI = C::WI, LPW = C::LPW, STAGE = C::STAGE, XBYTES = C::XBYTES;
+  constexpr int MT = C::MT, NTW = C::NTW;
+  __shared__ __attribute__((aligned(16))) char smem[C::SMEM];
+
+  const int tid = threadIdx.x;
+  const int lane = tid & 63;
+#ifdef HDU_EMU
+  const int wave = tid >> 6;
+#else
+  const int wave = __builtin_amdgcn_readfirstlane(tid >> 6);
+#endif
+  const int wm = wave / C::WAVES_N, wn = wave % C::WAVES_N;
+  const T* __restrict__ xp = (const T*)p.x;
+
+  unsigned t = (p.xcd_swizzle & 1) ? xcd_tile_index(blockIdx.x, gridDim.x) : blockIdx.x;
+  const int z = (int)(t % (unsigned)nsplit); t /= (unsigned)nsplit;
+  const unsigned tile = t;
+  const int ng = (int)(t % (unsigned)ngroups); t /= (unsigned)ngroups;
+  const int od = (int)(t % (unsigned)p.Do); t /= (unsigned)p.Do;
+  const int txi = (int)(t % (unsigned)tiles_x); t /= (unsigned)tiles_x;
+  const int tyi = (int)(t % (unsigned)tiles_y);
+  const int n = (int)(t / (unsigned)tiles_y);
+  const int y0 = tyi * C::TH, x0 = txi * TW;
+  const int n0 = ng * BN;
+
+  unsigned roff[LPW];
+  int rlc[LPW];
+#pragma unroll
+  for (int j = 0; j < LPW; ++j) {
+    const int jj = j * NW + wave;
+    if (jj < XI) {
+      const int q = jj * 64 + lane;
+      const int hp = q >> 1;
+      const int lc = (q & 1) ^ ((hp >> 3) & 1);
+      const int hr = hp / HC, hc = hp - hr * HC;
+      const int iy = y0 - 1 + hr, ix = x0 - 1 + hc;
+      const bool ok = hp < HP && (unsigned)iy < (unsigned)p.He && (unsigned)ix < (unsigned)p.We;
+      roff[j] = ok ? (unsigned)((iy * p.Wi + ix) * (int)p.ldx + lc * 8) * 2u : HDU_OOB;
+      rlc[j] = lc * 8;
+    } else if (jj < XI + WI) {
+      const int q = (jj - XI) * 64 + lane;
+      const int row = q / 18, rem = q - row * 18;
+      const int tap = rem >> 1;
+      const int lc = (rem & 1) ^ ((row >> 3) & 1);
+      const int co = n0 + row;
+      const bool ok = row < BN && co < p.Cout;
+      roff[j] = ok ? (unsigned)((co * 9 + tap) * p.Cin + lc * 8) * 2u : HDU_OOB;
+      rlc[j] = lc * 8;
+    } else {
+      roff[j] = HDU_OOB;
+      rlc[j] = 0;
+    }
+  }
+  const hdu_bufsrd wsrd = hdu_make_srd(p.w, p.w_bytes);
+  const T* plane = xp + (long long)(n * p.Di + od) * ((long long)p.Hi * p.Wi * p.ldx);
+  const unsigned plane_bytes = (unsigned)((((long long)p.Hi * p.Wi - 1) * p.ldx + p.Cin) * 2);
+  auto issue_piece = [&](const hdu_bufsrd& xsrd, int c0, char* base, int j, bool live) {
+    const int jj = j * NW + wave;
+    const bool ok = live && roff[j] != HDU_OOB && c0 + rlc[j] < p.Cin;
+    if (jj < XI) hdu_bufload_lds16(xsrd, ok ? roff[j] : HDU_OOB, base + jj * 1024);
+    else hdu_bufload_lds16(wsrd, ok ? roff[j] + (unsigned)c0 * 2u : HDU_OOB, base + jj * 1024);
+  };
+
+  f32x16 acc[MT][NTW];
+#pragma unroll
+  for (int i = 0; i < MT; ++i)
+#pragma unroll
+    for (int j = 0; j < NTW; ++j)
+#pragma unroll
+      for (int r = 0; r < 16; ++r) acc[i][j][r] = 0.f;
+
+  const int nch = (p.Cin + 15) >> 4;
+  const int c_lo = nch * z / nsplit, c_hi = nch * (z + 1) / nsplit;
+  const int nst = c_hi - c_lo;
+  int ic = c_lo;
+#pragma unroll
+  for (int pre = 0; pre < NS - 1; ++pre) {
+    const bool live = pre < nst;
+    const int c0 = live ? ic * 16 : 0;
+    const hdu_bufsrd xsrd = hdu_make_srd(plane + c0, plane_bytes - (unsigned)c0 * 2u);
+#pragma unroll
+    for (int j = 0; j < LPW; ++j) issue_piece(xsrd, c0, smem + pre * STAGE, j, live);
+    if (live) ++ic;
+  }
+
+  const int l31 = lane & 31, lh = lane >> 5;
+  int wrow_off[NTW], hp_base[MT];
+#pragma unroll
+  for (int j = 0; j < NTW; ++j) {
+    const int row = (wn * NTW + j) * 32 + l31;
+    wrow_off[j] = XBYTES + row * 288 + ((lh ^ ((row >> 3) & 1)) << 4);
+  }
+#pragma unroll
+  for (int i = 0; i < MT; ++i) {
+    const int px = (wm * MT + i) * 32 + l31;
+    hp_base[i] = (px / TW) * HC + px % TW;
+  }
+
+  int slot = 0;
+  for (int s = 0; s < nst; ++s) {
+    hw_wait_vmcnt<(NS - 2) * LPW>();
+    HDU_RAW_BARRIER();
+    const bool more = s + NS - 1 < nst;
+    const int nc0 = more ? ic * 16 : 0;
+    const hdu_bufsrd nxsrd = hdu_make_srd(plane + nc0, plane_bytes - (unsigned)nc0 * 2u);
+    char* nbase = smem + (slot == 0 ? NS - 1 : slot - 1) * STAGE;
+    if (more) ++ic;
+    const char* Xs = smem + slot * STAGE;
+    constexpr int PER_TAP = (LPW + 8) / 9;
+#pragma unroll
+    for (int tap = 0; tap < 9; ++tap) {
+      const int kh = tap / 3, kw = tap - kh * 3;
+      u32x4 af[MT], bf[NTW];
+#pragma unroll
+      for (int i = 0; i < MT; ++i) {
+        const int hp = hp_base[i] + kh * HC + kw;
+        af[i] = *(const u32x4*)(Xs + hp * 32 + ((lh ^ ((hp >> 3) & 1)) << 4));
+      }
+#pragma unroll
+      for (int j = 0; j < NTW; ++j) bf[j] = *(const u32x4*)(Xs + wrow_off[j] + tap * 32);
+#pragma unroll
+      for (int i = 0; i < MT; ++i)
+#pragma unroll
+        for (int j = 0; j < NTW; ++j) acc[i][j] = hdu_mfma_32x32x16_bf16(bf[j], af[i], acc[i][j]);
+#pragma unroll
+      for (int u = 0; u < PER_TAP; ++u)
+        if (tap * PER_TAP + u < LPW) issue_piece(nxsrd, nc0, nbase, tap * PER_TAP + u, more);
+    }
+    slot = slot == NS - 1 ? 0 : slot + 1;
+  }
+
+  if (nsplit > 1) {
+    hw_wait_vmcnt<0>();
+    if (!hs_combine<C>(p, acc, smem, tile, z, nsplit, n0, wn, wave, lane, tid)) return;
+  }
+  const long long mplane = ((long long)n * p.Do + od) * p.Ho;
+  if constexpr (BNB) hs_epilogue_bnb<C>(p, acc, smem, mplane, y0, x0, n0, wm, wn, lane, tid);
+  else hw_epilogue<C>(p, acc, smem, mplane, y0, x0, n0, wm, wn, lane, tid, blockIdx.x);
+}
+
+typedef HaloSplit<32, 8, 2, 4, 3> HS_32x8;
+typedef HaloSplit<16, 8, 2, 4, 3> HS_16x8;
+typedef HaloSplit<32, 8, 1, 4, 3> HS_32x8n;
+typedef HaloSplit<16, 8, 1, 4, 3> HS_16x8n;
+
+struct HsPlan {
+  int cfg;
+  int tw, th, bn;
+  int tiles_x, tiles_y, ngroups, nsplit;
+  long long tiles;
+};
+
+static bool hs_shape_ok(const ConvK& k, int dtype) {
+  if (dtype != HDU_BF16 || k.pro_a != nullptr || k.skip != nullptr || !k.vec_out || (k.ud | k.uh | k.uw) != 0) return false;
+  if (k.KD != 1 || k.KH != 3 || k.KW != 3 || k.sd != 1 || k.sh != 1 || k.sw != 1 || k.pd != 0 || k.ph != 1 || k.pw != 1) return false;
+  if (k.Do != k.De || k.Ho != k.He || k.Wo != k.We) return false;
+  if (k.Cin % 8 || k.Cout % 8) return false;
+  if ((long long)k.Hi * k.Wi * k.ldx * 2 >= (1ll << 32)) return false;
+  if ((long long)k.Cout * 9 * k.Cin * 2 >= (1ll << 32)) return false;
+  return true;
+}
+
+static HsPlan hs_plan(const ConvK& k, int dtype) {
+  HsPlan pl{};
+  const int knob = g_tuning[HDU_TUNE_SMALL_HALO];
+  if (knob < 2 || !hs_shape_ok(k, dtype)) return pl;
+  if (k.We > 32 || k.Cin < 16) return pl;
+  pl.tw = k.We <= 16 ? 16 : 32;
+  pl.th = 8;
+  pl.bn = k.Cout <= 32 ? 32 : 64;
+  pl.tiles_x = (k.We + pl.tw - 1) / pl.tw;
+  pl.tiles_y = (k.He + pl.th - 1) / pl.th;
+  pl.ngroups = (k.Cout + pl.bn - 1) / pl.bn;
+  const long long per_plane = (long long)pl.tiles_x * pl.tiles_y * pl.ngroups;
+  pl.tiles = (long long)k.N * k.Do * per_plane;
+  const int nch = (k.Cin + 15) / 16;
+  int S = knob - 1;
+  if (g_tuning[HDU_TUNE_SPLITK] == 1) S = 1;
+  if (S > nch) S = nch;
+  if (S > 16) S = 16;
+  if (S < 1) S = 1;
+  pl.nsplit = S;
+  if (pl.tiles * S >= (1ll << 31)) return pl;
+  if (S > 1 && pl.tiles > 512) return pl;
+  pl.cfg = pl.tw == 32 ? (pl.bn == 64 ? 1 : 3) : (pl.bn == 64 ? 2 : 4);
+  return pl;
+}
+
+static size_t hs_split_floats(int cfg) {
+  switch (cfg) {
+    case 1: return HS_32x8::SPLIT_FLOATS;
+    case 2: return HS_16x8::SPLIT_FLOATS;
+    case 3: return HS_32x8n::SPLIT_FLOATS;
+    default: return HS_16x8n::SPLIT_FLOATS;
+  }
+}
+
+static size_t hs_ws_bytes(const HsPlan& pl) {
+  return pl.cfg && pl.nsplit > 1 ? (size_t)pl.tiles * (size_t)pl.nsplit * hs_split_floats(pl.cfg) * sizeof(float) : 0;
+}
+
+static bool hs_taken(const ConvK& k, int dtype, size_t sk_bytes_avail, HsPlan* out) {
+  const HsPlan pl = hs_plan(k, dtype);
+  if (out) *out = pl;
+  if (!pl.cfg) return false;
+  return pl.nsplit == 1 || (k.sk_ws && k.sk_cnt && hs_ws_bytes(pl) <= sk_bytes_avail);
+}
+
+template <typename C>
+static void hs_launch(const ConvK& k, const HsPlan& pl, hipStream_t s) {
+  const unsigned grid = (unsigned)(pl.tiles * pl.nsplit);
+  if (k.bnb_u != nullptr)
+    HDU_LAUNCH((conv_halo_splitk_kernel<C, true>), dim3(grid), dim3(256), 0, s, k, pl.tiles_x, pl.tiles_y, pl.ngroups, pl.nsplit);
+  else
+    HDU_LAUNCH((conv_halo_splitk_kernel<C, false>), dim3(grid), dim3(256), 0, s, k, pl.tiles_x, pl.tiles_y, pl.ngroups, pl.nsplit);
+}
+
+bool hdu_halo_splitk_taken(const ConvK& k, int dtype, size_t sk_bytes_avail) { return hs_taken(k, dtype, sk_bytes_avail, nullptr); }
+
+size_t hdu_halo_splitk_ws_bytes(const ConvK& k, int dtype) { return hs_ws_bytes(hs_plan(k, dtype)); }
+
+const char* hdu_halo_splitk_name(const ConvK& k, int dtype, size_t sk_bytes_avail) {
+  HsPlan pl;
+  if (!hs_taken(k, dtype, sk_bytes_avail, &pl)) return "";
+  static const char* names[2][5] = {
+      {"", "conv_halo_splitk_kernel<32x8x64>", "conv_halo_splitk_kernel<16x8x64>", "conv_halo_splitk_kernel<32x8x32>",
+       "conv_halo_splitk_kernel<16x8x32>"},
+      {"", "conv_halo_splitk_kernel<32x8x64,bnb>", "conv_halo_splitk_kernel<16x8x64,bnb>", "conv_halo_splitk_kernel<32x8x32,bnb>",
+       "conv_halo_splitk_kernel<16x8x32,bnb>"}};
+  return names[k.bnb_u != nullptr ? 1 : 0][pl.cfg];
+}
+
+bool hdu_halo_splitk_launch(const ConvK& k, int dtype, size_t sk_bytes_avail, hipStream_t s) {
+  HsPlan pl;
+  if (!hs_taken(k, dtype, sk_bytes_avail, &pl)) return false;
+  ConvK kk = k;
+  if (pl.nsplit == 1) { kk.sk_ws = nullptr; kk.sk_cnt = nullptr; }
+  switch (pl.cfg) {
+    case 1: hs_launch<HS_32x8>(kk, pl, s); return true;
+    case 2: hs_launch<HS_16x8>(kk, pl, s); return true;
+    case 3: hs_launch<HS_32x8n>(kk, pl, s); return true;
+    default: hs_launch<HS_16x8n>(kk, pl, s); return true;
+  }
+}
diff --git a/h-denseunet_amd/csrc/conv_halo_wide.hip b/h-denseunet_amd/csrc/conv_halo_wide.hip
--- a/h-denseunet_amd/csrc/conv_halo_wide.hip
+++ b/h-denseunet_amd/csrc/conv_halo_wide.hip
@@ -1,22 +1,5 @@
-#include "conv_common.h"
+#include "conv_halo_common.h"
 #include "hdu_host.h"
-
-typedef float f32x16 __attribute__((ext_vector_type(16)));
-
-__device__ __forceinline__ f32x16 hdu_mfma_32x32x16_bf16(u32x4 a, u32x4 b, f32x16 c) {
-#ifdef HDU_EMU
-  return hipemu_mfma_32x32x16_bf16(__builtin_bit_cast(hipemu_u16x8, a), __builtin_bit_cast(hipemu_u16x8, b), c);
-#else
-  return __builtin_amdgcn_mfma_f32_32x32x16_bf16(__builtin_bit_cast(hdu_bf16x8, a), __builtin_bit_cast(hdu_bf16x8, b), c, 0, 0, 0);
-#endif
-}
-
-template <int N> __device__ __forceinline__ void hw_wait_vmcnt() {
-  static_assert(N >= 0 && N < 64, "vmcnt immediate");
-#ifndef HDU_EMU
-  asm volatile("s_waitcnt vmcnt(%0)" ::"i"(N) : "memory");
-#endif
-}
 
 template <int TH_, int NT_, int WAVES_M_, int WAVES_N_, int NS_> struct HaloWide {
   static constexpr int TH = TH_, NT = NT_, WAVES_M = WAVES_M_, WAVES_N = WAVES_N_, NS = NS_;
@@ -35,155 +18,6 @@
   static_assert(SMEM <= 160 * 1024, "LDS");
   static_assert((NS - 2) * LPW < 64, "vmcnt");
 };
-
-template <typename C, typename RowValid>
-__device__ __forceinline__ void hw_epilogue_stats(const ConvK& p, const char* smem, int n0, int tid, unsigned slot, RowValid valid) {
-  constexpr int NCC = C::BN / 8, CPI = C::NTHR / 16;
-  float* dst = p.stats_partial + (long long)(slot % (unsigned)p.stats_slots) * 2 * p.Cout;
-  const int rl = tid & 15;
-#pragma unroll 1
-  for (int it = 0; it < (NCC + CPI - 1) / CPI; ++it) {
-    const int cc = (tid >> 4) + it * CPI;
-    const int nbase = n0 + cc * 8;
-    const bool col = cc < NCC && nbase < p.Cout;
-    const int ccq = col ? cc : 0, nc = col ? nbase : 0;
-    float s1[8], s2[8], sh[8];
-#pragma unroll
-    for (int j = 0; j < 8; j += 4) {
-      const f32x4 v4 = *(const f32x4*)(p.stats_shift + nc + j);
-      sh[j] = v4[0]; sh[j + 1] = v4[1]; sh[j + 2] = v4[2]; sh[j + 3] = v4[3];
-    }
-#pragma unroll
-    for (int j = 0; j < 8; ++j) { s1[j] = 0.f; s2[j] = 0.f; }
-#pragma unroll 1
-    for (int q0 = 0; q0 < C::BM / 16; q0 += 8) {
-      u32x4 rv[8];
-#pragma unroll
-      for (int q = 0; q < 8; ++q) rv[q] = *(const u32x4*)(smem + (rl + (q0 + q) * 16) * C::ROWB + ccq * 16);
-#pragma unroll
-      for (int q = 0; q < 8; ++q) {
-        const float keep = (col && valid(rl + (q0 + q) * 16)) ? 1.f : 0.f;
-        float f[8];
-        Chunk<bf16_t>::unpack(rv[q], f);
-#pragma unroll
-        for (int j = 0; j < 8; ++j) { const float d = (f[j] - sh[j]) * keep; s1[j] += d; s2[j] += d * d; }
-      }
-    }
-#pragma unroll
-    for (int j = 0; j < 8; ++j) { s1[j] = hdu_row16_sum(s1[j]); s2[j] = hdu_row16_sum(s2[j]); }
-    float mine = 0.f;
-#pragma unroll
-    for (int j = 0; j < 8; ++j) {
-      mine = rl == j ? s1[j] : mine;
-      mine = rl == 8 + j ? s2[j] : mine;
-    }
-    if (col) atomicAdd(dst + (rl < 8 ? 0 : p.Cout) + nbase + (rl & 7), mine);
-  }
-}
-
-template <typename C>
-__device__ __forceinline__ void hw_epilogue(const ConvK& p, f32x16 (&acc)[C::MT][C::NTW], char* smem, long long mplane, int y0, int x0,
-                                            int n0, int wm, int wn, int lane, int tid, unsigned slot) {
-  typedef bf16_t T;
-  constexpr int BN = C::BN, BM = C::BM, NTHR = C::NTHR, ROWB = C::ROWB, MT = C::MT, NTW = C::NTW;
-  const int l31 = lane & 31, lh = lane >> 5;
-  hw_wait_vmcnt<0>();
-  __syncthreads();
-  const unsigned dseed = p.drop_seed + (p.drop_seed_dev ? *p.drop_seed_dev : 0u);
-  const bool has_bias = p.bias != nullptr, drop = p.drop_scale != 0.f, has_epi = p.epi_a != nullptr;
-#pragma unroll
-  for (int j = 0; j < NTW; ++j) {
-    f32x4 bias_v[4], epa_v[4], epb_v[4];
-#pragma unroll
-    for (int g = 0; g < 4; ++g) {
-      const int nn = n0 + (wn * NTW + j) * 32 + 8 * g + 4 * lh;
-      const int nc = nn < p.Cout ? nn : 0;
-      bias_v[g] = has_bias ? *(const f32x4*)(p.bias + nc) : f32x4{0.f, 0.f, 0.f, 0.f};
-      epa_v[g] = has_epi ? *(const f32x4*)(p.epi_a + nc) : f32x4{1.f, 1.f, 1.f, 1.f};
-      epb_v[g] = has_epi ? *(const f32x4*)(p.epi_b + nc) : f32x4{0.f, 0.f, 0.f, 0.f};
-    }
-#pragma unroll
-    for (int i = 0; i < MT; ++i) {
-      const int trow = wm * MT + i;
-      const int row = trow * 32 + l31;
-      const long long m = (mplane + y0 + trow) * p.Wo + x0 + l31;
-#pragma unroll
-      for (int g = 0; g < 4; ++g) {
-        const int col = (wn * NTW + j) * 32 + 8 * g + 4 * lh;
-        const int nn = n0 + col;
-        float v[4] = {acc[i][j][4 * g], acc[i][j][4 * g + 1], acc[i][j][4 * g + 2], acc[i][j][4 * g + 3]};
-        if (has_bias) {
-#pragma unroll
-          for (int r = 0; r < 4; ++r) v[r] += bias_v[g][r];
-        }
-        if (drop) {
-#pragma unroll
-          for (int r = 0; r < 4; ++r) {
-            const unsigned h = hdu_hash32((unsigned long long)m * (unsigned)p.Cout + (unsigned)(nn + r), dseed);
-            v[r] = h < p.drop_thresh ? v[r] * p.drop_scale : 0.f;
-          }
-        }
-        if (has_epi) {
-#pragma unroll
-          for (int r = 0; r < 4; ++r) {
-            v[r] = epa_v[g][r] * v[r] + epb_v[g][r];
-            if (p.epi_relu) v[r] = v[r] > 0.f ? v[r] : 0.f;
-          }
-        }
-        Chunk<T>::store4((T*)(smem + row * ROWB) + col, v);
-      }
-    }
-  }
-  __syncthreads();
-  T* __restrict__ yp = (T*)p.y;
-  constexpr int NCC = BN / 8;
-  constexpr int NIT = (BM * NCC + NTHR - 1) / NTHR;
-  auto out_ptr = [&](int q, bool& ok) -> T* {
-    const int row = q / NCC, cc = q - row * NCC;
-    const int oy = y0 + (row >> 5), ox = x0 + (row & 31);
-    const int nn = n0 + cc * 8;
-    ok = q < BM * NCC && oy < p.Ho && ox < p.Wo && nn < p.Cout;
-    return ok ? yp + ((mplane + oy) * p.Wo + ox) * p.ldy + nn : yp;
-  };
-  if (p.accumulate) {
-#pragma unroll 1
-    for (int it0 = 0; it0 < NIT; it0 += 4) {
-      u32x4 old[4];
-      T* dst[4];
-      bool ok[4];
-#pragma unroll
-      for (int u = 0; u < 4; ++u) {
-        dst[u] = out_ptr(tid + (it0 + u) * NTHR, ok[u]);
-        ok[u] = ok[u] && it0 + u < NIT;
-        old[u] = *(const u32x4*)dst[u];
-      }
-#pragma unroll
-      for (int u = 0; u < 4; ++u) {
-        if (!ok[u]) continue;
-        const int q = tid + (it0 + u) * NTHR;
-        const int row = q / NCC, cc = q - row * NCC;
-        float f[8], g[8];
-        Chunk<T>::unpack(*(const u32x4*)(smem + row * ROWB + cc * 16), f);
-        Chunk<T>::unpack(old[u], g);
-#pragma unroll
-        for (int jj = 0; jj < 8; ++jj) f[jj] += g[jj];
-        *(u32x4*)dst[u] = Chunk<T>::pack(f);
-      }
-    }
-  } else {
-#pragma unroll
-    for (int it = 0; it < NIT; ++it) {
-      const int q = tid + it * NTHR;
-      bool ok;
-      T* dst = out_ptr(q, ok);
-      if (!ok) continue;
-      const int row = q / NCC, cc = q - row * NCC;
-      *(u32x4*)dst = *(const u32x4*)(smem + row * ROWB + cc * 16);
-    }
-  }
-  if (p.stats_partial)
-    hw_epilogue_stats<C>(p, smem, n0, tid, slot, [&](int row) { return y0 + (row >> 5) < p.Ho && x0 + (row & 31) < p.Wo; });
-}
 
 template <typename C>
 __global__ __launch_bounds__(C::NTHR) void conv_halo_wide_kernel(ConvK p, int tiles_x, int tiles_y, int ngroups) {
diff --git a/h-denseunet_amd/csrc/conv_igemm.hip b/h-denseunet_amd/csrc/conv_igemm.hip
--- a/h-denseunet_amd/csrc/conv_igemm.hip
+++ b/h-denseunet_amd/csrc/conv_igemm.hip
@@ -2755,10 +2755,10 @@
 
 #include "hdu_host.h"
 
-int g_tuning[32] = {2, 0, 0, 1, 0, 0, 0, 0, 0, 0, 0, 0, 0, 0, 0, 0, 0, 0, 0, 0, 0, 0, 0, 0, 0, 0, 0, 0, 0, 0, 0, 0};
+int g_tuning[HDU_TUNE_KEYS] = {2, 0, 0, 1};
 
 extern "C" int hdu_set_tuning(int key, int value) {
-  if (key < 0 || key >= 32) return hdu_set_error(HDU_ERR_ARG, "set_tuning: bad key");
+  if (key < 0 || key >= HDU_TUNE_KEYS) return hdu_set_error(HDU_ERR_ARG, "set_tuning: bad key");
   g_tuning[key] = value;
   return 0;
 }
@@ -3072,6 +3072,12 @@
 bool hdu_halo_wide_launch(const ConvK& k, int dtype, hipStream_t s);
 bool hdu_stem_wgrad_taken(const ConvK& k, int dtype);
 bool hdu_stem_wgrad_launch(const ConvK& k, int dtype, float* dw, hipStream_t s);
+bool hdu_halo_splitk_taken(const ConvK& k, int dtype, size_t sk_bytes_avail);
+size_t hdu_halo_splitk_ws_bytes(const ConvK& k, int dtype);
+const char* hdu_halo_splitk_name(const ConvK& k, int dtype, size_t sk_bytes_avail);
+bool hdu_halo_splitk_launch(const ConvK& k, int dtype, size_t sk_bytes_avail, hipStream_t s);
+
+static bool small_halo_ok(const ConvK& k, int dtype, size_t sk_bytes_avail) { return hdu_halo_splitk_taken(k, dtype, sk_bytes_avail); }
 
 static bool fprop_halo_ok(const ConvK& k, int dtype) {
   return dtype == HDU_BF16 && k.bnb_u == nullptr && !g_tuning[HDU_TUNE_NO_HALO_FPROP] && k.pro_a == nullptr && k.skip == nullptr && k.KD == 1 &&
@@ -3159,6 +3165,10 @@
     }
     return hdu_check_launch("conv_fprop(halo)");
   }
+  if (small_halo_ok(k, d->dtype, d->splitk_ws_bytes)) {
+    hdu_halo_splitk_launch(k, d->dtype, d->splitk_ws_bytes, (hipStream_t)stream);
+    return hdu_check_launch("conv_fprop(halo, split-K)");
+  }
   if (d->dtype == HDU_BF16) dispatch_igemm<bf16_t>(k, d->splitk_ws_bytes, (hipStream_t)stream);
   else dispatch_igemm<float>(k, d->splitk_ws_bytes, (hipStream_t)stream);
   return hdu_check_launch("conv_fprop");
@@ -3168,6 +3178,7 @@
   ConvK k;
   if (fill_convk(d, &k, false)) return 0;
   if (k.M == 0 || pw_bstat_ok(k, d->dtype) || hdu_halo_wide_taken(k, d->dtype) || fprop_halo_ok(k, d->dtype) || (k.pro_a != nullptr && !igemm_pro_dma_ok(k)) || k.skip != nullptr) return 0;
+  if (small_halo_ok(k, d->dtype, (size_t)-1)) return hdu_halo_splitk_ws_bytes(k, d->dtype);
   int bm, bn;
   choose_igemm(k, &bm, &bn);
   if (bm == 128 && igemm_pers_ok(k, bn)) return 0;
@@ -3514,6 +3525,8 @@
     snprintf(buf, buflen, "%s", hdu_halo_wide_name(k, d->dtype));
   } else if (fprop_halo_ok(k, d->dtype)) {
     snprintf(buf, buflen, "conv_halo_fprop_kernel<%d>", choose_halo_bn(k));
+  } else if (small_halo_ok(k, d->dtype, d->splitk_ws_bytes)) {
+    snprintf(buf, buflen, "%s", hdu_halo_splitk_name(k, d->dtype, d->splitk_ws_bytes));
   } else {
     int bm, bn;
     choose_igemm(k, &bm, &bn);
diff --git a/h-denseunet_amd/csrc/hdu_host.h b/h-denseunet_amd/csrc/hdu_host.h
--- a/h-denseunet_amd/csrc/hdu_host.h
+++ b/h-denseunet_amd/csrc/hdu_host.h
@@ -12,4 +12,4 @@
   return (unsigned)b;
 }
 
-extern int g_tuning[32];
+extern int g_tuning[HDU_TUNE_KEYS];
diff --git a/h-denseunet_amd/engine.py b/h-denseunet_amd/engine.py
--- a/h-denseunet_amd/engine.py
+++ b/h-denseunet_amd/engine.py
@@ -954,7 +954,7 @@
             return False
         if self._sums_kernel_ok is None:
             name = ops.conv_kernel_name(d, 0)
-            self._sums_kernel_ok = name.startswith("conv_igemm_ring_kernel") or name.startswith("conv_igemm_dma_kernel")
+            self._sums_kernel_ok = name.startswith(("conv_igemm_ring_kernel", "conv_igemm_dma_kernel", "conv_halo_splitk_kernel"))
         if not self._sums_kernel_ok or not bn.takes_epilogue_sums(self.x):
             return False
         x = self.x.act
diff --git a/h-denseunet_amd/lib.py b/h-denseunet_amd/lib.py
--- a/h-denseunet_amd/lib.py
+++ b/h-denseunet_amd/lib.py
@@ -244,6 +244,8 @@
         lib.hdu_set_tuning(8, int(os.environ["HDU_NO_HALO"]))
     if "HDU_HALO_WIDE" in os.environ:
         lib.hdu_set_tuning(29, int(os.environ["HDU_HALO_WIDE"]))
+    if "HDU_SMALL_HALO" in os.environ:
+        lib.hdu_set_tuning(32, int(os.environ["HDU_SMALL_HALO"]))
     if "HDU_HALO_MIN_W" in os.environ:
         lib.hdu_set_tuning(28, int(os.environ["HDU_HALO_MIN_W"]))
     if "HDU_HALO_TARGET" in os.environ:
diff --git a/include/hdu.h b/include/hdu.h
--- a/include/hdu.h
+++ b/include/hdu.h
@@ -55,6 +55,8 @@
 #define HDU_TUNE_HALO_WIDE 29
 #define HDU_TUNE_SPLIT3_FORM 31
 #define HDU_TUNE_WGRAD_NCT 21
+#define HDU_TUNE_SMALL_HALO 32
+#define HDU_TUNE_KEYS 33
 int hdu_set_tuning(int key, int value);
 
 typedef struct hdu_conv_desc {
```
